# zhoubin-me/agent0

Hardware: AMD Instinct MI355X
Metric: env-frames/sec (learner FPS: transitions collected and saved to replay per second with the learner running, pre-frameskip) (higher is better)
Workload: dtype f32

## Files before the change

agent0_amd/common/atari_wrappers.py:

```python
from __future__ import annotations

from typing import Optional

import torch

ACTION_DIMS = {"Asterix": 9, "BeamRider": 9, "Breakout": 4, "Enduro": 9, "MsPacman": 9, "Qbert": 6, "Seaquest": 18, "SpaceInvaders": 6, "Pong": 6}


class _Space:
    def __init__(self, shape=None, n=None):
        self.shape, self.n = shape, n

    def __getitem__(self, i):
        return self


class DeviceSynthVecEnv:

    H = W = 84
    TASKS = {"stream": 0, "block": 1, "chase": 2}

    def __init__(self, env_id: str, num_envs: int, seed: int = 42, rank: int = 0, ops=None, task: str = "stream"):
        if task not in self.TASKS:
            raise ValueError(f"env_task={task!r}: expected one of {sorted(self.TASKS)}")
# ... 4 lines not shown
        self.ops, self.E, self.seed, self.rank = ops, num_envs, seed, rank
        self.env_id = env_id
        self.action_dim = ACTION_DIMS.get(env_id, 18)
        self.observation_space = _Space(shape=(num_envs, 4, self.H, self.W))
        self.action_space = _Space(n=self.action_dim)
        n = num_envs * 4 * self.H * self.W
        self._obs = [ops.zeros(n, dtype=torch.uint8), ops.zeros(n, dtype=torch.uint8)]
        self._cur = 0
        self.ep_ret = ops.zeros(num_envs)
        self.reward, self.terminal, self.truncated = ops.zeros(num_envs), ops.zeros(num_envs), ops.zeros(num_envs)
        self.life_loss, self.final_mask, self.final_ret = ops.zeros(num_envs), ops.zeros(num_envs), ops.zeros(num_envs)
        self.g = 0

    @property
    def obs(self) -> torch.Tensor:
        return self._obs[self._cur]

    def set_history(self, k: int):
        k = max(int(k), 2)
        if k != len(self._obs):
            n = self._obs[0].numel()
            cur = self._obs[self._cur]
            self._obs = [cur] + [self.ops.zeros(n, dtype=torch.uint8) for _ in range(k - 1)]
            self._cur = 0

    def history(self, j: int) -> torch.Tensor:
        return self._obs[(self._cur - j) % len(self._obs)]

    def reset(self, **kwargs):
        self.g = 0
        self._cur = 0
        self.ops.env_reset(self.seed, self.rank, self.E, self._obs[0], self.ep_ret, task=self.task)
        return self._obs[0], {}

    def step(self, action: torch.Tensor, final_mask: Optional[torch.Tensor] = None, final_ret: Optional[torch.Tensor] = None, ctrl: Optional[torch.Tensor] = None):
        self.g += 1
        nxt = (self._cur + 1) % len(self._obs)
        fm = self.final_mask if final_mask is None else final_mask
        fr = self.final_ret if final_ret is None else final_ret
        self.ops.env_step(self.seed, self.rank, self.E, self.g, self._obs[self._cur], self._obs[nxt], self.ep_ret, self.reward,
                          self.terminal, self.truncated, self.life_loss, fm, fr, ctrl, action=action, A=self.action_dim, task=self.task)
        self._cur = nxt
        info = {"life_loss": self.life_loss, "final_mask": fm, "final_ret": fr}
        return self._obs[nxt], self.reward, self.terminal, self.truncated, info

    def step_commit(self, action, final_mask, final_ret, n, steps, gamma, ring_act, ring_rew, ring_done, obs0, replay, start_slot, ctrl=None):
        self.g += 1
        nxt = (self._cur + 1) % len(self._obs)
        self.ops.env_step_commit(self.seed, self.rank, self.E, self.g, self._obs[self._cur], self._obs[nxt], self.ep_ret, final_mask, final_ret, n, steps, gamma,
                                 action, ring_act, ring_rew, ring_done, obs0, replay.frames, replay.size, start_slot, replay.act, replay.rew, replay.done, ctrl, A=self.action_dim, task=self.task)
        self._cur = nxt
        return self._obs[nxt]

    def act_step_commit(self, tail_args, final_mask, final_ret, n, steps, gamma, ring_act, ring_rew, ring_done, obs0, replay, start_slot, kind: str = "qhead", enc=None):
        self.g += 1
        nxt = (self._cur + 1) % len(self._obs)
        common = (self.seed, self.rank, self.g, self._obs[self._cur], self._obs[nxt], self.ep_ret, final_mask, final_ret, n, steps, gamma, ring_act, ring_rew, ring_done, obs0,
                  replay.frames, replay.size, start_slot, replay.act, replay.rew, replay.done)
        if enc is not None:
            {"qhead": self.ops.actor_qhead_env_step_enc, "dist": self.ops.actor_dist_tail_env_step_enc, "quantile": self.ops.actor_quantile_tail_env_step_enc}[kind](
                *tail_args, *common, task=self.task, wt=enc[0], enc_w=enc[1], act3_next=enc[2])
        else:
            {"qhead": self.ops.actor_qhead_env_step, "dist": self.ops.actor_dist_tail_env_step, "quantile": self.ops.actor_quantile_tail_env_step}[kind](*tail_args, *common, task=self.task)
        self._cur = nxt
        return self._obs[nxt]

    def state_dict(self) -> dict:
        return {"g": int(self.g), "cur": int(self._cur), "seed": int(self.seed), "rank": int(self.rank), "obs": torch.stack(self._obs).cpu(), "ep_ret": self.ep_ret.cpu()}

    def load_state_dict(self, sd: dict):
        if len(sd["obs"]) != len(self._obs) or sd["obs"][0].numel() != self._obs[0].numel():
            raise ValueError(f"env state: {len(sd['obs'])} observation buffers of {sd['obs'][0].numel()} bytes, this env keeps {len(self._obs)} of {self._obs[0].numel()}")
        self.g, self._cur, self.seed, self.rank = int(sd["g"]), int(sd["cur"]), int(sd["seed"]), int(sd["rank"])
        for dst, src in zip(self._obs, sd["obs"]):
            dst.copy_(torch.as_tensor(src).reshape(-1))
        self.ep_ret.copy_(torch.as_tensor(sd["ep_ret"]))

    def close(self):
        pass


from .host_envs import AtariSlice, FireOnReset, LifeLossInfo, PRESS_AFTER_RESET


def real_atari_available() -> bool:
    try:
        import gymnasium, ale_py
    except ImportError:
        return False
    return True


def make_atari(env_id: str, num_envs: int, episode_life: bool = True, seed: int = 42, rank: int = 0, ops=None, synthetic=None, num_workers=None, task: str = "stream",
               groups: int = 1):
    groups = int(groups)
    if not 1 <= groups <= int(num_envs):
        raise ValueError(f"make_atari: groups={groups} must lie in [1, num_envs={num_envs}] (actor.env_groups)")
    if synthetic is None:
        synthetic = not real_atari_available()
    if synthetic:
        return DeviceSynthVecEnv(env_id, num_envs, seed=seed, rank=rank, ops=ops, task=task)
    from .env_pool import HostEnvGroups, HostEnvPool

    if num_workers is None:
        num_workers = 0 if num_envs < 4 else min(16, max(1, num_envs // 16))
    if groups >= 2:
        return HostEnvGroups(AtariSlice(env_id, episode_life, seed + 1000003 * rank), num_envs, groups=groups, obs_shape=(4, 84, 84),
                             action_dim=ACTION_DIMS.get(env_id, 18), num_workers=num_workers, ops=ops)
    return HostEnvPool(AtariSlice(env_id, episode_life, seed + 1000003 * rank), num_envs, obs_shape=(4, 84, 84), action_dim=ACTION_DIMS.get(env_id, 18),
                       num_workers=num_workers, ops=ops)
```

agent0_amd/csrc/net.hip:

```cpp
#include "igemm_x9.h"
#include "short_k_fwd.h"
#include "a0_internal.h"
#include "net_impl.h"
#include "update_tail.h"

#include <vector>

__global__ __launch_bounds__(256) void a0_reduce_slabs_kernel(const float* __restrict__ slabs, long long slab_stride, int nslab,
                                                               float* __restrict__ out, long long count) {
    __shared__ float red[8][33];
    const int c = threadIdx.x & 31, g = threadIdx.x >> 5;
    const long long i = (long long)blockIdx.x * 32 + c;
    float s = 0.f;
    if (i < count)
        for (int z = g; z < nslab; z += 8) s += slabs[(long long)z * slab_stride + i];
    red[g][c] = s;
    __syncthreads();
    if (g == 0 && i < count) {
        float t = 0.f;
#pragma unroll
        for (int j = 0; j < 8; ++j) t += red[j][c];
        out[i] = t;
    }
}
// ... 494 lines not shown
extern "C" int a0_dense_fwd_partial_multi_slabs(int n, int R, int N, int K) { return a0_fwd_multi_splits(n, R, N, K); }

extern "C" int a0_dense_fwd_partial_multi(int n, const float* const* X, int ldx, const float* const* W, int R, int N, int K, float* const* slabs, const long long* slab_stride,
                                          void* stream) {
    A0_TRY
    if (!X || !W || !slabs || (ldx & 3) || !a0_dense_fwd_partial_multi_ok(n, R, N, K)) return a0_fail(A0_EINVAL, "a0_dense_fwd_partial_multi: shapes a0_dense_fwd_partial_multi_ok accepts");
    a0_x9_group<OpMatKC, OpMatKC, EpiSlab> grp;
    for (int i = 0; i < 3; ++i) {
        const int j = i < n ? i : 0;
        if (!X[j] || !W[j] || !slabs[j]) return a0_fail(A0_EINVAL, "a0_dense_fwd_partial_multi: null operand");
        grp.pa[i] = a0_mat_src{X[j], ldx};
        grp.pb[i] = a0_mat_src{W[j], K};
        const long long stride = slab_stride ? slab_stride[j] : (long long)R * N;
        if (stride < (long long)R * N || (stride & 3)) return a0_fail(A0_EINVAL, "a0_dense_fwd_partial_multi: slab stride");
        grp.pe[i] = EpiSlab::Params{slabs[j], stride, N};
    }
    const int splits = a0_fwd_multi_splits(n, R, N, K);
    hipEvent_t e0 = nullptr, e1 = nullptr;
    const bool probe = a0_probe_events(A0_TAG_DENSE_FWD, &e0, &e1);
    A0_HIP_THROW((a0_igemm_x9_group_launch<OpMatKC, OpMatKC, EpiSlab, 4, 2, 1, 1>((hipStream_t)stream, n, grp, R, N, K, splits, e0, e1)));
    if (probe) a0_probe_commit(2.0 * n * (double)R * (double)N * (double)K);
    return A0_OK;
    A0_CATCH
}

#include "actor_tail.h"
__global__ __launch_bounds__(256) void a0_actor_qhead_kernel(const float* __restrict__ slabs, long long slab_stride, int nslab, const float* __restrict__ b1,
                                                             const float* __restrict__ W2, const float* __restrict__ b2, int A, int dueling, int E,
                                                             unsigned long long seed, uint32_t stream_a, uint32_t stream_u, unsigned long long off_a,
                                                             unsigned long long off_u, float eps, const long long* __restrict__ ctrl,
                                                             const float* __restrict__ eps_ptr, int* __restrict__ action, float* __restrict__ qmax) {
    __shared__ float raw[4][64];
    extern __shared__ float w2s[];
    const int lane = threadIdx.x & 63, wave = threadIdx.x >> 6;
    const int e = blockIdx.x * 4 + wave;
    const int NQ = A + (dueling ? 1 : 0);
    for (int i = threadIdx.x; i < NQ * 128; i += 256) ((a0_f4*)w2s)[i] = ((const a0_f4*)W2)[i];
    __syncthreads();
    if (e >= E) return;
    if (ctrl) { off_a += (unsigned long long)ctrl[A0_CTRL_RNG_ACTION]; off_u += (unsigned long long)ctrl[A0_CTRL_RNG_UNIFORM]; }
    eps = a0_env_eps(eps, eps_ptr, (uint32_t)__builtin_amdgcn_readfirstlane(e));
    int act = 0; float best = 0.f;
    a0_qhead_wave(slabs, slab_stride, nslab, b1, w2s, b2, A, dueling, e, lane, raw[wave], seed, stream_a, stream_u, off_a, off_u, eps, act, best);
    if (lane == 0) { action[e] = act; qmax[e] = best; }
}

__global__ __launch_bounds__(512) void a0_actor_qhead_env_kernel(a0_qenv_args P) {
    __shared__ float raw[64];
    __shared__ int s_chase_cell;
    extern __shared__ float w2s[];
    a0_actor_qhead_env_body(P, raw, w2s, &s_chase_cell);
}

extern "C" long long a0_actor_qhead_scratch(int E, int K) {
    const int splits = a0_fc1_splits(E, 512, K);
    return (long long)splits * E * 512;
}

extern "C" int a0_actor_qhead_n(const float* feat, int E, int K, int splits, const float* W1, const float* b1, const float* W2, const float* b2, int A, int dueling,
                                float* scratch, unsigned long long seed, unsigned int stream_a, unsigned int stream_u, unsigned long long off_a,
                                unsigned long long off_u, float eps, const long long* ctrl, const float* eps_ptr, int* action, float* qmax, void* stream) {
    A0_TRY
    if (!feat || !W1 || !b1 || !W2 || !b2 || !scratch || !action || !qmax || E < 1 || K < 4 || (K & 3) || A < 1 || A + (dueling ? 1 : 0) > 24)
        return a0_fail(A0_EINVAL, "a0_actor_qhead: bad argument (A + dueling <= 24: the head rows are staged in 48 KB of LDS)");
    if (splits < 1 || splits > 64 || splits > (K + 31) / 32) return a0_fail(A0_EINVAL, "a0_actor_qhead_n: splits must lie in [1, min(64, ceil(K / 32))]");
    a0_hip_backend bk{(hipStream_t)stream};
    a0_mat_src a{feat, K};
    a0_mat_src bw{W1, K};
    EpiSlab::Params ep{scratch, (long long)E * 512, 512};
    bk.tag = A0_TAG_DENSE_FWD;
    a0_fc1_partial_launch(bk, a, bw, ep, E, 512, K, splits);
    hipLaunchKernelGGL(a0_actor_qhead_kernel, dim3((E + 3) / 4), dim3(256), (size_t)(A + (dueling ? 1 : 0)) * 512 * sizeof(float), (hipStream_t)stream, scratch, (long long)E * 512, splits, b1, W2, b2, A, dueling, E,
                       seed, stream_a, stream_u, off_a, off_u, eps, ctrl, eps_ptr, action, qmax);
    A0_HIP_THROW(hipGetLastError());
    return A0_OK;
    A0_CATCH
}

extern "C" int a0_actor_qhead(const float* feat, int E, int K, const float* W1, const float* b1, const float* W2, const float* b2, int A, int dueling,
                              float* scratch, unsigned long long seed, unsigned int stream_a, unsigned int stream_u, unsigned long long off_a,
                              unsigned long long off_u, float eps, const long long* ctrl, const float* eps_ptr, int* action, float* qmax, void* stream) {
    return a0_actor_qhead_n(feat, E, K, a0_fc1_splits(E, 512, K), W1, b1, W2, b2, A, dueling, scratch, seed, stream_a, stream_u, off_a, off_u, eps, ctrl, eps_ptr, action,
                            qmax, stream);
}

extern "C" int a0_actor_qhead_env_step(const float* feat, int E, int K, const float* W1, const float* b1, const float* W2, const float* b2, int A, int dueling,
                                       float* scratch, unsigned long long seed, unsigned int stream_a, unsigned int stream_u, unsigned long long off_a,
                                       unsigned long long off_u, float eps, const long long* ctrl, const float* eps_ptr, int* action, float* qmax,
                                       unsigned long long env_seed, unsigned int rank, unsigned int g, const uint8_t* obs_in, uint8_t* obs_out, float* ep_ret,
                                       float* final_mask, float* final_ret, int n, long long steps, double gamma, int* ring_act, float* ring_rew, float* ring_done,
                                       const uint8_t* obs0, uint8_t* frames, long long cap, long long start_slot, int* r_act, float* r_rew, float* r_done, int task, void* stream) {
    A0_TRY
    if (!feat || !W1 || !b1 || !W2 || !b2 || !scratch || !action || !qmax || E < 1 || K < 4 || (K & 3) || A < 1 || A + (dueling ? 1 : 0) > 24)
        return a0_fail(A0_EINVAL, "a0_actor_qhead_env_step: bad argument (A + dueling <= 24: the head rows are staged in 48 KB of LDS)");
    if (!obs_in || !obs_out || obs_in == obs_out || !ep_ret || !final_mask || !final_ret || !ring_act || !ring_rew || !ring_done || !obs0 || !frames || !r_act ||
        !r_rew || !r_done || n < 1 || steps < 0 || cap < E || start_slot < 0 || task < A0_ENV_TASK_STREAM || task > A0_ENV_TASK_CHASE || (task == A0_ENV_TASK_CHASE && A < 4))
        return a0_fail(A0_EINVAL, "a0_actor_qhead_env_step: bad env argument (the chase task needs at least four actions)");
    if ((((uintptr_t)obs_in) | ((uintptr_t)obs_out) | ((uintptr_t)obs0) | ((uintptr_t)frames)) & 15) return a0_fail(A0_EINVAL, "a0_actor_qhead_env_step: buffers must be 16-byte aligned");
    a0_hip_backend bk{(hipStream_t)stream};
    const int splits = a0_fc1_splits(E, 512, K);
    a0_mat_src a{feat, K};
    a0_mat_src bw{W1, K};
    EpiSlab::Params ep{scratch, (long long)E * 512, 512};
    bk.tag = A0_TAG_DENSE_FWD;
    a0_fc1_partial_launch(bk, a, bw, ep, E, 512, K, splits);
    a0_qenv_args P;
    P.slabs = scratch; P.slab_stride = (long long)E * 512; P.nslab = splits; P.b1 = b1; P.W2 = W2; P.b2 = b2; P.A = A; P.dueling = dueling; P.E = E;
    P.rng_seed = seed; P.stream_a = stream_a; P.stream_u = stream_u; P.off_a = off_a; P.off_u = off_u; P.eps = eps; P.ctrl = ctrl; P.eps_ptr = eps_ptr;
    P.action = action; P.qmax = qmax;
    P.env_seed = env_seed; P.rank = rank; P.g = g; P.obs_in = obs_in; P.obs_out = obs_out; P.ep_ret = ep_ret; P.final_mask = final_mask; P.final_ret = final_ret;
    P.n = n; P.steps = steps; P.gamma = gamma; P.ring_act = ring_act; P.ring_rew = ring_rew; P.ring_done = ring_done; P.obs0 = obs0; P.frames = frames;
    P.cap = cap; P.start = start_slot % cap; P.r_act = r_act; P.r_rew = r_rew; P.r_done = r_done; P.task = task;
    hipLaunchKernelGGL(a0_actor_qhead_env_kernel, dim3(E), dim3(512), (size_t)(A + (dueling ? 1 : 0)) * 512 * sizeof(float), (hipStream_t)stream, P);
    A0_HIP_THROW(hipGetLastError());
    return A0_OK;
    A0_CATCH
}

extern "C" int a0_actor_qhead_env_step_enc(const float* feat, int E, int K, const float* W1, const float* b1, const float* W2, const float* b2, int A, int dueling,
                                           float* scratch, unsigned long long seed, unsigned int stream_a, unsigned int stream_u, unsigned long long off_a,
                                           unsigned long long off_u, float eps, const long long* ctrl, const float* eps_ptr, int* action, float* qmax,
                                           unsigned long long env_seed, unsigned int rank, unsigned int g, const uint8_t* obs_in, uint8_t* obs_out, float* ep_ret,
                                           float* final_mask, float* final_ret, int n, long long steps, double gamma, int* ring_act, float* ring_rew, float* ring_done,
                                           const uint8_t* obs0, uint8_t* frames, long long cap, long long start_slot, int* r_act, float* r_rew, float* r_done, int task,
                                           const float* wt, const a0_encoder_weights* w, float* act3_next, void* stream) {
    A0_TRY
    if (!feat || !W1 || !b1 || !W2 || !b2 || !scratch || !action || !qmax || E < 1 || K != 3136 || A < 1 || A + (dueling ? 1 : 0) > 24)
        return a0_fail(A0_EINVAL, "a0_actor_qhead_env_step_enc: bad argument (4 x 84 x 84 observations, A + dueling <= 24)");
    if (!obs_in || !obs_out || obs_in == obs_out || !ep_ret || !final_mask || !final_ret || !ring_act || !ring_rew || !ring_done || !obs0 || !frames || !r_act ||
        !r_rew || !r_done || n < 1 || steps < 0 || cap < E || start_slot < 0 || task < A0_ENV_TASK_STREAM || task > A0_ENV_TASK_CHASE || (task == A0_ENV_TASK_CHASE && A < 4))
        return a0_fail(A0_EINVAL, "a0_actor_qhead_env_step_enc: bad env argument");
    if ((((uintptr_t)obs_in) | ((uintptr_t)obs_out) | ((uintptr_t)obs0) | ((uintptr_t)frames)) & 15) return a0_fail(A0_EINVAL, "a0_actor_qhead_env_step_enc: buffers must be 16-byte aligned");
    a0_hip_backend bk{(hipStream_t)stream};
    const int splits = a0_fc1_splits(E, 512, K);
    a0_mat_src a{feat, K};
    a0_mat_src bw{W1, K};
    EpiSlab::Params ep{scratch, (long long)E * 512, 512};
    bk.tag = A0_TAG_DENSE_FWD;
    a0_fc1_partial_launch(bk, a, bw, ep, E, 512, K, splits);
    a0_qenv_args P;
    P.slabs = scratch; P.slab_stride = (long long)E * 512; P.nslab = splits; P.b1 = b1; P.W2 = W2; P.b2 = b2; P.A = A; P.dueling = dueling; P.E = E;
    P.rng_seed = seed; P.stream_a = stream_a; P.stream_u = stream_u; P.off_a = off_a; P.off_u = off_u; P.eps = eps; P.ctrl = ctrl; P.eps_ptr = eps_ptr;
    P.action = action; P.qmax = qmax;
    P.env_seed = env_seed; P.rank = rank; P.g = g; P.obs_in = obs_in; P.obs_out = obs_out; P.ep_ret = ep_ret; P.final_mask = final_mask; P.final_ret = final_ret;
    P.n = n; P.steps = steps; P.gamma = gamma; P.ring_act = ring_act; P.ring_rew = ring_rew; P.ring_done = ring_done; P.obs0 = obs0; P.frames = frames;
    P.cap = cap; P.start = start_slot % cap; P.r_act = r_act; P.r_rew = r_rew; P.r_done = r_done; P.task = task;
    return a0_actor_step_enc_launch(P, wt, w, act3_next, (hipStream_t)stream);
    A0_CATCH
}

__global__ __launch_bounds__(256) void a0_mean_rows_kernel(const float* __restrict__ x, int E, float* __restrict__ out) {
    __shared__ float red[256];
    const float* p = x + (long long)blockIdx.x * E;
    float s = 0.f;
    for (int e = threadIdx.x; e < E; e += 256) s += p[e];
    red[threadIdx.x] = s;
    __syncthreads();
    for (int o = 128; o > 0; o >>= 1) { if ((int)threadIdx.x < o) red[threadIdx.x] += red[threadIdx.x + o]; __syncthreads(); }
    if (threadIdx.x == 0) out[blockIdx.x] = red[0] / (float)E;
}

extern "C" int a0_mean_rows(const float* x, int T, int E, float* out, void* stream) {
    if (!x || !out || T < 1 || E < 1) return a0_fail(A0_EINVAL, "a0_mean_rows: bad argument");
    hipLaunchKernelGGL(a0_mean_rows_kernel, dim3(T), dim3(256), 0, (hipStream_t)stream, x, E, out);
    return a0_fail_hip((int)hipGetLastError(), "a0_mean_rows");
}

extern "C" int a0_dense_dgrad(const float* dY, const float* W, const float* act_mask, float* dX, int R, int N, int K, void* stream) {
    A0_TRY
    if (!dY || !W || !dX || R < 1 || (N & 3) || (K & 3)) return a0_fail(A0_EINVAL, "a0_dense_dgrad: bad shape");
    a0_hip_backend bk{(hipStream_t)stream};
    a0_dense_dgrad_impl(bk, dY, W, act_mask, dX, R, N, K);
    return A0_OK;
    A0_CATCH
}

extern "C" int a0_dense_dgrad_hadamard_ok(int R, int N, int K, int n) {
    return (g_gemm_x9 != 0 && (n == 32 || n == 64) && R >= 4096 && !(R & 255) && !(R % n) && !(N & 15) && N >= 64 && !(K & 3) && K >= 128) ? 1 : 0;
}
extern "C" int a0_dense_dgrad_hadamard(const float* dY, const float* W, const float* emb, const float* feat, float* demb, float* d3, int R, int N, int K, int n, void* stream) {
    A0_TRY
    if (!dY || !W || !emb || !feat || !demb || !d3 || !a0_dense_dgrad_hadamard_ok(R, N, K, n)) return a0_fail(A0_EINVAL, "a0_dense_dgrad_hadamard: shapes a0_dense_dgrad_hadamard_ok accepts");
    const a0_mat_src a{dY, N};
    const a0_mat_src bw{W, K};
    const EpiHadamard::Params e{emb, feat, demb, d3, K, n};
    hipEvent_t e0 = nullptr, e1 = nullptr;
    const bool probe = a0_probe_events(A0_TAG_DENSE_DGRAD, &e0, &e1);
    A0_HIP_THROW((a0_igemm_x9_launch<OpMatKC, OpMatXC, EpiHadamard, 4, 2, 2, 2, 1>((hipStream_t)stream, a, bw, e, R, K, N, 1, e0, e1)));
    if (probe) a0_probe_commit(2.0 * (double)R * (double)N * (double)K);
    return A0_OK;
    A0_CATCH
}

extern "C" int a0_dense_dgrad_wgrad_ok(int R, int N, int K) {
    const long long b128 = (long long)((R + 127) / 128) * ((K + 63) / 64), b64 = (long long)((N + 63) / 64) * ((K + 63) / 64);
    return (g_gemm_x9 != 0 && g_probe.tag == 0 && R == N && R >= 1 && R <= 1024 && !(N & 3) && !(K & 3) && b128 < 256 && b64 >= 256 && N >= 512 &&
            (long long)((R + 127) / 128) * ((K + 127) / 128) < A0_X9_BIG_TILES) ? 1 : 0;
}
static int a0_dense_dgrad_wgrad_small_ok(int R, int N, int K) {
    const long long t1 = (long long)((R + 63) / 64) * ((K + 63) / 64), t2 = (long long)((N + 63) / 64) * ((K + 63) / 64);
    return (g_gemm_x9 != 0 && g_probe.tag == 0 && R >= 64 && R <= 1024 && N >= 64 && !(N & 3) && !(K & 3) && t1 + t2 <= 256 && t2 >= 16) ? 1 : 0;
// ... 126 lines not shown
```

agent0_amd/csrc/runtime.hip:

```cpp
#include "learner_state.h"

#include <chrono>
#include <thread>

namespace {

typedef a0_host_rng Rng;
constexpr int STREAM_EGREEDY_U = 1, STREAM_EGREEDY_A = 2, STREAM_SUMTREE = 5, STREAM_PERM = 6;

struct Owned {
    std::vector<void*> ptrs;
    template <class T> T* alloc(long long n, bool zero = true) {
        void* p = nullptr;
        A0_HIP_THROW(hipMalloc(&p, (size_t)(n > 0 ? n : 1) * sizeof(T)));
        ptrs.push_back(p);
        if (zero) A0_HIP_THROW(hipMemset(p, 0, (size_t)(n > 0 ? n : 1) * sizeof(T)));
        return (T*)p;
    }
    ~Owned() { for (void* p : ptrs) (void)hipFree(p); }
};

__global__ void a0_pow_scalar_kernel(const float* __restrict__ p, double alpha, float* __restrict__ out) {
    const double x = (double)p[0];
    out[0] = (float)(alpha == 0.5 ? sqrt(x) : pow(x, alpha));
// ... 194 lines not shown
        start[g] = (unsigned long long)(R->ep.pos * B); n_perm[g] = (unsigned long long)R->ep.top; seed[g] = R->ep.seed;
        R->ep.pos += 1;
    }
    A0_CHECK(a0_replay_sample_slots_multi(n, start, n_perm, seed, R->top, R->head(), R->size, R->act, R->rew, R->done, B, R->m_idx, R->m_slot, R->m_act, R->m_rew, R->m_done,
                                          R->m_prio, stream));
    for (int g = 0; g < n; ++g) {
        const long long o = (long long)g * B;
        out[g] = a0_batch{R->m_idx + o, R->m_slot + o, R->m_act + o, R->m_rew + o, R->m_done + o, R->m_prio + o, R->ones};
    }
    return A0_OK;
    A0_CATCH
}

extern "C" int a0_rbuf_update_priority(a0_rbuf* R, const float* loss, const int* learner_state, void* stream) {
    A0_TRY
    if (!R || !loss) return a0_fail(A0_EINVAL, "a0_rbuf_update_priority: null argument");
    if (!R->prio) return A0_OK;
    if (R->flat) return a0_priority_update(R->prio_vec, R->b_idx, loss, R->B, (float)R->d.eps, (float)R->d.alpha, R->pstate, learner_state, stream);
    if (a0_sumtree_set_from_loss_ok(R->cap2)) {
        R->top_stale = true;
        return a0_sumtree_set_from_loss(R->tree, R->cap2, R->b_idx, loss, R->B, (float)R->d.eps, (float)R->d.alpha, R->pstate, learner_state, 1, stream);
    }
    A0_CHECK(a0_priority_from_loss(loss, R->B, (float)R->d.eps, (float)R->d.alpha, R->b_prio, R->pstate, learner_state, stream));
    return a0_sumtree_set(R->tree, R->cap2, R->b_idx, R->b_prio, R->B, learner_state, stream);
    A0_CATCH
}

struct a0_actor {
    a0_actor_desc d;
    int E = 0, T = 0, n = 1, K = 2, cur = 0, feat = 3136, obs_bytes = 4 * 84 * 84;
    unsigned g = 0;
    long long steps = 0;
    Rng rng;
    Owned mem;
    std::vector<uint8_t*> obs;
    float *ep_ret = nullptr, *qmax_all = nullptr, *stat_mask = nullptr, *stat_ret = nullptr, *qs = nullptr, *ring_rew = nullptr, *ring_done = nullptr, *act3 = nullptr, *scratch = nullptr;
    int *action = nullptr, *ring_act = nullptr;
    std::vector<float> h_mask, h_ret;
    float *p_mask = nullptr, *p_ret = nullptr, *p_qs = nullptr;
    hipEvent_t stats_ev = nullptr;
    ~a0_actor() {
        if (p_mask) (void)hipHostFree(p_mask);
        if (p_ret) (void)hipHostFree(p_ret);
        if (p_qs) (void)hipHostFree(p_qs);
        if (stats_ev) (void)hipEventDestroy(stats_ev);
    }
    float *h = nullptr, *head_slabs = nullptr, *fwd_scratch = nullptr;
    int dist_Npad = 0;
    float *q_taus = nullptr, *q_cosx = nullptr, *q_x = nullptr;
    float *f_logits = nullptr, *f_tau_all = nullptr;
    bool bound = false;
    float *own_flat = nullptr, *own_wt = nullptr, *own_eff = nullptr, *own_noise = nullptr;
    unsigned int* w_planes = nullptr;
    bool pool_on = false;
    a0_env_pool_desc pool{};
    uint8_t* ring_obs = nullptr;
    long long pool_whole = 0;
    float ladder_alpha = 0.f;
    long long ladder_i0 = 0, ladder_n = 1;
    float* eps_vec = nullptr;
};

struct a0_actor_net {
    const float* flat; const float* wt; float* eff; float* noise;
    const a0_learner* L;
    const float* Wf() const { return L->d.noisy ? eff + L->eff_fc1.w() : flat + L->fc1.w(); }
    const float* bf() const { return L->d.noisy ? eff + L->eff_fc1.b() : flat + L->fc1.b(); }
    const float* Wh() const { return L->d.noisy ? eff + L->eff_head.w() : flat + L->head.w(); }
    const float* bh() const { return L->d.noisy ? eff + L->eff_head.b() : flat + L->head.b(); }
};
static a0_actor_net a0_actor_view(const a0_actor* a, a0_learner* L) {
    if (a->own_flat) return a0_actor_net{a->own_flat, a->own_wt, a->own_eff, a->own_noise, L};
    return a0_actor_net{L->online, L->wt_on, L->eff_on, L->noise, L};
}

extern "C" int a0_actor_bind(a0_actor* a, const a0_learner* L, int own_network) {
    A0_TRY
    if (!a || !L) return a0_fail(A0_EINVAL, "a0_actor_bind: null argument");
    if (L->d.A != a->d.A || (L->d.dueling != 0) != (a->d.dueling != 0)) return a0_fail(A0_EINVAL, "a0_actor_bind: actor and learner were created for different heads");
    const int E = a->E;
    const bool dist = L->d.algo == A0_ALGO_C51 || L->d.algo == A0_ALGO_QR, fqf = L->d.algo == A0_ALGO_FQF, quant = L->d.algo == A0_ALGO_IQN || fqf;
    if (a->bound && a->dist_Npad != L->Npad) return a0_fail(A0_EINVAL, "a0_actor_bind: this actor was sized for another head");
    if (!a->bound) {
        const int nt = fqf ? L->F : (quant ? L->d.iqn_K : 1);
        if (quant) {
            const long long R = (long long)E * nt;
            if (a0_dense_fwd_scratch((int)R, L->feat, 64) != 0) return a0_fail(A0_EINVAL, "a0_actor_bind: E * K rows too few for the embedding kernel this path takes");
            a->h = a->mem.alloc<float>(R * 512);
            a->head_slabs = a->mem.alloc<float>((long long)a0_dense_fwd_partial_slabs((int)R, L->Npad, 512) * R * L->Npad);
            long long sc = a0_dense_fwd_scratch((int)R, 512, L->feat);
            if (fqf && a0_dense_fwd_scratch(E, 32, L->feat) > sc) sc = a0_dense_fwd_scratch(E, 32, L->feat);
            a->fwd_scratch = a->mem.alloc<float>(sc > 4 ? sc : 4);
            a->q_taus = a->mem.alloc<float>(ceil_to(R, 4)); a->q_cosx = a->mem.alloc<float>(R * 64); a->q_x = a->mem.alloc<float>(R * L->feat);
            if (fqf) { a->f_logits = a->mem.alloc<float>((long long)E * 32); a->f_tau_all = a->mem.alloc<float>((long long)E * (nt + 1)); }
            if (a0_dense_fwd_wplanes_ok((int)R, 512, L->feat)) a->w_planes = a->mem.alloc<unsigned int>(a0_weight_planes_words(512, L->feat), false);
        } else if (dist) {
            a->h = a->mem.alloc<float>((long long)E * 512);
            a->head_slabs = a->mem.alloc<float>((long long)a0_dense_fwd_partial_slabs(E, L->Npad, 512) * E * L->Npad);
            const long long sc = a0_dense_fwd_scratch(E, 512, L->feat);
            a->fwd_scratch = a->mem.alloc<float>(sc > 4 ? sc : 4);
        }
        a->dist_Npad = L->Npad;
        a->bound = true;
    }
    if (own_network && !a->own_flat) {
        a->own_flat = a->mem.alloc<float>(L->n_pad); a->own_wt = a->mem.alloc<float>(L->wt_floats);
        if (L->d.noisy) { a->own_eff = a->mem.alloc<float>(L->n_eff); a->own_noise = a->mem.alloc<float>(L->noise_len); }
    }
    A0_HIP_THROW(hipDeviceSynchronize());
    return A0_OK;
    A0_CATCH
}

extern "C" int a0_actor_snapshot(a0_actor* a, const a0_learner* L, void* stream) {
    A0_TRY
    if (!a || !L || !a->own_flat) return a0_fail(A0_EINVAL, "a0_actor_snapshot: an actor bound with its own network (a0_actor_bind(actor, learner, 1))");
    hipStream_t st = (hipStream_t)stream;
    A0_HIP_THROW(hipMemcpyAsync(a->own_flat, L->online, (size_t)L->n_pad * 4, hipMemcpyDeviceToDevice, st));
    A0_HIP_THROW(hipMemcpyAsync(a->own_wt, L->wt_on, (size_t)L->wt_floats * 4, hipMemcpyDeviceToDevice, st));
    if (L->d.noisy) {
        A0_HIP_THROW(hipMemcpyAsync(a->own_eff, L->eff_on, (size_t)L->n_eff * 4, hipMemcpyDeviceToDevice, st));
        A0_HIP_THROW(hipMemcpyAsync(a->own_noise, L->noise, (size_t)L->noise_len * 4, hipMemcpyDeviceToDevice, st));
    }
    return A0_OK;
    A0_CATCH
}

extern "C" int a0_actor_create(const a0_actor_desc* d, a0_actor** out) {
    A0_TRY
    if (!d || !out) return a0_fail(A0_EINVAL, "a0_actor_create: null argument");
    if (d->E < 1 || d->T < 1 || d->A < 1 || d->n_step < 1 || d->reset_noise_freq < 0 || !(d->discount > 0.0) || d->env_task < A0_ENV_TASK_STREAM || d->env_task > A0_ENV_TASK_CHASE || (d->env_task == A0_ENV_TASK_CHASE && d->A < 4))
        return a0_fail(A0_EINVAL, "a0_actor_create: bad description");
    a0_actor* a = new a0_actor();
    try {
        a->d = *d; a->E = d->E; a->T = d->T; a->n = d->n_step;
        a->rng.init(d->seed, d->rank);
        a->K = 2;
        if (a->n > 1) {
            a->K = a->n + 1;
            for (int r = a->n + 1; r < 2 * a->n + 3; ++r) if (a->T % r == 0) { a->K = r; break; }
        }
        const long long E = a->E, T = a->T;
        for (int i = 0; i < a->K; ++i) a->obs.push_back(a->mem.alloc<uint8_t>(E * a->obs_bytes));
        a->ep_ret = a->mem.alloc<float>(E); a->qmax_all = a->mem.alloc<float>(T * E); a->stat_mask = a->mem.alloc<float>(T * E); a->stat_ret = a->mem.alloc<float>(T * E);
        a->qs = a->mem.alloc<float>(T); a->action = a->mem.alloc<int>(E);
        a->ring_act = a->mem.alloc<int>((long long)a->n * E); a->ring_rew = a->mem.alloc<float>((long long)a->n * E); a->ring_done = a->mem.alloc<float>((long long)a->n * E);
        a->act3 = a->mem.alloc<float>(E * a->feat); a->scratch = a->mem.alloc<float>(a0_actor_qhead_scratch(a->E, a->feat));
        a->h_mask.resize((size_t)(T * E)); a->h_ret.resize((size_t)(T * E));
        if (a0_env_synth_reset_task(d->seed, d->rank, a->E, a->obs[0], a->ep_ret, d->env_task, nullptr) != A0_OK) { delete a; return A0_EINVAL; }
        A0_HIP_THROW(hipDeviceSynchronize());
    } catch (...) { delete a; throw; }
    *out = a;
    return A0_OK;
    A0_CATCH
}

extern "C" int a0_actor_destroy(a0_actor* a) { delete a; return A0_OK; }

extern "C" int a0_actor_attach_pool(a0_actor* a, const a0_env_pool_desc* d) {
    A0_TRY
    if (!a || !d) return a0_fail(A0_EINVAL, "a0_actor_attach_pool: null argument");
    if (d->E != a->E || d->nstack < 2 || d->frame_bytes < 16 || d->frame_bytes % 16 || (long long)d->nstack * d->frame_bytes != a->obs_bytes || d->W < 1 || d->seq < 0 ||
        !(d->timeout_s > 0.0) || !d->act_dev || !d->ctl_dev || !d->done_host || !d->new_dev || d->seq_mask <= 0)
        return a0_fail(A0_EINVAL, "a0_actor_attach_pool: bad description (E and nstack * frame_bytes of the actor, at least one worker)");
    for (int h = 0; h < 2; ++h)
        if (!d->new_host[h] || !d->scal_host[h] || !d->obs_host[h] || !d->obs_dev[h] || !d->scal_dev[h]) return a0_fail(A0_EINVAL, "a0_actor_attach_pool: null buffer");
    if (a->own_flat) return a0_fail(A0_ESTATE, "a0_actor_attach_pool: an actor with its own network (the launch schedule) does not drive a pool");
    if (a->steps != 0) return a0_fail(A0_ESTATE, "a0_actor_attach_pool: attach before the first rollout");
    if (a->n > 1 && !a->ring_obs) a->ring_obs = a->mem.alloc<uint8_t>((long long)a->n * a->E * a->obs_bytes);
    a->pool = *d;
    a->pool_on = true;
    a->pool_whole = 0;
    return A0_OK;
    A0_CATCH
}

extern "C" int a0_actor_set_eps_ladder(a0_actor* a, float alpha, long long i0, long long n_total) {
    A0_TRY
    if (!a) return a0_fail(A0_EINVAL, "a0_actor_set_eps_ladder: null handle");
    if (!(alpha > 0.f)) { a->ladder_alpha = 0.f; return A0_OK; }
    if (i0 < 0 || n_total < 1 || i0 + a->E > n_total) return a0_fail(A0_EINVAL, "a0_actor_set_eps_ladder: the actor's envs are [i0, i0 + E) of n_total");
    if (!a->eps_vec) { a->eps_vec = a->mem.alloc<float>(a->E); A0_HIP_THROW(hipDeviceSynchronize()); }
    a->ladder_alpha = alpha; a->ladder_i0 = i0; a->ladder_n = n_total;
    return A0_OK;
    A0_CATCH
}

extern "C" int a0_actor_detach_pool(a0_actor* a) {
    if (!a) return a0_fail(A0_EINVAL, "a0_actor_detach_pool: null handle");
    a->pool_on = false;
    return A0_OK;
}

extern "C" int a0_actor_pool_seq(a0_actor* a, long long* seq_out, long long* whole_out, long long set_seq) {
    if (!a || !a->pool_on) return a0_fail(A0_ESTATE, "a0_actor_pool_seq: no pool attached");
    if (seq_out) *seq_out = a->pool.seq;
    if (whole_out) *whole_out = a->pool_whole;
    if (set_seq >= 0) a->pool.seq = set_seq;
    return A0_OK;
}

static int a0_pool_wait(const a0_env_pool_desc& P, long long seq) {
    const auto t0 = std::chrono::steady_clock::now();
    for (;;) {
        bool all = true, dead = false;
        for (int w = 0; w < P.W; ++w) {
            const long long v = __atomic_load_n(P.done_host + w, __ATOMIC_ACQUIRE);
            all = all && v == seq;
            dead = dead || v < 0;
        }
        if (all) return A0_OK;
        if (dead) return a0_fail(A0_ESTATE, "a0_actor_rollout: an env worker process died");
        const double waited = std::chrono::duration<double>(std::chrono::steady_clock::now() - t0).count();
        if (waited > P.timeout_s) return a0_fail(A0_ESTATE, "a0_actor_rollout: the env workers did not finish a step within the pool's timeout");
        if (waited > 2e-3) std::this_thread::sleep_for(std::chrono::microseconds(20));
    }
}

static int a0_actor_compose(const a0_actor_net& V, void* stream) {
    const a0_learner* L = V.L;
    const float *mu[3], *sg[3], *nin[3], *nw[3], *nb[3];
    float* eff[3];
    int N[3], K[3], r0[3], r1[3];
    for (int k = 0; k < L->n_mods; ++k) {
        const a0_noise_mod& m = L->mods[k];
        const Blk &bm = m.block ? L->head : L->fc1, &bs = m.block ? L->head_sigma : L->fc1_sigma, &be = m.block ? L->eff_head : L->eff_fc1;
        mu[k] = V.flat + bm.off; sg[k] = V.flat + bs.off; eff[k] = V.eff + be.off; N[k] = bm.N; K[k] = bm.K; r0[k] = m.r0; r1[k] = m.r1;
        nin[k] = V.noise + m.off_in; nw[k] = V.noise + m.off_w; nb[k] = V.noise + m.off_b;
// ... 38 lines not shown
                                            E, a->rng.seed, STREAM_EGREEDY_A, STREAM_EGREEDY_U, oa, ou, epsilon, nullptr, eps_vec, a->action, qm, stream));
        } else if (dist) {
            A0_CHECK(a0_dense_fwd(a->act3, L->feat, V.Wf(), V.bf(), a->h, E, 512, L->feat, 1, a->fwd_scratch, stream));
            const int ns = a0_dense_fwd_partial_slabs(E, L->Npad, 512);
            A0_CHECK(a0_dense_fwd_partial(a->h, 512, V.Wh(), E, L->Npad, 512, a->head_slabs, stream));
            const unsigned long long oa = a->rng.reserve(STREAM_EGREEDY_A, E), ou = a->rng.reserve(STREAM_EGREEDY_U, E);
            A0_CHECK(a0_actor_dist_tail(a->head_slabs, (long long)E * L->Npad, ns, V.bh(), L->Npad, A, L->T, a->d.dueling ? 1 : 0, L->d.algo == A0_ALGO_C51 ? 2 : 1,
                                        L->d.algo == A0_ALGO_C51 ? L->atoms : nullptr, E, a->rng.seed, STREAM_EGREEDY_A, STREAM_EGREEDY_U, oa, ou, epsilon, nullptr, eps_vec,
                                        a->action, qm, stream));
        } else {
            const unsigned long long oa = a->rng.reserve(STREAM_EGREEDY_A, E), ou = a->rng.reserve(STREAM_EGREEDY_U, E);
            A0_CHECK(a0_actor_qhead(a->act3, E, a->feat, V.Wf(), V.bf(), V.Wh(), V.bh(), A, a->d.dueling ? 1 : 0, a->scratch, a->rng.seed, STREAM_EGREEDY_A, STREAM_EGREEDY_U,
                                    oa, ou, epsilon, nullptr, eps_vec, a->action, qm, stream));
        }
        A0_CHECK(a0_env_pool_send(a->action, (int*)P.act_dev, E, (long long*)P.ctl_dev, P.step_word | (seq & P.seq_mask), stream));
        A0_CHECK(a0_pool_wait(P, seq));
        int whole = 0;
        A0_CHECK(a0_env_pool_upload((const uint8_t*)P.new_host[half], (uint8_t*)P.new_dev, (const float*)P.scal_host[half], (float*)P.scal_dev[half], 7, 6,
                                    (const uint8_t*)P.obs_host[half], nullptr, nxt, E, P.nstack, P.frame_bytes, &whole, stream));
        a->pool_whole += whole;
        A0_CHECK(a0_host_step_ingest(cur, (const uint8_t*)P.new_dev, (const float*)P.scal_dev[half], nxt, E, P.nstack, P.frame_bytes, P.use_life_loss, a->action, a->n, a->n,
                                     a->steps, a->d.discount, a->ring_act, a->ring_rew, a->ring_done, a->ring_obs, R->frames, R->size, (start + (long long)t * E) % R->size,
                                     R->act, R->rew, R->done, a->stat_mask + (long long)t * E, a->stat_ret + (long long)t * E, nullptr, stream));
        P.seq = seq;
        a->steps += 1;
    }
    return a0_mean_rows(a->qmax_all, a->T, E, a->qs, stream);
}

extern "C" int a0_actor_rollout(a0_actor* a, a0_learner* L, a0_rbuf* R, float epsilon, void* stream) {
    A0_TRY
    a0_trace_scope range("rollout");
    if (!a || !L || !R) return a0_fail(A0_EINVAL, "a0_actor_rollout: null argument");
    if (L->d.A != a->d.A || (L->d.dueling != 0) != (a->d.dueling != 0) || R->obs_bytes != a->obs_bytes || R->size < a->E)
        return a0_fail(A0_EINVAL, "a0_actor_rollout: actor, learner and replay were created for different shapes");
    const int E = a->E, A = a->d.A;
    const bool dist = L->d.algo == A0_ALGO_C51 || L->d.algo == A0_ALGO_QR, fqf = L->d.algo == A0_ALGO_FQF, quant = L->d.algo == A0_ALGO_IQN || fqf;
    const int freq = a->d.reset_noise_freq > 0 ? a->d.reset_noise_freq : 4;
    const int nt = fqf ? L->F : (quant ? L->d.iqn_K : 1);
    if (!a->bound || a->dist_Npad != L->Npad) A0_CHECK(a0_actor_bind(a, L, 0));
    const a0_actor_net V = a0_actor_view(a, L);
    const long long start = R->written % R->size;
    a0_encoder_weights w = L->enc(V.flat);
    if (L->d.noisy && a->steps % freq != 0) A0_CHECK(a0_actor_compose(V, stream));
    const bool planes = quant && a->w_planes && a0_dense_fwd_wplanes_ok(E * nt, 512, L->feat);
    if (planes && !(L->d.noisy && a->steps % freq == 0)) A0_CHECK(a0_split_planes(V.Wf(), a->w_planes, 512, L->feat, stream));
    const float* eps_vec = nullptr;
    if (a->ladder_alpha > 0.f) {
        A0_CHECK(a0_eps_ladder(epsilon, nullptr, a->ladder_alpha, E, a->ladder_i0, a->ladder_n, a->eps_vec, stream));
        eps_vec = a->eps_vec;
        epsilon = A0_EPS_PER_ENV;
    }
    if (a->pool_on) return a0_actor_rollout_pool(a, L, R, epsilon, eps_vec, V, w, start, stream);
    const bool step_enc = !a->own_flat;
    bool feat_ready = false;
    for (int t = 0; t < a->T; ++t) {
        if (L->d.noisy && a->steps % freq == 0) {
            A0_CHECK(a0_rng_normal(a->rng.seed, 4 , a->rng.reserve(4, L->noise_len), 0.1f, V.noise, L->noise_len, stream));
            A0_CHECK(a0_actor_compose(V, stream));
            if (planes) A0_CHECK(a0_split_planes(V.Wf(), a->w_planes, 512, L->feat, stream));
        }
        const uint8_t* cur_obs = a->obs[a->cur];
        a0_frames_arg f{cur_obs, nullptr, (long long)a->obs_bytes, 0};
        if (!feat_ready) A0_CHECK(a0_net_encoder_fwd_fused(L->C, L->H, L->W, V.wt, &w, &f, E, nullptr, nullptr, a->act3, stream));
        feat_ready = false;
        const long long back = (a->steps + 1 < a->n ? a->steps + 1 : a->n) - 1;
        const uint8_t* obs0 = a->obs[((a->cur - back) % a->K + a->K) % a->K];
        if (quant) {
            const int rows = E * nt;
            const float* on = V.flat;
            if (fqf) {
                A0_CHECK(a0_dense_fwd(a->act3, L->feat, on + L->frac.w(), on + L->frac.b(), a->f_logits, E, 32, L->feat, 0, a->fwd_scratch, stream));
                A0_CHECK(a0_fqf_taus_cos(a->f_logits, 32, a->f_tau_all, a->q_taus, a->q_cosx, 64, E, nt, stream));
            } else {
                A0_CHECK(a0_tau_cos_features(a->rng.seed, 3 , a->rng.reserve(3, rows), nullptr, 0, a->q_taus, a->q_cosx, rows, 64, stream));
            }
            A0_CHECK(a0_dense_fwd_mul(a->q_cosx, 64, on + L->cos.w(), on + L->cos.b(), a->act3, nt, a->q_x, rows, L->feat, 64, 1, stream));
            if (planes) A0_CHECK(a0_dense_fwd_wplanes(a->q_x, L->feat, a->w_planes, V.bf(), a->h, rows, 512, L->feat, 1, stream));
            else A0_CHECK(a0_dense_fwd(a->q_x, L->feat, V.Wf(), V.bf(), a->h, rows, 512, L->feat, 1, a->fwd_scratch, stream));
            const int ns = a0_dense_fwd_partial_slabs(rows, L->Npad, 512);
            A0_CHECK(a0_dense_fwd_partial(a->h, 512, V.Wh(), rows, L->Npad, 512, a->head_slabs, stream));
            const unsigned long long oa = a->rng.reserve(STREAM_EGREEDY_A, E), ou = a->rng.reserve(STREAM_EGREEDY_U, E);
            const int nx = (a->cur + 1) % a->K;
            a->g += 1;
            if (step_enc && t + 1 < a->T) {
                A0_CHECK(a0_actor_quantile_tail_env_step_enc(a->head_slabs, (long long)rows * L->Npad, ns, V.bh(), L->Npad, A, nt, a->d.dueling ? 1 : 0, fqf ? 3 : 1, fqf ? a->f_tau_all : nullptr, E, a->rng.seed,
                                                             STREAM_EGREEDY_A, STREAM_EGREEDY_U, oa, ou, epsilon, nullptr, eps_vec, a->action, a->qmax_all + (long long)t * E, a->d.seed,
                                                             a->d.rank, a->g, cur_obs, a->obs[nx], a->ep_ret, a->stat_mask + (long long)t * E, a->stat_ret + (long long)t * E, a->n, a->steps,
                                                             a->d.discount, a->ring_act, a->ring_rew, a->ring_done, obs0, R->frames, R->size, (start + (long long)t * E) % R->size, R->act,
                                                             R->rew, R->done, a->d.env_task, V.wt, &w, a->act3, stream));
                feat_ready = true;
            } else
            A0_CHECK(a0_actor_quantile_tail_env_step(a->head_slabs, (long long)rows * L->Npad, ns, V.bh(), L->Npad, A, nt, a->d.dueling ? 1 : 0, fqf ? 3 : 1, fqf ? a->f_tau_all : nullptr, E, a->rng.seed,
                                                     STREAM_EGREEDY_A, STREAM_EGREEDY_U, oa, ou, epsilon, nullptr, eps_vec, a->action, a->qmax_all + (long long)t * E, a->d.seed,
                                                     a->d.rank, a->g, cur_obs, a->obs[nx], a->ep_ret, a->stat_mask + (long long)t * E, a->stat_ret + (long long)t * E, a->n, a->steps,
                                                     a->d.discount, a->ring_act, a->ring_rew, a->ring_done, obs0, R->frames, R->size, (start + (long long)t * E) % R->size, R->act,
                                                     R->rew, R->done, a->d.env_task, stream));
            a->cur = nx;
            a->steps += 1;
            continue;
        }
        if (dist) {
            A0_CHECK(a0_dense_fwd(a->act3, L->feat, V.Wf(), V.bf(), a->h, E, 512, L->feat, 1, a->fwd_scratch, stream));
            const int ns = a0_dense_fwd_partial_slabs(E, L->Npad, 512);
            A0_CHECK(a0_dense_fwd_partial(a->h, 512, V.Wh(), E, L->Npad, 512, a->head_slabs, stream));
            const unsigned long long oa = a->rng.reserve(STREAM_EGREEDY_A, E), ou = a->rng.reserve(STREAM_EGREEDY_U, E);
            const int nx = (a->cur + 1) % a->K;
            a->g += 1;
            if (4LL * ((long long)A * L->T + L->T) * 4 > 160 * 1024) return a0_fail(A0_EINVAL, "a0_actor_rollout: head too wide for the distributional tail kernel");
            if (step_enc && t + 1 < a->T) {
                A0_CHECK(a0_actor_dist_tail_env_step_enc(a->head_slabs, (long long)E * L->Npad, ns, V.bh(), L->Npad, A, L->T, a->d.dueling ? 1 : 0, L->d.algo == A0_ALGO_C51 ? 2 : 1,
                                                         L->d.algo == A0_ALGO_C51 ? L->atoms : nullptr, E, a->rng.seed,
                                                         STREAM_EGREEDY_A, STREAM_EGREEDY_U, oa, ou, epsilon, nullptr, eps_vec, a->action, a->qmax_all + (long long)t * E, a->d.seed, a->d.rank,
                                                         a->g, cur_obs, a->obs[nx], a->ep_ret, a->stat_mask + (long long)t * E, a->stat_ret + (long long)t * E, a->n, a->steps, a->d.discount,
                                                         a->ring_act, a->ring_rew, a->ring_done, obs0, R->frames, R->size, (start + (long long)t * E) % R->size, R->act, R->rew, R->done,
                                                         a->d.env_task, V.wt, &w, a->act3, stream));
                feat_ready = true;
            } else
            A0_CHECK(a0_actor_dist_tail_env_step(a->head_slabs, (long long)E * L->Npad, ns, V.bh(), L->Npad, A, L->T, a->d.dueling ? 1 : 0, L->d.algo == A0_ALGO_C51 ? 2 : 1,
                                                 L->d.algo == A0_ALGO_C51 ? L->atoms : nullptr, E, a->rng.seed,
                                                 STREAM_EGREEDY_A, STREAM_EGREEDY_U, oa, ou, epsilon, nullptr, eps_vec, a->action, a->qmax_all + (long long)t * E, a->d.seed, a->d.rank,
                                                 a->g, cur_obs, a->obs[nx], a->ep_ret, a->stat_mask + (long long)t * E, a->stat_ret + (long long)t * E, a->n, a->steps, a->d.discount,
                                                 a->ring_act, a->ring_rew, a->ring_done, obs0, R->frames, R->size, (start + (long long)t * E) % R->size, R->act, R->rew, R->done,
                                                 a->d.env_task, stream));
            a->cur = nx;
            a->steps += 1;
            continue;
        }
        if (A + (a->d.dueling ? 1 : 0) > 24) return a0_fail(A0_EINVAL, "a0_actor_rollout: scalar heads with A + dueling <= 24 actions");
        const unsigned long long off_a = a->rng.reserve(STREAM_EGREEDY_A, E), off_u = a->rng.reserve(STREAM_EGREEDY_U, E);
        const int nxt = (a->cur + 1) % a->K;
        a->g += 1;
        if (step_enc && t + 1 < a->T) {
            A0_CHECK(a0_actor_qhead_env_step_enc(a->act3, E, a->feat, V.Wf(), V.bf(), V.Wh(), V.bh(), A, a->d.dueling ? 1 : 0,
                                                 a->scratch, a->rng.seed, STREAM_EGREEDY_A, STREAM_EGREEDY_U, off_a, off_u, epsilon, nullptr, eps_vec, a->action, a->qmax_all + (long long)t * E,
                                                 a->d.seed, a->d.rank, a->g, cur_obs, a->obs[nxt], a->ep_ret, a->stat_mask + (long long)t * E, a->stat_ret + (long long)t * E, a->n, a->steps,
                                                 a->d.discount, a->ring_act, a->ring_rew, a->ring_done, obs0, R->frames, R->size, (start + (long long)t * E) % R->size, R->act, R->rew, R->done,
                                                 a->d.env_task, V.wt, &w, a->act3, stream));
            feat_ready = true;
        } else
        A0_CHECK(a0_actor_qhead_env_step(a->act3, E, a->feat, V.Wf(), V.bf(), V.Wh(), V.bh(), A, a->d.dueling ? 1 : 0,
                                         a->scratch, a->rng.seed, STREAM_EGREEDY_A, STREAM_EGREEDY_U, off_a, off_u, epsilon, nullptr, eps_vec, a->action, a->qmax_all + (long long)t * E,
                                         a->d.seed, a->d.rank, a->g, cur_obs, a->obs[nxt], a->ep_ret, a->stat_mask + (long long)t * E, a->stat_ret + (long long)t * E, a->n, a->steps,
                                         a->d.discount, a->ring_act, a->ring_rew, a->ring_done, obs0, R->frames, R->size, (start + (long long)t * E) % R->size, R->act, R->rew, R->done,
                                         a->d.env_task, stream));
        a->cur = nxt;
        a->steps += 1;
    }
    return a0_mean_rows(a->qmax_all, a->T, E, a->qs, stream);
    A0_CATCH
}

extern "C" int a0_actor_collect(a0_actor* a, float* qs_host, float* returns_host, int max_returns, int* n_returns, void* stream) {
    A0_TRY
    if (!a) return a0_fail(A0_EINVAL, "a0_actor_collect: null handle");
    hipStream_t st = (hipStream_t)stream;
    const size_t n = (size_t)a->T * a->E;
    if (qs_host) A0_HIP_THROW(hipMemcpyAsync(qs_host, a->qs, (size_t)a->T * 4, hipMemcpyDeviceToHost, st));
    A0_HIP_THROW(hipMemcpyAsync(a->h_mask.data(), a->stat_mask, n * 4, hipMemcpyDeviceToHost, st));
    A0_HIP_THROW(hipMemcpyAsync(a->h_ret.data(), a->stat_ret, n * 4, hipMemcpyDeviceToHost, st));
    A0_HIP_THROW(hipStreamSynchronize(st));
    int k = 0;
    for (size_t i = 0; i < n; ++i)
        if (a->h_mask[i] != 0.f) { if (returns_host && k < max_returns) returns_host[k] = a->h_ret[i]; ++k; }
    if (n_returns) *n_returns = k;
    return A0_OK;
    A0_CATCH
}

extern "C" int a0_actor_collect_begin(a0_actor* a, void* stream) {
    A0_TRY
    if (!a) return a0_fail(A0_EINVAL, "a0_actor_collect_begin: null handle");
    hipStream_t st = (hipStream_t)stream;
    const size_t n = (size_t)a->T * a->E;
    if (!a->p_mask) {
        A0_HIP_THROW(hipHostMalloc((void**)&a->p_mask, n * 4, hipHostMallocDefault));
        A0_HIP_THROW(hipHostMalloc((void**)&a->p_ret, n * 4, hipHostMallocDefault));
        A0_HIP_THROW(hipHostMalloc((void**)&a->p_qs, (size_t)a->T * 4, hipHostMallocDefault));
        A0_HIP_THROW(hipEventCreateWithFlags(&a->stats_ev, hipEventDisableTiming));
    }
    A0_HIP_THROW(hipMemcpyAsync(a->p_qs, a->qs, (size_t)a->T * 4, hipMemcpyDeviceToHost, st));
    A0_HIP_THROW(hipMemcpyAsync(a->p_mask, a->stat_mask, n * 4, hipMemcpyDeviceToHost, st));
    A0_HIP_THROW(hipMemcpyAsync(a->p_ret, a->stat_ret, n * 4, hipMemcpyDeviceToHost, st));
    A0_HIP_THROW(hipEventRecord(a->stats_ev, st));
    return A0_OK;
    A0_CATCH
}

extern "C" int a0_actor_collect_end(a0_actor* a, float* qs_host, float* returns_host, int max_returns, int* n_returns) {
    A0_TRY
    if (!a || !a->stats_ev) return a0_fail(A0_EINVAL, "a0_actor_collect_end: no a0_actor_collect_begin before it");
    A0_HIP_THROW(hipEventSynchronize(a->stats_ev));
    const size_t n = (size_t)a->T * a->E;
    if (qs_host) for (int t = 0; t < a->T; ++t) qs_host[t] = a->p_qs[t];
    int k = 0;
    for (size_t i = 0; i < n; ++i)
        if (a->p_mask[i] != 0.f) { if (returns_host && k < max_returns) returns_host[k] = a->p_ret[i]; ++k; }
    if (n_returns) *n_returns = k;
// ... 105 lines not shown
```

agent0_amd/deepq/agent.py:

```python
from __future__ import annotations

import os

from typing import Optional

import numpy as np
import torch

from agent0_amd.common.atari_wrappers import make_atari
from agent0_amd.common.utils import DeviceRng
from .config import AlgoEnum, ExpConfig
from .dist import eps_ladder_span, graph_capture_kwargs
from .engine import DeviceLearner, Workspace
from .model import DeepQNet, layout_from_cfg
from .replay import ReplayDataset, StageRing, TransitionBlock


def _ops_from(cfg, ops=None):
    if cfg.device.value != "cuda":
        raise RuntimeError("agent0_amd runs on MI355X only: set device=cuda (no CPU fallback; see oracle/ for the CPU restatement used in tests)")
    if ops is None:
        from agent0_amd.ops import HipOps
        ops = HipOps()
    return ops


class Actor:
    def __init__(self, cfg: ExpConfig, model: Optional[DeepQNet] = None, replay: Optional[ReplayDataset] = None, ops=None, rank: int = 0, envs=None):
        self.cfg = cfg
        self.ops = ops = model.ops if model is not None else _ops_from(cfg, ops)
        self.rng = DeviceRng(ops, cfg.seed, rank)
        self.envs = envs if envs is not None else make_atari(cfg.env_id, cfg.actor.num_envs, seed=cfg.seed, rank=rank, ops=ops, task=cfg.env_task,
                                                             groups=int(cfg.actor.env_groups))
        self.obs, _ = self.envs.reset()
        self.model = model if model is not None else DeepQNet(cfg, ops=ops)
        self.replay = replay
        self.L = self.model.L
        E = self.E = int(cfg.actor.num_envs)
        self.n = int(cfg.learner.n_step_q)
        self.steps = 0
        self.obs_bytes = self.L.C * self.L.H * self.L.W
        n_tau = self.L.F if self.L.algo == "fqf" else (cfg.learner.iqn.K if self.L.algo == "iqn" else 1)
        self.n_tau = n_tau
        self.ws = Workspace(ops, self.L, E, n_tau)
        self.taus = ops.empty(E * n_tau) if self.L.algo == "iqn" else None
        self.greedy, self.rand_a, self.action = ops.zeros(E, dtype=torch.int32), ops.zeros(E, dtype=torch.int32), ops.zeros(E, dtype=torch.int32)
        self.u, self.qmax = ops.zeros(E), ops.zeros(E)
        T = max(int(cfg.actor.sample_steps), int(cfg.actor.test_steps) if False else int(cfg.actor.sample_steps))
        self.qs = ops.zeros(T)
        self.fused_tail = self.L.algo in ("dqn", "mdqn") and self.L.feat % 4 == 0 and self.L.A + (1 if self.L.dueling else 0) <= 24
        self.dist_tail = (not self.fused_tail) and self.L.algo in ("c51", "qr") and 4 * (self.L.A * self.L.T + self.L.T) * 4 <= 160 * 1024
        self._head_slabs = ops.empty(ops.dense_fwd_partial_slabs(E, self.L.Npad, 512) * E * self.L.Npad) if self.dist_tail else None
        self.quant_tail = (self.L.algo in ("iqn", "fqf") and hasattr(self.envs, "act_step_commit") and self.obs_bytes == 4 * 84 * 84
                           and ops.dense_fwd_scratch(E * n_tau, self.L.feat, self.L.num_cosines) == 0)
        self.quant_slabs = self.L.algo in ("iqn", "fqf") and ops.dense_fwd_scratch(E * n_tau, self.L.feat, self.L.num_cosines) == 0
        if self.quant_slabs:
            self._head_slabs = ops.empty(ops.dense_fwd_partial_slabs(E * n_tau, self.L.Npad, 512) * E * n_tau * self.L.Npad)
        self.qmax_all = ops.zeros(T * E) if (self.fused_tail or self.dist_tail or self.quant_slabs) else None
        self._qh_scratch = ops.empty(ops.actor_qhead_scratch(E, self.L.feat)) if self.fused_tail else None
        self.stat_mask, self.stat_ret = ops.zeros(T * E), ops.zeros(T * E)
        self.ring_act, self.ring_rew, self.ring_done = ops.zeros(self.n * E, dtype=torch.int32), ops.zeros(self.n * E), ops.zeros(self.n * E)
        T_ = int(cfg.actor.sample_steps)
        self.ring_len = next((r for r in range(self.n, 2 * self.n + 1) if T_ % r == 0), self.n)
        self.env_history = self.n > 1 and hasattr(self.envs, "set_history")
        if self.env_history:
            self.envs.set_history(next((r for r in range(self.n + 1, 2 * self.n + 3) if T_ % r == 0), self.n + 1))
        self.ring_obs = ops.zeros(self.ring_len * E * self.obs_bytes, dtype=torch.uint8) if (self.n > 1 and not self.env_history) else None
        self.use_graph = True
        self._graph, self._graph_warm = None, 0
        self.ctrl = ops.zeros(8, dtype=torch.int64)
        self.eps_dev = ops.zeros(1)
        self._ctrl_host = torch.zeros(8, dtype=torch.int64).pin_memory()
        self._eps_host = torch.zeros(1).pin_memory()
        self.rank = int(rank)
        self.ladder_alpha = max(float(cfg.actor.eps_ladder), 0.0)
        self.eps_vec = None
        self.out_act, self.out_rew, self.out_done = ops.zeros(E, dtype=torch.int32), ops.zeros(E), ops.zeros(E)
        self.atoms = self.model.head.atoms.reshape(-1).contiguous() if self.L.algo == "c51" else None
        self._stage = None
        self.fused_commit = hasattr(self.envs, "step_commit") and (self.obs_bytes == 4 * 84 * 84)
        self.tail_env = (self.fused_tail or self.dist_tail) and self.fused_commit and hasattr(self.envs, "act_step_commit") and os.environ.get("A0_TAIL_ENV", "1") != "0"
        self.groups = None
        if hasattr(self.envs, "pools"):
            if not (self.fused_tail or self.dist_tail or self.quant_slabs):
                raise ValueError("a grouped host env needs a head with a one-kernel actor tail (scalar: A + dueling <= 24; c51 / qr: the head's outputs in LDS); use one group")
            self._splits = self._split_plan()
            rows = E * n_tau if self.quant_slabs else E
            self.groups = []
            for pool, off in zip(self.envs.pools, self.envs.offsets):
                k = pool.E
                g = dict(pool=pool, off=off, E=k, ws=Workspace(ops, self.L, k, n_tau), action=self.action[off:off + k],
                         ring_act=ops.zeros(self.n * k, dtype=torch.int32), ring_rew=ops.zeros(self.n * k), ring_done=ops.zeros(self.n * k),
                         out_act=ops.zeros(k, dtype=torch.int32), out_rew=ops.zeros(k), out_done=ops.zeros(k),
                         scratch=ops.empty(self._splits["qhead"] * k * 512) if self.fused_tail else None,
                         slabs=ops.empty(self._splits["head"] * k * (rows // E) * self.L.Npad) if not self.fused_tail else None,
                         ring_obs=ops.zeros(self.ring_len * k * self.obs_bytes, dtype=torch.uint8) if self.n > 1 else None)
                self.groups.append(g)

    def _split_plan(self) -> dict:
        L, ops, dev, E = self.L, self.ops, self.model._dev, self.E
        if self.fused_tail:
            return {"qhead": ops.dense_fwd_partial_slabs(E, 512, L.feat)}
        R = E * self.n_tau if self.quant_slabs else E
        plan = {"fc1": dev.dense_splits("fc1", R), "head": ops.dense_fwd_partial_slabs(R, L.Npad, 512)}
        if L.algo == "fqf":
            plan["frac"] = dev.dense_splits("frac", E)
        return plan

    def _qhead_args(self, epsilon, ctrl, eps_ptr, t):
        L, E, dev, rng = self.L, self.E, self.model._dev, self.rng
        (W1, b1), (W2, b2) = dev.wb("fc1"), dev.wb("head")
        return (self.ws.act3, E, L.feat, W1, b1, W2, b2, L.A, L.dueling, self._qh_scratch, rng.seed, rng.STREAM_EGREEDY_A, rng.STREAM_EGREEDY_U,
                rng.reserve(rng.STREAM_EGREEDY_A, E), rng.reserve(rng.STREAM_EGREEDY_U, E), float(epsilon), self.action, self.qmax_all[t * E:(t + 1) * E], ctrl, eps_ptr)

    def _dist_tail_args(self, epsilon, ctrl, eps_ptr, t):
        L, ops, E, dev, rng = self.L, self.ops, self.E, self.model._dev, self.rng
        dev._dense(self.ws.act3, L.feat, "fc1", self.ws.h, E, True)
        Wh, bh = dev.wb("head")
        ns = ops.dense_fwd_partial(self.ws.h, 512, Wh, E, L.Npad, 512, self._head_slabs)
        return (self._head_slabs, ns, bh, L.Npad, L.A, L.T, L.dueling, 2 if L.algo == "c51" else 1, self.atoms, E, rng.seed, rng.STREAM_EGREEDY_A, rng.STREAM_EGREEDY_U,
                rng.reserve(rng.STREAM_EGREEDY_A, E), rng.reserve(rng.STREAM_EGREEDY_U, E), float(epsilon), self.action, self.qmax_all[t * E:(t + 1) * E], ctrl, eps_ptr)

    def _quant_tail_args(self, epsilon, ctrl, eps_ptr, t, w_planes=None):
        L, ops, E, dev, rng = self.L, self.ops, self.E, self.model._dev, self.rng
        fused_cos = hasattr(ops, "tau_cos_features")
        if L.algo == "fqf":
            dev.fqf_taus(self.ws, E, with_cos=fused_cos)
            taus, aux, mode = self.ws.tau_hat, self.ws.tau_all, 3
        else:
            if fused_cos:
                rng.uniform_cos(rng.STREAM_TAUS, self.taus, self.ws.cosx, E * self.n_tau, L.num_cosines)
            else:
                rng.uniform(rng.STREAM_TAUS, self.taus, E * self.n_tau)
            taus, aux, mode = self.taus, None, 1
        ns = dev.head_slabs(self.ws, E, taus, self.n_tau, self._head_slabs, cos_ready=fused_cos,
                            w_planes=getattr(self, "_planes_on", False) if w_planes is None else w_planes)
        _, bh = dev.wb("head")
        return (self._head_slabs, ns, bh, L.Npad, L.A, self.n_tau, L.dueling, mode, aux, E, rng.seed, rng.STREAM_EGREEDY_A, rng.STREAM_EGREEDY_U,
                rng.reserve(rng.STREAM_EGREEDY_A, E), rng.reserve(rng.STREAM_EGREEDY_U, E), float(epsilon), self.action, self.qmax_all[t * E:(t + 1) * E], ctrl, eps_ptr)

    def _act_device(self, epsilon: float, qs_slot: Optional[torch.Tensor], ctrl=None, eps_ptr=None, t: int = 0, tail: bool = True):
        L, ops, E, dev = self.L, self.ops, self.E, self.model._dev
        dev.encode(self.ws, self.obs, None, self.obs_bytes, 0, E, keep=False)
        if not tail:
            return
        if self.fused_tail:
            ops.actor_qhead(*self._qhead_args(epsilon, ctrl, eps_ptr, t))
            return
        if self.dist_tail:
            ops.actor_dist_tail(*self._dist_tail_args(epsilon, ctrl, eps_ptr, t))
            return
        if self.quant_slabs:
            ops.actor_quantile_tail(*self._quant_tail_args(epsilon, ctrl, eps_ptr, t, w_planes=False))
            return
        if L.algo == "fqf":
            dev.fqf_taus(self.ws, E)
            dev.head(self.ws, E, self.ws.tau_hat, L.F)
        elif L.algo == "iqn":
            self.rng.uniform(self.rng.STREAM_TAUS, self.taus, E * self.n_tau)
            dev.head(self.ws, E, self.taus, self.n_tau)
        else:
            dev.head(self.ws, E)
        dev.select(self.ws, E, self.n_tau, self.greedy, qmax=self.qmax, atoms=self.atoms)
        rng = self.rng
        ops.actor_egreedy_rng(self.greedy, rng.seed, rng.STREAM_EGREEDY_A, rng.STREAM_EGREEDY_U, rng.reserve(rng.STREAM_EGREEDY_A, E),
                              rng.reserve(rng.STREAM_EGREEDY_U, E), L.A, float(epsilon), E, self.action, self.qmax, qs_slot, ctrl, eps_ptr)

    def _eps_ladder(self, epsilon, eps_ptr=None):
        from agent0_amd.ops import EPS_PER_ENV
        i0, n_total = eps_ladder_span(self.rank, self.E)
        if self.eps_vec is None:
            self.eps_vec = self.ops.zeros(self.E)
        self.ops.eps_ladder(epsilon, eps_ptr, self.ladder_alpha, self.E, i0, n_total, self.eps_vec)
        return EPS_PER_ENV, self.eps_vec

    def act(self, epsilon):
        one = self.ops.zeros(1)
        self._act_device(epsilon, one)
        if self.fused_tail or self.dist_tail or self.quant_slabs:
            self.ops.mean_rows(self.qmax_all, 1, self.E, one)
        return self.action.cpu().numpy().astype(np.int64), float(one[0])

    def reset(self):
        self.obs, _ = self.envs.reset()

    def _rollout(self, epsilon, T, start, bound, test, stage, frames_out, ctrl=None, eps_ptr=None):
        cfg, ops, E = self.cfg, self.ops, self.E
        R = self.ring_len
        if self.ladder_alpha > 0 and not test:
            epsilon, eps_ptr = self._eps_ladder(epsilon, eps_ptr)
        if cfg.learner.noisy_net and self.steps % cfg.learner.reset_noise_freq != 0:
            self.model._dev.compose_noise()
        dev = self.model._dev
        step_enc = ((self.tail_env and (self.fused_tail or self.dist_tail) or (self.quant_tail and self.fused_commit and hasattr(ops, "actor_quantile_tail_env_step_enc")))
                    and bound and not test and dev.fused and (self.L.C, self.L.H, self.L.W) == (4, 84, 84) and hasattr(ops, "actor_qhead_env_step_enc")
                    and not isinstance(self.replay, StageRing))
        self._planes_on = bool(self.quant_tail and bound and not test and self.fused_commit and hasattr(ops, "dense_fwd_wplanes")
                               and ops.dense_fwd_wplanes_ok(E * self.n_tau, 512, self.L.feat))
        if self._planes_on and not (cfg.learner.noisy_net and self.steps % cfg.learner.reset_noise_freq == 0):
            dev.refresh_fc1_planes()
        feat_ready = False
        for t in range(T):
            if cfg.learner.noisy_net and self.steps % cfg.learner.reset_noise_freq == 0:
                self.model.reset_noise(rng=self.rng)
                if self._planes_on:
                    dev.refresh_fc1_planes()
            merged = bound and not test and (self.tail_env or (self.quant_tail and self.fused_commit))
            if not feat_ready:
                self._act_device(epsilon, self.qs[t:t + 1], ctrl, eps_ptr, t, tail=not merged)
            cur_obs = self.obs
            if self.n > 1 and self.env_history:
                obs0 = self.envs.history(min(self.steps + 1, self.n) - 1)
            elif self.n > 1:
                slot = self.steps % R
                self.ring_obs[slot * E * self.obs_bytes:(slot + 1) * E * self.obs_bytes].copy_(cur_obs)
                count = min(self.steps + 1, self.n)
                oldest = (self.steps - (count - 1)) % R
                obs0 = self.ring_obs[oldest * E * self.obs_bytes:(oldest + 1) * E * self.obs_bytes]
            else:
                obs0 = cur_obs
            if merged:
                rp = self.replay
                kind = "qhead" if self.fused_tail else ("dist" if self.dist_tail else "quantile")
                targs = {"qhead": self._qhead_args, "dist": self._dist_tail_args, "quantile": self._quant_tail_args}[kind](epsilon, ctrl, eps_ptr, t)
                enc = (dev.wt, dev.encoder_weights(), self.ws.act3) if (step_enc and t + 1 < T) else None
                self.obs = self.envs.act_step_commit(targs, self.stat_mask[t * E:(t + 1) * E], self.stat_ret[t * E:(t + 1) * E], self.n, self.steps,
                                                     float(cfg.learner.discount), self.ring_act, self.ring_rew, self.ring_done, obs0, rp, (start + t * E) % rp.size,
                                                     kind=kind, enc=enc)
                feat_ready = enc is not None
                self.steps += 1
                continue
            if bound and not test and self.fused_commit:
                rp = self.replay
                obs_next = self.envs.step_commit(self.action, self.stat_mask[t * E:(t + 1) * E], self.stat_ret[t * E:(t + 1) * E], self.n, self.steps,
                                                 float(cfg.learner.discount), self.ring_act, self.ring_rew, self.ring_done, obs0, rp, (start + t * E) % rp.size, ctrl)
                self.steps += 1
                self.obs = obs_next
                continue
            obs_next, reward, terminal, truncated, info = self.envs.step(self.action, final_mask=self.stat_mask[t * E:(t + 1) * E],
                                                                         final_ret=self.stat_ret[t * E:(t + 1) * E], ctrl=ctrl)
            ops.actor_nstep(E, self.n, self.steps, float(cfg.learner.discount), self.action, reward, terminal, truncated, info.get("life_loss"),
                            self.ring_act, self.ring_rew, self.ring_done, self.out_act, self.out_rew, self.out_done, ctrl)
            self.steps += 1
            if test:
                frames_out.append(obs_next.view(E, self.L.C, self.L.H, self.L.W)[:4, -1:].cpu().numpy())
            elif bound:
                rp = self.replay
                ops.replay_insert(rp.frames, rp.size, self.obs_bytes, (start + t * E) % rp.size, E, obs0, obs_next, self.out_act, self.out_rew, self.out_done,
                                  rp.act, rp.rew, rp.done, ctrl)
            else:
                sl = slice(t * E, (t + 1) * E)
                stage["obs"][sl].copy_(obs0.view(E, -1)); stage["obs_next"][sl].copy_(obs_next.view(E, -1))
                stage["act"][sl].copy_(self.out_act); stage["rew"][sl].copy_(self.out_rew); stage["done"][sl].copy_(self.out_done)
            self.obs = obs_next
        if self.fused_tail or self.dist_tail or self.quant_slabs:
            ops.mean_rows(self.qmax_all, T, E, self.qs)

    def _rollout_host(self, epsilon, T, start):
        cfg, ops, E, rp = self.cfg, self.ops, self.E, self.replay
        R, ob, gamma = self.ring_len, self.obs_bytes, float(cfg.learner.discount)
        if getattr(self, "_host_actions", None) is None:
            self._host_actions = (self.action, ops.zeros(E, dtype=torch.int32))

        def bookkeeping(t, steps, action, cur_obs, obs_next, reward, terminal, truncated, info):
            sl = slice(t * E, (t + 1) * E)
            self.stat_mask[sl].copy_(info["final_mask"], non_blocking=True)
            self.stat_ret[sl].copy_(info["final_ret"], non_blocking=True)
            if self.n > 1:
                slot = steps % R
                self.ring_obs[slot * E * ob:(slot + 1) * E * ob].copy_(cur_obs)
                oldest = (steps - (min(steps + 1, self.n) - 1)) % R
                obs0 = self.ring_obs[oldest * E * ob:(oldest + 1) * E * ob]
            else:
                obs0 = cur_obs
            ops.actor_nstep(E, self.n, steps, gamma, action, reward, terminal, truncated, info.get("life_loss"), self.ring_act, self.ring_rew, self.ring_done,
                            self.out_act, self.out_rew, self.out_done, None)
            ops.replay_insert(rp.frames, rp.size, ob, (start + t * E) % rp.size, E, obs0, obs_next, self.out_act, self.out_rew, self.out_done, rp.act, rp.rew, rp.done, None)

        eps_ptr = None
        if self.ladder_alpha > 0:
            epsilon, eps_ptr = self._eps_ladder(epsilon)
# ... 407 lines not shown
```

agent0_amd/deepq/engine.py:

```python
from __future__ import annotations

import math
import os
from typing import Dict, List, Optional

import torch

from .layout import Block, NetLayout

MODE_IDENT, MODE_MEAN, MODE_C51, MODE_FQF = 0, 1, 2, 3


def clip_limit(value) -> float:
    return float(value) if value is not None and value > 0 else -1.0


def target_tau_value(value) -> float:
    if value is None or not value > 0:
        return 0.0
    tau = float(value)
    if tau >= 1.0:
        raise ValueError(f"learner.target_tau={tau!r}: must be below 1 (tau >= 1 is the hard copy: leave learner.target_tau off)")
    return tau

# ... 139 lines not shown
        if self._scratch is None or self._scratch.numel() < n:
            self._scratch = self.ops.empty(n)
        return self._scratch

    def encode(self, ws: Workspace, frames, slot, sample_stride, chan_off, B, keep: bool = True):
        if self.fused:
            self.ops.encoder_fwd_fused(self.net, self.wt, self.encoder_weights(), frames, slot, sample_stride, chan_off, B,
                                       ws.act1 if keep else None, ws.act2 if keep else None, ws.act3)
        else:
            self.ops.encoder_fwd(self.net, self.encoder_weights(), frames, slot, sample_stride, chan_off, B, ws.act1, ws.act2, ws.act3)

    def dense_splits(self, name, R) -> int:
        blk = self.L.eff[name] if (self.L.noisy and name in ("fc1", "head")) else self.L.blocks[name]
        return self.ops.dense_fwd_splits(R, blk.N, blk.K)

    def _dense(self, X, ldx, name, Y, R, relu, splits: Optional[int] = None):
        W, b = self.wb(name)
        blk = self.L.eff[name] if (self.L.noisy and name in ("fc1", "head")) else self.L.blocks[name]
        N, K = blk.N, blk.K
        if splits is not None:
            self.ops.dense_fwd_n(X, ldx, W, b, Y, R, N, K, relu, splits, self.scratch(splits * R * N if splits > 1 else 0))
            return
        self.ops.dense_fwd(X, ldx, W, b, Y, R, N, K, relu, self.scratch(self.ops.dense_fwd_scratch(R, N, K)))

    def head(self, ws: Workspace, B, taus: Optional[torch.Tensor] = None, n_tau: int = 1, feat: Optional[torch.Tensor] = None):
        L, ops = self.L, self.ops
        feat = ws.act3 if feat is None else feat
        if not L.quantile:
            self._dense(feat, L.feat, "fc1", ws.h, B, True)
            self._dense(ws.h, 512, "head", ws.raw, B, False)
            ops.dueling_fwd(ws.raw, L.Npad, ws.q, B, L.A, L.T, L.dueling)
            return ws.q
        R = B * n_tau
        ops.cos_features(taus, ws.cosx, R, L.num_cosines)
        if not ws.grads and ops.dense_fwd_scratch(R, L.feat, L.num_cosines) == 0:
            Wc, bc = self.wb("cos")
            ops.dense_fwd_mul(ws.cosx, L.num_cosines, Wc, bc, feat, n_tau, ws.x, R, L.feat, L.num_cosines, True)
        elif ws.grads and ops.dense_fwd_mul_keep_ok(R, L.feat, L.num_cosines, L.num_cosines):
            Wc, bc = self.wb("cos")
            ops.dense_fwd_mul_keep(ws.cosx, L.num_cosines, Wc, bc, feat, n_tau, ws.emb, ws.x, R, L.feat, L.num_cosines, True)
        else:
            self._dense(ws.cosx, L.num_cosines, "cos", ws.emb, R, True)
            ops.hadamard_fwd(ws.emb, feat, ws.x, B, n_tau, L.feat)
        self._dense(ws.x, L.feat, "fc1", ws.h, R, True)
        self._dense(ws.h, 512, "head", ws.raw, R, False)
        ops.dueling_fwd(ws.raw, L.Npad, ws.q, R, L.A, 1, L.dueling)
        return ws.q

    def refresh_fc1_planes(self):
        W, _ = self.wb("fc1")
        if getattr(self, "fc1_planes", None) is None:
            self.fc1_planes = torch.empty(self.ops.weight_planes_words(512, self.L.feat), dtype=torch.int32, device=self.flat.device)
        self.ops.split_planes(W, self.fc1_planes, 512, self.L.feat)

    def head_slabs(self, ws: Workspace, B, taus: torch.Tensor, n_tau: int, slabs: torch.Tensor, cos_ready: bool = False, w_planes: bool = False,
                   splits: Optional[dict] = None) -> int:
        L, ops = self.L, self.ops
        R = B * n_tau
        if not cos_ready:
            ops.cos_features(taus, ws.cosx, R, L.num_cosines)
        Wc, bc = self.wb("cos")
        ops.dense_fwd_mul(ws.cosx, L.num_cosines, Wc, bc, ws.act3, n_tau, ws.x, R, L.feat, L.num_cosines, True)
        if w_planes:
            ops.dense_fwd_wplanes(ws.x, L.feat, self.fc1_planes, self.wb("fc1")[1], ws.h, R, 512, L.feat, True)
        else:
            self._dense(ws.x, L.feat, "fc1", ws.h, R, True, splits=None if splits is None else splits["fc1"])
        Wh, _ = self.wb("head")
        if splits is not None:
            return ops.dense_fwd_partial_n(ws.h, 512, Wh, R, L.Npad, 512, splits["head"], slabs)
        return ops.dense_fwd_partial(ws.h, 512, Wh, R, L.Npad, 512, slabs)

    def fc1(self, ws: Workspace, B):
        self._dense(ws.act3, self.L.feat, "fc1", ws.h, B, True)

    def fqf_taus(self, ws: Workspace, B, with_cos: bool = False, splits: Optional[int] = None):
        L = self.L
        self._dense(ws.act3, L.feat, "frac", ws.frac_logits, B, False, splits=splits)
        if with_cos:
            self.ops.fqf_taus_cos(ws.frac_logits, L.Fpad, ws.tau_all, ws.tau_hat, ws.cosx, L.num_cosines, B, L.F)
        else:
            self.ops.fqf_taus(ws.frac_logits, L.Fpad, ws.tau_all, ws.tau_hat, B, L.F)

    def select(self, ws: Workspace, B, n_tau, a_star, qsel=None, qmax=None, atoms=None):
        L, ops = self.L, self.ops
        if L.algo in ("dqn", "mdqn"):
            ops.select_action(ws.q, L.A, 1, 1, B, L.A, 1, MODE_IDENT, None, a_star, qsel, qmax)
        elif L.algo == "qr":
            ops.select_action(ws.q, L.A * L.T, L.T, 1, B, L.A, L.T, MODE_MEAN, None, a_star, qsel, qmax)
        elif L.algo == "c51":
            ops.select_action(ws.q, L.A * L.T, L.T, 1, B, L.A, L.T, MODE_C51, atoms, a_star, qsel, qmax)
        elif L.algo == "iqn":
            ops.select_action(ws.q, n_tau * L.A, 1, L.A, B, L.A, n_tau, MODE_MEAN, None, a_star, qsel, qmax)
        else:
            ops.select_action(ws.q, n_tau * L.A, 1, L.A, B, L.A, n_tau, MODE_FQF, ws.tau_all, a_star, qsel, qmax)


class DeviceLearner:

    def __init__(self, ops, L: NetLayout, batch_size: int, *, discount=0.99, n_step=1, double_q=False, lr=5e-4,
                 target_update_freq=500, vmin=-10.0, vmax=10.0, K=32, N=64, N_dash=64, max_grad_norm=-1.0, adam_eps=None,
                 mdqn_tau=0.03, mdqn_lo=-1.0, clip_grad_norm=-1.0, target_tau=0.0):
        self.ops, self.L, self.B = ops, L, batch_size
        self.net = ops.net(L.C, L.H, L.W)
        self.online = DeviceNet(ops, L, self.net)
        self.target = DeviceNet(ops, L, self.net)
        self.noise_joint = None
# ... 465 lines not shown
```

agent0_amd/deepq/native_loop.py:

```python
from __future__ import annotations

import ctypes as C
import os
import time
from typing import Optional

import numpy as np
import torch

from agent0_amd import _abi
from .config import ReplayEnum


class _RbufDesc(C.Structure):
    _fields_ = [("size", C.c_longlong), ("obs_bytes", C.c_int), ("B", C.c_int), ("prioritize", C.c_int), ("alpha", C.c_double), ("eps", C.c_double), ("beta0", C.c_double),
                ("total_steps", C.c_longlong), ("seed", C.c_ulonglong)]


class _ActorDesc(C.Structure):
    _fields_ = [("E", C.c_int), ("T", C.c_int), ("A", C.c_int), ("dueling", C.c_int), ("n_step", C.c_int), ("discount", C.c_double), ("seed", C.c_ulonglong), ("rank", C.c_uint),
                ("env_task", C.c_int), ("reset_noise_freq", C.c_int)]


class _PoolDesc(C.Structure):
# ... 99 lines not shown


class NativeLoop:
    def __init__(self, tr):
        self.tr = tr
        self.learner = self.rbuf = self.actor = None
        self.lib, self.ok = _abi.load(), _abi.check
        try:
            self._create(tr)
        except Exception:
            self.close()
            raise

    def _create(self, tr):
        cfg, ops = tr.cfg, tr.ops
        lc, rc = cfg.learner, cfg.replay
        lib, ok = self.lib, self.ok
        eng, rp, actor = tr.learner.engine, tr.replay, tr.actors[1]
        L = eng.L
        self.E, self.T, self.B = int(cfg.actor.num_envs), int(cfg.actor.sample_steps), int(lc.batch_size)
        self.prio = rp.prioritize
        desc = _abi.LearnerDesc(int(cfg.action_dim), int(bool(lc.dueling_head)), int(bool(lc.double_q)), self.B, int(lc.n_step_q), float(lc.discount), float(lc.learning_rate),
                                float(eng.adam_eps), int(lc.target_update_freq), {"dqn": 0, "c51": 1, "iqn": 2, "fqf": 3, "qr": 4, "mdqn": 5}[lc.algo.name], int(lc.qr.num_atoms if lc.algo.name == "qr" else lc.c51.num_atoms), float(lc.c51.vmin), float(lc.c51.vmax),
                                int(bool(lc.noisy_net)), (int(cfg.seed) + 15485863) & 0xFFFFFFFFFFFFFFFF, int(lc.iqn.K), int(lc.iqn.N), int(lc.iqn.N_dash), int(lc.iqn.F), float(lc.mdqn.tau), float(lc.mdqn.lo),
                                float(lc.max_grad_norm))
        p = lambda t: None if t is None else t.data_ptr()
        bufs = _LearnerBuffers(p(eng.online.flat), p(eng.target.flat), p(eng.grads), p(eng.adam_m), p(eng.adam_v), p(eng.state), p(eng.scalars), p(eng.loss_ring),
                               int(eng.loss_ring.numel()), p(eng.online.wt), p(eng.target.wt), p(eng.online.eff), p(eng.target.eff), p(eng.noise_joint), p(getattr(eng, "rms_sq", None)))
        self.learner = C.c_void_p()
        ok(lib.a0_learner_create_on(C.addressof(desc), C.addressof(bufs), C.addressof(self.learner)), "a0_learner_create_on")
        assert int(lib.a0_learner_param_floats(self.learner)) == L.n_params_padded
        if lc.algo.name == "c51":
            atoms = (C.c_float * L.T)(*[float(x) for x in eng.atoms.cpu().tolist()])
            ok(lib.a0_learner_set_support(self.learner, atoms), "a0_learner_set_support")
        if eng.clip_grad_norm > 0:
            ok(lib.a0_learner_set_grad_clip(self.learner, C.c_double(eng.clip_grad_norm), p(eng.gnorm_ring), int(eng.gnorm_ring.numel())), "a0_learner_set_grad_clip")
        hook = eng.grad_hook
        if hook is not None:
            ok(lib.a0_learner_set_exchange(self.learner, C.c_longlong(int(hook.comm) if hook.active else 0)), "a0_learner_set_exchange")
        if lc.noisy_net:
            rng = tr.learner.rng
            ok(lib.a0_learner_set_rng(self.learner, rng.STREAM_NOISE, C.c_ulonglong(rng.offsets.get(rng.STREAM_NOISE, 0))), "a0_learner_set_rng")
        self.flat = self.prio and not rp.use_sumtree
        rd = _RbufDesc(int(rp.size), int(rp.obs_bytes), self.B, 2 if self.flat else int(self.prio), float(rc.alpha), float(rc.eps), float(rc.beta0), int(cfg.trainer.total_steps), int(cfg.seed) + 104729)
        self.rbuf = C.c_void_p()
        ok(lib.a0_rbuf_create_on(C.addressof(rd), p(rp.frames), p(rp.act), p(rp.rew), p(rp.done), p(rp.priority) if self.flat else p(rp._tree) if self.prio else None, p(rp._pstate), C.addressof(self.rbuf)),
           "a0_rbuf_create_on")
        ad = _ActorDesc(self.E, self.T, int(cfg.action_dim), int(bool(lc.dueling_head)), int(lc.n_step_q), float(lc.discount), int(cfg.seed), int(tr.rank),
                        {"stream": 0, "block": 1, "chase": 2}[cfg.env_task], int(lc.reset_noise_freq))
        self.actor = C.c_void_p()
        ok(lib.a0_actor_create(C.addressof(ad), C.addressof(self.actor)), "a0_actor_create")
        if eng.target_tau > 0:
            ok(lib.a0_learner_set_target_tau(self.learner, C.c_double(eng.target_tau)), "a0_learner_set_target_tau")
        if actor.ladder_alpha > 0:
            from .dist import eps_ladder_span
            ops.actor_set_eps_ladder(self.actor, actor.ladder_alpha, *eps_ladder_span(int(tr.rank), self.E))
        self.lp = bool(tr.use_lp)
        ok(lib.a0_actor_bind(self.actor, self.learner, int(self.lp)), "a0_actor_bind")
        from agent0_amd.common.env_pool import HostEnvPool
        self.pool = actor.envs if isinstance(actor.envs, HostEnvPool) else None
        if self.pool is not None:
            self._pool_desc = pool_desc(self.pool)
            ok(lib.a0_actor_attach_pool(self.actor, C.addressof(self._pool_desc)), "a0_actor_attach_pool")
            self._pool_whole = 0
        self.stage = None
        if self.lp:
            sg = tr.stage
            sd = _RbufDesc(int(sg.size), int(sg.obs_bytes), min(self.B, int(sg.size)), 0, float(rc.alpha), float(rc.eps), float(rc.beta0), int(cfg.trainer.total_steps), int(cfg.seed) + 7)
            self._stage_pstate = ops.zeros(1)
            self.stage = C.c_void_p()
            ok(lib.a0_rbuf_create_on(C.addressof(sd), p(sg.frames), p(sg.act), p(sg.rew), p(sg.done), None, p(self._stage_pstate), C.addressof(self.stage)), "a0_rbuf_create_on (stage)")
            self._lp_pending = None
        lp = C.c_void_p()
        ok(lib.a0_learner_loss_buffer(self.learner, C.addressof(lp)), "a0_learner_loss_buffer")
        self.loss_ptr = lp
        self._qs, self._rs, self._nret = (C.c_float * self.T)(), (C.c_float * (self.T * self.E))(), C.c_int()
        self._pending_rollout = False
        self.fqf = lc.algo.name == "fqf"
        self._floss = ops.empty(self.B) if self.fqf else None
        self.frames_ptr = p(rp.frames)
        self.row_bytes = int(rp.row_bytes)

    def _rollout(self, st):
        tr, lib = self.tr, self.lib
        pool = self.pool
        if pool is not None:
            self.ok(lib.a0_actor_pool_seq(self.actor, None, None, C.c_longlong(pool.seq)), "a0_actor_pool_seq")
        self.ok(lib.a0_actor_rollout(self.actor, self.learner, self.rbuf, C.c_float(tr.epsilon_fn(tr.frame_count)), st), "a0_actor_rollout")
        if pool is not None:
            self._sync_pool()

    def _sync_pool(self):
        pool, actor = self.pool, self.tr.actors[1]
        seq, whole = C.c_longlong(), C.c_longlong()
        self.ok(self.lib.a0_actor_pool_seq(self.actor, C.byref(seq), C.byref(whole), C.c_longlong(-1)), "a0_actor_pool_seq")
        pool.g += seq.value - pool.seq
        pool.seq = seq.value
        pool.full_uploads += whole.value - self._pool_whole
        self._pool_whole = whole.value
        actor.obs = pool._obs[pool.seq & 1]

    def _commit(self, st):
        tr, rp = self.tr, self.tr.replay
        n = self.T * self.E
        self.ok(self.lib.a0_rbuf_commit(self.rbuf, n, st), "a0_rbuf_commit")
        tr.frame_count += n
# ... 206 lines not shown
```

agent0_amd/ops.py:

```python
from __future__ import annotations

import ctypes as C
from typing import Optional

import torch

from . import _abi
from ._abi import A0Error, EncoderPass, EncoderWeights, FramesArg, LearnerDesc, NetDesc, check


def _stream() -> int:
    return torch._C._cuda_getCurrentRawStream(torch._C._cuda_getDevice())


def _req(t: Optional[torch.Tensor], dtype, min_numel: int, name: str, optional: bool = False):
    if t is None:
        if optional:
            return None
        raise A0Error(f"{name}: tensor required")
    if not t.is_cuda:
        raise A0Error(f"{name}: expected a HIP device tensor (got {t.device}); agent0_amd has no CPU path")
    if t.dtype != dtype:
        raise A0Error(f"{name}: expected {dtype}, got {t.dtype}")
    if not t.is_contiguous():
# ... 259 lines not shown

    def update_tail(self, params, grads, m, v, n, state, scalars, b1, b2, eps, target, n_total, plan, w, C_, wt, wt_target, loss=None, loss_n=0, loss_ring=None):
        ew = self._enc_w(w)
        nw = self.conv_wt_floats(C_)
        check(self.lib.a0_update_tail(_req(params, torch.float32, n_total, "params"), _req(grads, torch.float32, n_total, "grads"), _req(m, torch.float32, n, "m"),
                                      _req(v, torch.float32, n, "v"), n, _req(state, torch.int32, 8, "state"), _req(scalars, torch.float32, 2, "scalars"),
                                      b1, b2, eps, _req(target, torch.float32, n_total, "target"), n_total, C.addressof(plan), C.addressof(ew), C_,
                                      _req(wt, torch.float32, nw, "wt"), _req(wt_target, torch.float32, nw, "wt_target"),
                                      _req(loss, torch.float32, max(loss_n, 1), "loss", optional=True), int(loss_n), _req(loss_ring, torch.float32, 1, "loss_ring", optional=True),
                                      0 if loss_ring is None else int(loss_ring.numel()), _stream()), "a0_update_tail")

    def dense_fwd_scratch(self, R, N, K) -> int:
        return int(self.lib.a0_dense_fwd_scratch(R, N, K))

    def dense_wgrad_scratch(self, R, N, K) -> int:
        return int(self.lib.a0_dense_wgrad_scratch(R, N, K))

    def dense_fwd(self, X, ldx, W, b, Y, R, N, K, relu, scratch):
        need = self.dense_fwd_scratch(R, N, K)
        check(self.lib.a0_dense_fwd(_req(X, torch.float32, (R - 1) * ldx + K, "X"), ldx, _req(W, torch.float32, N * K, "W"), _req(b, torch.float32, N, "b"),
                                    _req(Y, torch.float32, R * N, "Y"), R, N, K, int(relu),
                                    _req(scratch, torch.float32, need, "scratch", optional=(need == 0)), _stream()), "a0_dense_fwd")

    def dense_fwd_splits(self, R, N, K) -> int:
        return int(self.lib.a0_dense_fwd_splits(R, N, K))

    def dense_fwd_n(self, X, ldx, W, b, Y, R, N, K, relu, splits, scratch):
        need = splits * R * N if splits > 1 else 0
        check(self.lib.a0_dense_fwd_n(_req(X, torch.float32, (R - 1) * ldx + K, "X"), ldx, _req(W, torch.float32, N * K, "W"), _req(b, torch.float32, N, "b"),
                                      _req(Y, torch.float32, R * N, "Y"), R, N, K, int(relu), int(splits),
                                      _req(scratch, torch.float32, need, "scratch", optional=(need == 0)), _stream()), "a0_dense_fwd_n")

    def dense_dgrad_hadamard_ok(self, R, N, K, n) -> bool:
        return bool(self.lib.a0_dense_dgrad_hadamard_ok(R, N, K, n))

    def dense_dgrad_hadamard(self, dY, W, emb, feat, demb, d3, R, N, K, n):
        check(self.lib.a0_dense_dgrad_hadamard(_req(dY, torch.float32, R * N, "dY"), _req(W, torch.float32, N * K, "W"), _req(emb, torch.float32, R * K, "emb"),
                                               _req(feat, torch.float32, (R // n) * K, "feat"), _req(demb, torch.float32, R * K, "demb"), _req(d3, torch.float32, (R // n) * K, "d3"),
                                               R, N, K, n, _stream()), "a0_dense_dgrad_hadamard")

    def weight_planes_words(self, N, K) -> int:
        return int(self.lib.a0_weight_planes_words(N, K))

    def split_planes(self, W, planes, N, K):
        check(self.lib.a0_split_planes(_req(W, torch.float32, N * K, "W"), _req(planes, torch.int32, self.weight_planes_words(N, K), "planes"), N, K, _stream()), "a0_split_planes")

    def dense_fwd_wplanes_ok(self, R, N, K) -> bool:
        return bool(self.lib.a0_dense_fwd_wplanes_ok(R, N, K))

    def dense_fwd_wplanes(self, X, ldx, planes, b, Y, R, N, K, relu):
        check(self.lib.a0_dense_fwd_wplanes(_req(X, torch.float32, (R - 1) * ldx + K, "X"), ldx, _req(planes, torch.int32, self.weight_planes_words(N, K), "planes"),
                                            _req(b, torch.float32, N, "b"), _req(Y, torch.float32, R * N, "Y"), R, N, K, int(relu), _stream()), "a0_dense_fwd_wplanes")

    def dense_fwd_mul(self, X, ldx, W, b, M, group, Y, R, N, K, relu):
        check(self.lib.a0_dense_fwd_mul(_req(X, torch.float32, (R - 1) * ldx + K, "X"), ldx, _req(W, torch.float32, N * K, "W"), _req(b, torch.float32, N, "b"),
                                        _req(M, torch.float32, ((R - 1) // group + 1) * N, "M"), group, _req(Y, torch.float32, R * N, "Y"), R, N, K, int(relu), _stream()),
              "a0_dense_fwd_mul")

    def dense_fwd_mul_keep_ok(self, R, N, K, ldx) -> bool:
        return bool(self.lib.a0_dense_fwd_mul_keep_ok(R, N, K, ldx))

    def dense_fwd_mul_keep(self, X, ldx, W, b, M, group, E, Y, R, N, K, relu):
        check(self.lib.a0_dense_fwd_mul_keep(_req(X, torch.float32, (R - 1) * ldx + K, "X"), ldx, _req(W, torch.float32, N * K, "W"), _req(b, torch.float32, N, "b"),
                                             _req(M, torch.float32, ((R - 1) // group + 1) * N, "M"), group, _req(E, torch.float32, R * N, "E"),
                                             _req(Y, torch.float32, R * N, "Y"), R, N, K, int(relu), _stream()), "a0_dense_fwd_mul_keep")

    def dense_dgrad(self, dY, W, mask, dX, R, N, K):
        check(self.lib.a0_dense_dgrad(_req(dY, torch.float32, R * N, "dY"), _req(W, torch.float32, N * K, "W"),
                                      _req(mask, torch.float32, R * K, "mask", optional=True), _req(dX, torch.float32, R * K, "dX"), R, N, K, _stream()), "a0_dense_dgrad")

    def dense_wgrad(self, dY, X, ldx, grad, R, N, K, slabs):
        need = self.dense_wgrad_scratch(R, N, K)
        check(self.lib.a0_dense_wgrad(_req(dY, torch.float32, R * N, "dY"), _req(X, torch.float32, (R - 1) * ldx + K, "X"), ldx,
                                      _req(grad, torch.float32, N * K + N, "grad"), R, N, K,
                                      _req(slabs, torch.float32, need, "slabs", optional=(need == 0)), _stream()), "a0_dense_wgrad")

    def dueling_fwd(self, raw, ld, q, R, A, T, dueling):
        check(self.lib.a0_dueling_fwd(_req(raw, torch.float32, R * ld, "raw"), ld, _req(q, torch.float32, R * A * T, "q"), R, A, T, int(dueling), _stream()), "a0_dueling_fwd")

    def dueling_bwd(self, dq, draw, ld, R, A, T, dueling):
        check(self.lib.a0_dueling_bwd(_req(dq, torch.float32, R * A * T, "dq"), _req(draw, torch.float32, R * ld, "draw"), ld, R, A, T, int(dueling), _stream()), "a0_dueling_bwd")

    def select_action(self, x, sb, sa, st, B, A, T, mode, aux, a_star, qsel, qmax):
        span = (B - 1) * sb + (A - 1) * sa + (T - 1) * st + 1
        check(self.lib.a0_select_action(_req(x, torch.float32, span, "x"), sb, sa, st, B, A, T, mode,
                                        _req(aux, torch.float32, T if mode == 2 else (B * (T + 1) if mode == 3 else 0), "aux", optional=mode < 2),
                                        _req(a_star, torch.int32, B, "a_star", optional=True), _req(qsel, torch.float32, B * A, "qsel", optional=True),
                                        _req(qmax, torch.float32, B, "qmax", optional=True), _stream()), "a0_select_action")

    def loss_dqn(self, q, q_next, A, act, a_star, rew, done, wgt, gamma_n, B, loss, dq, state):
        check(self.lib.a0_loss_dqn(_req(q, torch.float32, B * A, "q"), _req(q_next, torch.float32, B * A, "q_next"), A, _req(act, torch.int32, B, "act"),
                                   _req(a_star, torch.int32, B, "a_star"), _req(rew, torch.float32, B, "rew"), _req(done, torch.float32, B, "done"),
                                   _req(wgt, torch.float32, B, "wgt"), gamma_n, B, _req(loss, torch.float32, B, "loss"), _req(dq, torch.float32, B * A, "dq"),
                                   _req(state, torch.int32, 8, "state"), _stream()), "a0_loss_dqn")

    def loss_mdqn(self, q, q_next, q_cur_tgt, A, act, rew, done, wgt, gamma_n, tau, lo, B, loss, dq, state):
        check(self.lib.a0_loss_mdqn(_req(q, torch.float32, B * A, "q"), _req(q_next, torch.float32, B * A, "q_next"), _req(q_cur_tgt, torch.float32, B * A, "q_cur_tgt"), A,
                                    _req(act, torch.int32, B, "act"), _req(rew, torch.float32, B, "rew"), _req(done, torch.float32, B, "done"),
                                    _req(wgt, torch.float32, B, "wgt"), gamma_n, tau, lo, B, _req(loss, torch.float32, B, "loss"), _req(dq, torch.float32, B * A, "dq"),
                                    _req(state, torch.int32, 8, "state"), _stream()), "a0_loss_mdqn")

    def loss_c51(self, logits, tgt_logits, A, T, act, a_star, rew, done, wgt, atoms, gamma_n, vmin, vmax, B, loss, dlogits, m_out, state):
        check(self.lib.a0_loss_c51(_req(logits, torch.float32, B * A * T, "logits"), _req(tgt_logits, torch.float32, B * A * T, "tgt_logits"), A, T,
                                   _req(act, torch.int32, B, "act"), _req(a_star, torch.int32, B, "a_star"), _req(rew, torch.float32, B, "rew"),
                                   _req(done, torch.float32, B, "done"), _req(wgt, torch.float32, B, "wgt"), _req(atoms, torch.float32, T, "atoms"),
                                   gamma_n, vmin, vmax, B, _req(loss, torch.float32, B, "loss"), _req(dlogits, torch.float32, B * A * T, "dlogits"),
# ... 315 lines not shown
    def actor_quantile_tail_env_step(self, slabs, nslab, bias, ld, A, T, dueling, mode, taus, E, seed, stream_a, stream_u, off_a, off_u, eps, action, qmax, ctrl, eps_ptr,
                                     env_seed, rank, g, obs_in, obs_out, ep_ret, final_mask, final_ret, n, steps, gamma, ring_act, ring_rew, ring_done, obs0, frames, cap,
                                     start_slot, r_act, r_rew, r_done, task=0):
        nb = E * 4 * 84 * 84
        check(self.lib.a0_actor_quantile_tail_env_step(
            _req(slabs, torch.float32, nslab * E * T * ld, "slabs"), E * T * ld, nslab, _req(bias, torch.float32, A + (1 if dueling else 0), "bias"), ld, A, T, int(dueling),
            mode, _req(taus, torch.float32, E * (T + 1), "taus", optional=(mode != 3)), E, seed, stream_a, stream_u, off_a, off_u, float(eps),
            _req(ctrl, torch.int64, 8, "ctrl", optional=True), _eps_req(eps, eps_ptr, E),
            _req(action, torch.int32, E, "action"), _req(qmax, torch.float32, E, "qmax"),
            env_seed, rank, g, _req(obs_in, torch.uint8, nb, "obs_in"), _req(obs_out, torch.uint8, nb, "obs_out"), _req(ep_ret, torch.float32, E, "ep_ret"),
            _req(final_mask, torch.float32, E, "final_mask"), _req(final_ret, torch.float32, E, "final_ret"), n, steps, float(gamma),
            _req(ring_act, torch.int32, n * E, "ring_act"), _req(ring_rew, torch.float32, n * E, "ring_rew"), _req(ring_done, torch.float32, n * E, "ring_done"),
            _req(obs0, torch.uint8, nb, "obs0"), _req(frames, torch.uint8, cap * 8 * 84 * 84, "frames"), cap, start_slot, _req(r_act, torch.int32, cap, "r_act"),
            _req(r_rew, torch.float32, cap, "r_rew"), _req(r_done, torch.float32, cap, "r_done"), int(task), _stream()), "a0_actor_quantile_tail_env_step")

    def actor_quantile_tail_env_step_enc(self, slabs, nslab, bias, ld, A, T, dueling, mode, taus, E, seed, stream_a, stream_u, off_a, off_u, eps, action, qmax, ctrl, eps_ptr,
                                         env_seed, rank, g, obs_in, obs_out, ep_ret, final_mask, final_ret, n, steps, gamma, ring_act, ring_rew, ring_done, obs0, frames, cap,
                                         start_slot, r_act, r_rew, r_done, task=0, wt=None, enc_w=None, act3_next=None):
        nb = E * 4 * 84 * 84
        ew = self._enc_w(enc_w)
        check(self.lib.a0_actor_quantile_tail_env_step_enc(
            _req(slabs, torch.float32, nslab * E * T * ld, "slabs"), E * T * ld, nslab, _req(bias, torch.float32, A + (1 if dueling else 0), "bias"), ld, A, T, int(dueling),
            mode, _req(taus, torch.float32, E * (T + 1), "taus", optional=(mode != 3)), E, seed, stream_a, stream_u, off_a, off_u, float(eps),
            _req(ctrl, torch.int64, 8, "ctrl", optional=True), _eps_req(eps, eps_ptr, E),
            _req(action, torch.int32, E, "action"), _req(qmax, torch.float32, E, "qmax"),
            env_seed, rank, g, _req(obs_in, torch.uint8, nb, "obs_in"), _req(obs_out, torch.uint8, nb, "obs_out"), _req(ep_ret, torch.float32, E, "ep_ret"),
            _req(final_mask, torch.float32, E, "final_mask"), _req(final_ret, torch.float32, E, "final_ret"), n, steps, float(gamma),
            _req(ring_act, torch.int32, n * E, "ring_act"), _req(ring_rew, torch.float32, n * E, "ring_rew"), _req(ring_done, torch.float32, n * E, "ring_done"),
            _req(obs0, torch.uint8, nb, "obs0"), _req(frames, torch.uint8, cap * 8 * 84 * 84, "frames"), cap, start_slot, _req(r_act, torch.int32, cap, "r_act"),
            _req(r_rew, torch.float32, cap, "r_rew"), _req(r_done, torch.float32, cap, "r_done"), int(task),
            _req(wt, torch.float32, self.conv_wt_floats(4), "wt"), C.addressof(ew), _req(act3_next, torch.float32, E * 3136, "act3_next"), _stream()), "a0_actor_quantile_tail_env_step_enc")

    def actor_qhead_scratch(self, E, K) -> int:
        return int(self.lib.a0_actor_qhead_scratch(E, K))

    def actor_qhead(self, feat, E, K, W1, b1, W2, b2, A, dueling, scratch, seed, stream_a, stream_u, off_a, off_u, eps, action, qmax, ctrl=None, eps_ptr=None):
        nq = A + (1 if dueling else 0)
        check(self.lib.a0_actor_qhead(_req(feat, torch.float32, E * K, "feat"), E, K, _req(W1, torch.float32, 512 * K, "W1"), _req(b1, torch.float32, 512, "b1"),
                                      _req(W2, torch.float32, nq * 512, "W2"), _req(b2, torch.float32, nq, "b2"), A, int(dueling),
                                      _req(scratch, torch.float32, self.actor_qhead_scratch(E, K), "scratch"), seed, stream_a, stream_u, off_a, off_u, float(eps),
                                      _req(ctrl, torch.int64, 8, "ctrl", optional=True), _eps_req(eps, eps_ptr, E),
                                      _req(action, torch.int32, E, "action"), _req(qmax, torch.float32, E, "qmax"), _stream()), "a0_actor_qhead")

    def actor_qhead_n(self, feat, E, K, splits, W1, b1, W2, b2, A, dueling, scratch, seed, stream_a, stream_u, off_a, off_u, eps, action, qmax, ctrl=None, eps_ptr=None):
        nq = A + (1 if dueling else 0)
        check(self.lib.a0_actor_qhead_n(_req(feat, torch.float32, E * K, "feat"), E, K, int(splits), _req(W1, torch.float32, 512 * K, "W1"), _req(b1, torch.float32, 512, "b1"),
                                        _req(W2, torch.float32, nq * 512, "W2"), _req(b2, torch.float32, nq, "b2"), A, int(dueling),
                                        _req(scratch, torch.float32, splits * E * 512, "scratch"), seed, stream_a, stream_u, off_a, off_u, float(eps),
                                        _req(ctrl, torch.int64, 8, "ctrl", optional=True), _eps_req(eps, eps_ptr, E),
                                        _req(action, torch.int32, E, "action"), _req(qmax, torch.float32, E, "qmax"), _stream()), "a0_actor_qhead_n")

    def actor_qhead_env_step(self, feat, E, K, W1, b1, W2, b2, A, dueling, scratch, seed, stream_a, stream_u, off_a, off_u, eps, action, qmax, ctrl, eps_ptr,
                             env_seed, rank, g, obs_in, obs_out, ep_ret, final_mask, final_ret, n, steps, gamma, ring_act, ring_rew, ring_done, obs0, frames, cap,
                             start_slot, r_act, r_rew, r_done, task=0):
        nq = A + (1 if dueling else 0)
        nb = E * 4 * 84 * 84
        check(self.lib.a0_actor_qhead_env_step(
            _req(feat, torch.float32, E * K, "feat"), E, K, _req(W1, torch.float32, 512 * K, "W1"), _req(b1, torch.float32, 512, "b1"),
            _req(W2, torch.float32, nq * 512, "W2"), _req(b2, torch.float32, nq, "b2"), A, int(dueling),
            _req(scratch, torch.float32, self.actor_qhead_scratch(E, K), "scratch"), seed, stream_a, stream_u, off_a, off_u, float(eps),
            _req(ctrl, torch.int64, 8, "ctrl", optional=True), _eps_req(eps, eps_ptr, E),
            _req(action, torch.int32, E, "action"), _req(qmax, torch.float32, E, "qmax"),
            env_seed, rank, g, _req(obs_in, torch.uint8, nb, "obs_in"), _req(obs_out, torch.uint8, nb, "obs_out"), _req(ep_ret, torch.float32, E, "ep_ret"),
            _req(final_mask, torch.float32, E, "final_mask"), _req(final_ret, torch.float32, E, "final_ret"), n, steps, float(gamma),
            _req(ring_act, torch.int32, n * E, "ring_act"), _req(ring_rew, torch.float32, n * E, "ring_rew"), _req(ring_done, torch.float32, n * E, "ring_done"),
            _req(obs0, torch.uint8, nb, "obs0"), _req(frames, torch.uint8, cap * 8 * 84 * 84, "frames"), cap, start_slot, _req(r_act, torch.int32, cap, "r_act"),
            _req(r_rew, torch.float32, cap, "r_rew"), _req(r_done, torch.float32, cap, "r_done"), int(task), _stream()), "a0_actor_qhead_env_step")

    def actor_qhead_env_step_enc(self, feat, E, K, W1, b1, W2, b2, A, dueling, scratch, seed, stream_a, stream_u, off_a, off_u, eps, action, qmax, ctrl, eps_ptr,
                                 env_seed, rank, g, obs_in, obs_out, ep_ret, final_mask, final_ret, n, steps, gamma, ring_act, ring_rew, ring_done, obs0, frames, cap,
                                 start_slot, r_act, r_rew, r_done, task=0, wt=None, enc_w=None, act3_next=None):
        nq = A + (1 if dueling else 0)
        nb = E * 4 * 84 * 84
        ew = self._enc_w(enc_w)
        check(self.lib.a0_actor_qhead_env_step_enc(
            _req(feat, torch.float32, E * K, "feat"), E, K, _req(W1, torch.float32, 512 * K, "W1"), _req(b1, torch.float32, 512, "b1"),
            _req(W2, torch.float32, nq * 512, "W2"), _req(b2, torch.float32, nq, "b2"), A, int(dueling),
            _req(scratch, torch.float32, self.actor_qhead_scratch(E, K), "scratch"), seed, stream_a, stream_u, off_a, off_u, float(eps),
            _req(ctrl, torch.int64, 8, "ctrl", optional=True), _eps_req(eps, eps_ptr, E),
            _req(action, torch.int32, E, "action"), _req(qmax, torch.float32, E, "qmax"),
            env_seed, rank, g, _req(obs_in, torch.uint8, nb, "obs_in"), _req(obs_out, torch.uint8, nb, "obs_out"), _req(ep_ret, torch.float32, E, "ep_ret"),
            _req(final_mask, torch.float32, E, "final_mask"), _req(final_ret, torch.float32, E, "final_ret"), n, steps, float(gamma),
            _req(ring_act, torch.int32, n * E, "ring_act"), _req(ring_rew, torch.float32, n * E, "ring_rew"), _req(ring_done, torch.float32, n * E, "ring_done"),
            _req(obs0, torch.uint8, nb, "obs0"), _req(frames, torch.uint8, cap * 8 * 84 * 84, "frames"), cap, start_slot, _req(r_act, torch.int32, cap, "r_act"),
            _req(r_rew, torch.float32, cap, "r_rew"), _req(r_done, torch.float32, cap, "r_done"), int(task),
            _req(wt, torch.float32, self.conv_wt_floats(4), "wt"), C.addressof(ew), _req(act3_next, torch.float32, E * K, "act3_next"), _stream()), "a0_actor_qhead_env_step_enc")

    def mean_rows(self, x, T, E, out):
        check(self.lib.a0_mean_rows(_req(x, torch.float32, T * E, "x"), T, E, _req(out, torch.float32, T, "out"), _stream()), "a0_mean_rows")

    def fill_f32(self, p, n, v):
        check(self.lib.a0_fill_f32(_req(p, torch.float32, n, "p"), n, v, _stream()), "a0_fill_f32")

    def priority_update(self, priority, ids, loss, B, eps, alpha, pstate, state):
        check(self.lib.a0_priority_update(_req(priority, torch.float32, 1, "priority"), _req(ids, torch.int64, B, "ids"), _req(loss, torch.float32, B, "loss"), B,
                                          eps, alpha, _req(pstate, torch.float32, 1, "pstate"), _req(state, torch.int32, 8, "state", optional=True), _stream()), "a0_priority_update")

    def priority_tail(self, priority, size, n, pstate, alpha):
        check(self.lib.a0_priority_tail(_req(priority, torch.float32, size, "priority"), size, n, _req(pstate, torch.float32, 1, "pstate"), alpha, _stream()), "a0_priority_tail")

    def sum_f32(self, x, n, scratch256, out):
        check(self.lib.a0_sum_f32(_req(x, torch.float32, n, "x"), n, _req(scratch256, torch.float32, 256, "scratch256"), _req(out, torch.float32, 1, "out"), _stream()), "a0_sum_f32")

    def is_weights(self, prio, B, psum, top, beta, w):
        check(self.lib.a0_is_weights(_req(prio, torch.float32, B, "prio"), B, _req(psum, torch.float32, 1, "psum"), top, beta, _req(w, torch.float32, B, "w"), _stream()), "a0_is_weights")

    def perm_batch(self, start, count, n, seed, out):
        check(self.lib.a0_perm_batch(start, count, n, seed & 0xFFFFFFFF, _req(out, torch.int64, count, "out"), _stream()), "a0_perm_batch")

    def sumtree_set(self, tree, cap2, idx, val, n, state=None):
        check(self.lib.a0_sumtree_set(_req(tree, torch.float32, 2 * cap2, "tree"), cap2, _req(idx, torch.int64, n, "idx"), _req(val, torch.float32, n, "val"), n,
                                      _req(state, torch.int32, 8, "state", optional=True), _stream()), "a0_sumtree_set")

    def sumtree_sample_batch(self, seed, stream, offset, tree, cap2, B, top, cap, beta, r_act, r_rew, r_done, idx_out, slot_out, act, rew, done, prio, w, rebuild_top=False):
        check(self.lib.a0_sumtree_sample_batch(seed, stream, offset, _req(tree, torch.float32, 2 * cap2, "tree"), cap2, B, top, cap, float(beta),
                                               _req(r_act, torch.int32, cap, "r_act"), _req(r_rew, torch.float32, cap, "r_rew"), _req(r_done, torch.float32, cap, "r_done"),
                                               _req(idx_out, torch.int64, B, "idx_out"), _req(slot_out, torch.int32, B, "slot_out"), _req(act, torch.int32, B, "act"),
                                               _req(rew, torch.float32, B, "rew"), _req(done, torch.float32, B, "done"), _req(prio, torch.float32, B, "prio"),
                                               _req(w, torch.float32, B, "w"), 1 if rebuild_top else 0, _stream()), "a0_sumtree_sample_batch")

    def sumtree_set_range(self, tree, cap2, start, n, size, val):
        check(self.lib.a0_sumtree_set_range(_req(tree, torch.float32, 2 * cap2, "tree"), cap2, start, n, size, _req(val, torch.float32, 1, "val"), _stream()),
              "a0_sumtree_set_range")

    def sumtree_rebuild(self, tree, cap2):
        check(self.lib.a0_sumtree_rebuild(_req(tree, torch.float32, 2 * cap2, "tree"), cap2, _stream()), "a0_sumtree_rebuild")

    def sumtree_sample(self, tree, cap2, xi, B, out_idx, out_p):
        check(self.lib.a0_sumtree_sample(_req(tree, torch.float32, 2 * cap2, "tree"), cap2, _req(xi, torch.float32, B, "xi"), B,
                                         _req(out_idx, torch.int64, B, "out_idx"), _req(out_p, torch.float32, B, "out_p"), _stream()), "a0_sumtree_sample")

    def sumtree_set_from_loss_ok(self, cap2) -> bool:
        return bool(self.lib.a0_sumtree_set_from_loss_ok(cap2))

    def sumtree_top_rebuild(self, tree, cap2):
        check(self.lib.a0_sumtree_top_rebuild(_req(tree, torch.float32, 2 * cap2, "tree"), cap2, _stream()), "a0_sumtree_top_rebuild")

    def snapshot_pack_bound(self, rows, frames_per_row, frame_bytes) -> int:
        n = int(self.lib.a0_snapshot_pack_bound(rows, frames_per_row, frame_bytes))
# ... 213 lines not shown
```

include/agent0_hip.h:

```cpp
#ifndef AGENT0_HIP_H
#define AGENT0_HIP_H

#include <stdint.h>

#ifdef __cplusplus
extern "C" {
#endif

#define A0_ABI_VERSION 1

#define A0_CTRL_ENV_STEP 0
#define A0_CTRL_ACTOR_STEPS 1
#define A0_CTRL_RNG_ACTION 2
#define A0_CTRL_RNG_UNIFORM 3
#define A0_CTRL_REPLAY_SLOT 4
#define A0_CTRL_RNG_TAUS 5
#define A0_CTRL_RNG_NOISE 6
#define A0_CTRL_WORDS 8

const char* a0_last_error(void);
int a0_abi_version(void);
const char* a0_build_info(void);
int a0_device_info(int* cu_count, long long* hbm_bytes, char* arch_name64);

// ... 49 lines not shown
int a0_net_encoder_wgrad(const a0_net* net, const a0_encoder_weights* w, const a0_frames_arg* frames, int B, const float* act1, const float* act2,
                         const float* d3, const float* d2, const float* d1, float* g1, float* g2, float* g3, float* slabs, const a0_pending_reduce* pend,
                         void* stream);

typedef struct a0_update_tail_plan { a0_reduce_seg seg[8]; int n; } a0_update_tail_plan;
int a0_net_encoder_wgrad_tail(const a0_net* net, const a0_encoder_weights* w, const a0_frames_arg* frames, int B, const float* act1, const float* act2,
                              const float* d3, const float* d2, const float* d1, float* g1, float* g2, float* g3, float* slabs, const a0_pending_reduce* pend,
                              a0_update_tail_plan* plan, int* state, float* scalars2, double lr, double beta1, double beta2, int target_update_freq, void* stream);

long long a0_dense_fwd_scratch(int R, int N, int K);
int a0_dense_fwd(const float* X, int ldx, const float* W, const float* b, float* Y, int R, int N, int K, int relu,
                 float* scratch, void* stream);
int a0_dense_fwd_splits(int R, int N, int K);
int a0_dense_fwd_n(const float* X, int ldx, const float* W, const float* b, float* Y, int R, int N, int K, int relu, int splits, float* scratch, void* stream);
int a0_dense_dgrad(const float* dY, const float* W, const float* act_mask, float* dX, int R, int N, int K, void* stream);
int a0_dense_dgrad_wgrad_ok(int R, int N, int K);
int a0_dense_dgrad_wgrad_ok2(int R, int N, int K);
int a0_dense_dgrad_wgrad(const float* dY, const float* W, const float* X, int ldx, float* dX, float* grad_w_b, int R, int N, int K, void* stream);
int a0_dense_dgrad_wgrad2_ok(int R, int N, int K, int N2, int K2);
int a0_dense_dgrad_wgrad2(const float* dY, const float* W, const float* X, int ldx, float* dX, float* grad, int R, int N, int K,
                          const float* dY2, const float* X2, int ldx2, float* grad2, int N2, int K2, void* stream);
long long a0_dense_wgrad_scratch(int R, int N, int K);
int a0_dense_wgrad(const float* dY, const float* X, int ldx, float* grad_w_b, int R, int N, int K, float* slabs, void* stream);
int a0_dense_wgrad_multi(int n, const float* const* dY, const float* const* X, const int* ldx, float* const* grad_w_b, const int* R, const int* N, const int* K,
                         float* slabs, const long long* slab_off, a0_pending_reduce* pend, void* stream);

int a0_dense_fwd_mul(const float* X, int ldx, const float* W, const float* b, const float* M, int group, float* Y, int R, int N, int K, int relu, void* stream);

int a0_dense_fwd_mul_keep_ok(int R, int N, int K, int ldx);
int a0_dense_fwd_mul_keep(const float* X, int ldx, const float* W, const float* b, const float* M, int group, float* E, float* Y, int R, int N, int K, int relu, void* stream);

int a0_dense_fwd_partial_slabs(int R, int N, int K);
int a0_dense_fwd_partial(const float* X, int ldx, const float* W, int R, int N, int K, float* slabs, void* stream);
int a0_dense_fwd_partial_n(const float* X, int ldx, const float* W, int R, int N, int K, int splits, float* slabs, void* stream);
int a0_dense_fwd_partial_multi_ok(int n, int R, int N, int K);
int a0_dense_fwd_partial_multi_slabs(int n, int R, int N, int K);
int a0_dense_fwd_partial_multi(int n, const float* const* X, int ldx, const float* const* W, int R, int N, int K, float* const* slabs, const long long* slab_stride,
                               void* stream);
int a0_reduce_bias_act_multi(int n, const float* const* slabs, const long long* slab_stride, const int* nslab, const float* const* bias, float* const* out,
                             const int* rows, int N, int relu, void* stream);

int a0_probe_begin(int tag, int max_launches);
int a0_probe_end(double* host_out3);

int a0_trace_enabled(void);
int a0_trace_rank(int rank);
int a0_trace_push(const char* name);
int a0_trace_pop(void);

long long a0_weight_planes_words(int N, int K);
int a0_split_planes(const float* W, unsigned int* planes, int N, int K, void* stream);
int a0_dense_fwd_wplanes_ok(int R, int N, int K);
int a0_dense_fwd_wplanes(const float* X, int ldx, const unsigned int* Wplanes, const float* b, float* Y, int R, int N, int K, int relu, void* stream);

int a0_gemm_mode(int mode);

int a0_x9_products(int n);

int a0_dueling_fwd(const float* raw, int ld, float* q, int R, int A, int T, int dueling, void* stream);
int a0_dueling_bwd(const float* dq, float* draw, int ld, int R, int A, int T, int dueling, void* stream);

int a0_select_action(const float* x, long long sb, long long sa, long long st, int B, int A, int T, int mode,
                     const float* aux, int* a_star, float* qsel, float* qmax, void* stream);
int a0_actor_dist_tail(const float* slabs, long long slab_stride, int nslab, const float* bias, int ld, int A, int T, int dueling, int mode,
                       const float* atoms, int E, unsigned long long seed, unsigned int stream_a, unsigned int stream_u, unsigned long long off_a,
                       unsigned long long off_u, float eps, const long long* ctrl, const float* eps_ptr, int* action, float* qmax, void* stream);
int a0_actor_quantile_tail(const float* slabs, long long slab_stride, int nslab, const float* bias, int ld, int A, int T, int dueling, int mode,
                           const float* taus, int E, unsigned long long seed, unsigned int stream_a, unsigned int stream_u, unsigned long long off_a,
                           unsigned long long off_u, float eps, const long long* ctrl, const float* eps_ptr, int* action, float* qmax, void* stream);
int a0_actor_dist_tail_env_step(const float* slabs, long long slab_stride, int nslab, const float* bias, int ld, int A, int T, int dueling, int mode,
                                const float* atoms, int E, unsigned long long seed, unsigned int stream_a, unsigned int stream_u, unsigned long long off_a,
                                unsigned long long off_u, float eps, const long long* ctrl, const float* eps_ptr, int* action, float* qmax,
                                unsigned long long env_seed, unsigned int rank, unsigned int g, const uint8_t* obs_in, uint8_t* obs_out, float* ep_ret,
                                float* final_mask, float* final_ret, int n, long long steps, double gamma, int* ring_act, float* ring_rew, float* ring_done,
                                const uint8_t* obs0, uint8_t* frames, long long cap, long long start_slot, int* r_act, float* r_rew, float* r_done, int task, void* stream);

int a0_actor_quantile_tail_env_step(const float* slabs, long long slab_stride, int nslab, const float* bias, int ld, int A, int T, int dueling, int mode,
                                    const float* taus, int E, unsigned long long seed, unsigned int stream_a, unsigned int stream_u, unsigned long long off_a,
                                    unsigned long long off_u, float eps, const long long* ctrl, const float* eps_ptr, int* action, float* qmax,
                                    unsigned long long env_seed, unsigned int rank, unsigned int g, const uint8_t* obs_in, uint8_t* obs_out, float* ep_ret,
                                    float* final_mask, float* final_ret, int n, long long steps, double gamma, int* ring_act, float* ring_rew, float* ring_done,
                                    const uint8_t* obs0, uint8_t* frames, long long cap, long long start_slot, int* r_act, float* r_rew, float* r_done, int task, void* stream);

int a0_loss_dqn(const float* q, const float* q_next, int A, const int* act, const int* a_star, const float* rew,
                const float* done, const float* wgt, float gamma_n, int B, float* loss, float* dq, int* nan_flag, void* stream);
int a0_dqn_head_loss(const float* h_on, const float* h_tg, const float* h_sel, const float* W_on, const float* b_on, const float* W_tg,
                     const float* b_tg, int A, int dueling, int ld, const int* act, const float* rew, const float* done, const float* wgt,
                     float gamma_n, int B, float* loss, float* q_on_out, float* q_tg_out, float* draw, int* nan_flag, void* stream);
int a0_dqn_head_loss_slabs(const float* slabs_on, const float* slabs_tg, const float* slabs_sel, long long slab_stride, int nslab, const float* b1_on,
                           const float* b1_tg, float* h_on_out, const float* W_on, const float* b_on, const float* W_tg, const float* b_tg, int A,
                           int dueling, int ld, const int* act, const float* rew, const float* done, const float* wgt, float gamma_n, int B, float* loss,
                           float* q_on_out, float* q_tg_out, float* draw, int* nan_flag, float* dh_out, void* stream);

int a0_loss_mdqn(const float* q, const float* q_next, const float* q_cur_tgt, int A, const int* act, const float* rew, const float* done,
                 const float* wgt, float gamma_n, float tau, float lo, int B, float* loss, float* dq, int* nan_flag, void* stream);
int a0_mdqn_head_loss_slabs(const float* slabs_on, const float* slabs_tg, const float* slabs_cur, long long slab_stride, int nslab, const float* b1_on,
                            const float* b1_tg, float* h_on_out, const float* W_on, const float* b_on, const float* W_tg, const float* b_tg, int A,
                            int dueling, int ld, const int* act, const float* rew, const float* done, const float* wgt, float gamma_n, float tau, float lo,
                            int B, float* loss, float* q_on_out, float* q_tg_out, float* q_cur_out, float* draw, int* nan_flag, float* dh_out, void* stream);
int a0_c51_head_loss_slabs(const float* slabs_on, long long stride_on, int nslab_on, int rows_on, const float* slabs_tg, long long stride_tg, int nslab_tg,
                           int sel_off, const float* bias_on, const float* bias_tg, int ld, int A, int T, int dueling, const int* act, const float* rew,
                           const float* done, const float* wgt, const float* atoms, float gamma_n, float vmin, float vmax, int B, float* loss, float* draw,
                           float* q_on_out, float* q_tg_out, float* m_out, int* a_star_out, int* nan_flag, void* stream);
int a0_qr_head_loss_slabs(const float* slabs_on, long long stride_on, int nslab_on, int rows_on, const float* slabs_tg, long long stride_tg, int nslab_tg,
                          int sel_off, const float* bias_on, const float* bias_tg, int ld, int A, int T, int dueling, const int* act, const float* rew,
                          const float* done, const float* wgt, const float* taus, float gamma_n, int B, float* loss, float* draw, float* q_on_out,
// ... 76 lines not shown
int a0_learner_create_on(const a0_learner_desc* desc, const a0_learner_buffers* buffers, a0_learner** out);
int a0_learner_set_rng(a0_learner* learner, int stream_id, unsigned long long offset);
int a0_learner_rng_state(a0_learner* learner, unsigned long long* words, int set);
int a0_learner_destroy(a0_learner* learner);
long long a0_learner_param_floats(const a0_learner* learner);
int a0_learner_set_exchange(a0_learner* learner, long long comm);
int a0_learner_set_grad_clip(a0_learner* learner, double max_norm, float* norm_ring_dev, int ring_cap);
int a0_learner_set_target_tau(a0_learner* learner, double tau);
int a0_learner_set_params(a0_learner* learner, const float* online_packed, const float* target_packed, void* stream);
int a0_learner_get(const a0_learner* learner, float* online_out, float* target_out, float* adam_m_out, float* adam_v_out, int* state_out8, void* stream);
int a0_learner_loss_buffer(const a0_learner* learner, float** loss_dev);
enum { A0_PEEK_GRADS = 0, A0_PEEK_ACT1 = 1, A0_PEEK_ACT2 = 2, A0_PEEK_ACT3 = 3, A0_PEEK_FC1 = 4, A0_PEEK_LOSS = 5, A0_PEEK_GRAD_NORM_RING = 6  };
int a0_learner_peek(const a0_learner* learner, int what, float** dev_ptr, long long* count);
int a0_learner_get_frac_loss(const a0_learner* learner, float* out_dev, void* stream);
int a0_learner_set_support(a0_learner* learner, const float* atoms_host);
int a0_learner_update(a0_learner* learner, const uint8_t* frames, const int* slot, long long row_bytes, const int* act, const float* rew, const float* done,
                      const float* wgt, float* loss_out, void* stream);

typedef struct a0_rbuf a0_rbuf;
typedef struct a0_rbuf_desc {
    long long size; int obs_bytes, B, prioritize;
    double alpha, eps, beta0; long long total_steps;
    unsigned long long seed;
} a0_rbuf_desc;
typedef struct a0_batch { const long long* idx; const int* slot; const int* act; const float* rew; const float* done; const float* prio; const float* weights; } a0_batch;
int a0_rbuf_create(const a0_rbuf_desc* desc, a0_rbuf** out);
int a0_rbuf_create_on(const a0_rbuf_desc* desc, uint8_t* frames, int* act, float* rew, float* done, float* tree, float* max_p, a0_rbuf** out);
int a0_rbuf_destroy(a0_rbuf* replay);
long long a0_rbuf_len(const a0_rbuf* replay);
long long a0_rbuf_write_cursor(const a0_rbuf* replay);
int a0_rbuf_info(const a0_rbuf* replay, long long* top, long long* written, double* beta);
int a0_rbuf_buffers(a0_rbuf* replay, uint8_t** frames, int** act, float** rew, float** done, float** tree, float** max_p);
int a0_rbuf_read(const a0_rbuf* replay, long long rows, uint8_t* frames_out, int* act_out, float* rew_out, float* done_out, float* tree_out, float* max_p_out, void* stream);
int a0_rbuf_commit(a0_rbuf* replay, long long n, void* stream);
int a0_rbuf_extend_from(a0_rbuf* replay, const a0_rbuf* stage, long long start_row, long long n, void* stream);
int a0_rbuf_sample(a0_rbuf* replay, a0_batch* out, void* stream);
int a0_rbuf_sample_block(a0_rbuf* replay, int n, a0_batch* out, void* stream);
int a0_rbuf_update_priority(a0_rbuf* replay, const float* loss, const int* learner_state, void* stream);

typedef struct a0_actor a0_actor;
typedef struct a0_actor_desc {
    int E, T, A, dueling, n_step;
    double discount;
    unsigned long long seed; unsigned int rank;
    int env_task;
    int reset_noise_freq;
} a0_actor_desc;
int a0_actor_create(const a0_actor_desc* desc, a0_actor** out);
int a0_actor_destroy(a0_actor* actor);
int a0_actor_bind(a0_actor* actor, const a0_learner* learner, int own_network);
int a0_actor_snapshot(a0_actor* actor, const a0_learner* learner, void* stream);
int a0_actor_rollout(a0_actor* actor, a0_learner* learner, a0_rbuf* replay, float epsilon, void* stream);
int a0_actor_set_eps_ladder(a0_actor* actor, float alpha, long long i0, long long n_total);
int a0_actor_collect(a0_actor* actor, float* qs_host, float* returns_host, int max_returns, int* n_returns, void* stream);
typedef struct a0_env_pool_desc {
    int E, nstack, W, use_life_loss;
    long long frame_bytes;
    void* new_host[2]; void* scal_host[2]; void* obs_host[2];
    void* act_dev; void* ctl_dev;
    long long* done_host;
    void* obs_dev[2]; void* scal_dev[2]; void* new_dev;
    long long step_word, seq_mask;
    long long seq;
    double timeout_s;
} a0_env_pool_desc;
int a0_actor_attach_pool(a0_actor* actor, const a0_env_pool_desc* desc);
int a0_actor_detach_pool(a0_actor* actor);
int a0_actor_pool_seq(a0_actor* actor, long long* seq_out, long long* whole_out, long long set_seq);
int a0_actor_collect_begin(a0_actor* actor, void* stream);
int a0_actor_collect_end(a0_actor* actor, float* qs_host, float* returns_host, int max_returns, int* n_returns);

long long a0_rbuf_state_size(const a0_rbuf* replay);
int a0_rbuf_state_save(a0_rbuf* replay, void* blob_host, long long capacity, void* stream);
int a0_rbuf_state_load(a0_rbuf* replay, const void* blob_host, long long bytes, void* stream);
long long a0_actor_state_size(const a0_actor* actor);
int a0_actor_state_save(a0_actor* actor, void* blob_host, long long capacity, void* stream);
int a0_actor_state_load(a0_actor* actor, const void* blob_host, long long bytes, void* stream);
long long a0_snapshot_pack_bound(long long rows, int frames_per_row, int frame_bytes);
long long a0_snapshot_literal_offset(long long rows, int frames_per_row);
int a0_snapshot_pack(const uint8_t* rows, long long n_rows, int frames_per_row, int frame_bytes, long long stride, uint8_t* packed, unsigned int* work, void* stream);
int a0_snapshot_unpack(const uint8_t* packed, long long n_rows, int frames_per_row, int frame_bytes, uint8_t* rows_out, int* bad_flag, void* stream);

int a0_nan_flag_export(const int* state, float* out, void* stream);
int a0_rmsprop_step(float* params, const float* grads, float* square_avg, long long n, double lr, double alpha, double eps,
                    double max_grad_norm, float* clip_scratch, void* stream);
int a0_target_sync(float* target, const float* online, long long n, const int* state, int force, void* stream);
int a0_noisy_compose(const float* mu, const float* sigma, float* eff, int N, int K, int r0, int r1, const float* noise_in,
                     const float* noise_out_w, const float* noise_out_b, void* stream);
int a0_noisy_grad_sigma(const float* gmu, float* gsigma, int N, int K, int r0, int r1, const float* noise_in,
                        const float* noise_out_w, const float* noise_out_b, void* stream);
int a0_noisy_multi(int grad, int nmod, const float* const* mu, const float* const* sigma, float* const* eff, const int* N, const int* K, const int* r0,
                   const int* r1, const float* const* noise_in, const float* const* noise_out_w, const float* const* noise_out_b, void* stream);

int a0_replay_insert(uint8_t* frames, long long cap, int obs_bytes, long long start_slot, int n, const uint8_t* obs,
                     const uint8_t* obs_next, const int* act, const float* rew, const float* done, int* r_act,
                     float* r_rew, float* r_done, const long long* ctrl, void* stream);
int a0_replay_lookup(const long long* idx, int B, long long top, long long head, long long cap, int* slot, const int* r_act,
                     const float* r_rew, const float* r_done, const float* priority, int* act, float* rew, float* done,
                     float* prio, long long* idx_out, void* stream);
int a0_replay_gather(const uint8_t* frames, int row_bytes, const int* slot, int B, uint8_t* out, void* stream);
int a0_replay_sample_gather(int mode, unsigned long long start, unsigned long long n_perm, unsigned int seed, const float* tree, long long cap2,
                            const float* xi, long long top, long long head, long long cap, const uint8_t* frames, int row_bytes, const int* r_act,
                            const float* r_rew, const float* r_done, const float* priority, int B, uint8_t* out, long long* idx_out, int* slot_out,
                            int* act, float* rew, float* done, float* prio, void* stream);
int a0_replay_sample_slots(unsigned long long start, unsigned long long n_perm, unsigned int seed, long long top, long long head, long long cap,
                           const int* r_act, const float* r_rew, const float* r_done, const float* priority, int B, long long* idx_out, int* slot_out,
                           int* act, float* rew, float* done, float* prio, void* stream);
int a0_replay_sample_slots_multi(int n, const unsigned long long* start, const unsigned long long* n_perm, const unsigned int* seed, long long top, long long head, long long cap,
                                 const int* r_act, const float* r_rew, const float* r_done, int B, long long* idx_out, int* slot_out, int* act, float* rew, float* done,
                                 float* prio, void* stream);
int a0_fill_f32(float* p, long long n, float v, void* stream);
int a0_priority_update(float* priority, const long long* ids, const float* loss, int B, float eps, float alpha,
                       float* pstate, const int* state, void* stream);
int a0_priority_tail(float* priority, long long size, long long n, const float* pstate, float alpha, void* stream);
int a0_sum_f32(const float* x, long long n, float* scratch256, float* out, void* stream);
int a0_is_weights(const float* prio, int B, const float* psum, long long top, float beta, float* w, void* stream);
int a0_perm_batch(unsigned long long start, int count, unsigned long long n, unsigned int seed, long long* out, void* stream);
int a0_sumtree_set(float* tree, long long cap2, const long long* idx, const float* val, int n, const int* state, void* stream);
int a0_sumtree_set_range(float* tree, long long cap2, long long start, long long n, long long size, const float* val, void* stream);
int a0_sumtree_rebuild(float* tree, long long cap2, void* stream);
int a0_sumtree_sample(const float* tree, long long cap2, const float* xi, int B, long long* out_idx, float* out_p, void* stream);
int a0_sumtree_sample_batch(unsigned long long seed, unsigned int stream, unsigned long long offset, float* tree, long long cap2, int B, long long top,
                            long long cap, float beta, const int* r_act, const float* r_rew, const float* r_done, long long* idx_out, int* slot_out,
                            int* act, float* rew, float* done, float* prio, float* w, int rebuild_top, void* stream_h);
int a0_priority_from_loss(const float* loss, int n, float eps, float alpha, float* val, float* pstate, const int* state, void* stream);
int a0_sumtree_set_from_loss_ok(long long cap2);
int a0_sumtree_set_from_loss(float* tree, long long cap2, const long long* idx, const float* loss, int n, float eps, float alpha, float* pstate, const int* state,
                             int defer_top, void* stream);
int a0_sumtree_top_rebuild(float* tree, long long cap2, void* stream);

#define A0_EPS_PER_ENV (-1.0f)
int a0_eps_ladder(float eps, const float* eps_ptr, float alpha, int E, long long i0, long long n_total, float* eps_vec, void* stream);
int a0_actor_egreedy(const int* greedy, const int* rand_action, const float* u, float eps, int E, int* action,
                     const float* qmax, float* qs_out, void* stream);
long long a0_actor_qhead_scratch(int E, int K);
int a0_actor_qhead(const float* feat, int E, int K, const float* W1, const float* b1, const float* W2, const float* b2, int A, int dueling,
                   float* scratch, unsigned long long seed, unsigned int stream_a, unsigned int stream_u, unsigned long long off_a,
                   unsigned long long off_u, float eps, const long long* ctrl, const float* eps_ptr, int* action, float* qmax, void* stream);
int a0_actor_qhead_n(const float* feat, int E, int K, int splits, const float* W1, const float* b1, const float* W2, const float* b2, int A, int dueling,
                     float* scratch, unsigned long long seed, unsigned int stream_a, unsigned int stream_u, unsigned long long off_a,
                     unsigned long long off_u, float eps, const long long* ctrl, const float* eps_ptr, int* action, float* qmax, void* stream);
int a0_actor_qhead_env_step(const float* feat, int E, int K, const float* W1, const float* b1, const float* W2, const float* b2, int A, int dueling,
                            float* scratch, unsigned long long seed, unsigned int stream_a, unsigned int stream_u, unsigned long long off_a,
                            unsigned long long off_u, float eps, const long long* ctrl, const float* eps_ptr, int* action, float* qmax,
                            unsigned long long env_seed, unsigned int rank, unsigned int g, const uint8_t* obs_in, uint8_t* obs_out, float* ep_ret,
                            float* final_mask, float* final_ret, int n, long long steps, double gamma, int* ring_act, float* ring_rew, float* ring_done,
                            const uint8_t* obs0, uint8_t* frames, long long cap, long long start_slot, int* r_act, float* r_rew, float* r_done, int task, void* stream);
int a0_mean_rows(const float* x, int T, int E, float* out, void* stream);

int a0_actor_qhead_env_step_enc(const float* feat, int E, int K, const float* W1, const float* b1, const float* W2, const float* b2, int A, int dueling,
                                float* scratch, unsigned long long seed, unsigned int stream_a, unsigned int stream_u, unsigned long long off_a,
                                unsigned long long off_u, float eps, const long long* ctrl, const float* eps_ptr, int* action, float* qmax,
                                unsigned long long env_seed, unsigned int rank, unsigned int g, const uint8_t* obs_in, uint8_t* obs_out, float* ep_ret,
                                float* final_mask, float* final_ret, int n, long long steps, double gamma, int* ring_act, float* ring_rew, float* ring_done,
                                const uint8_t* obs0, uint8_t* frames, long long cap, long long start_slot, int* r_act, float* r_rew, float* r_done, int task,
                                const float* wt, const a0_encoder_weights* w, float* act3_next, void* stream);
int a0_actor_dist_tail_env_step_enc(const float* slabs, long long slab_stride, int nslab, const float* bias, int ld, int A, int T, int dueling, int mode,
                                    const float* atoms, int E, unsigned long long seed, unsigned int stream_a, unsigned int stream_u, unsigned long long off_a,
                                    unsigned long long off_u, float eps, const long long* ctrl, const float* eps_ptr, int* action, float* qmax,
                                    unsigned long long env_seed, unsigned int rank, unsigned int g, const uint8_t* obs_in, uint8_t* obs_out, float* ep_ret,
                                    float* final_mask, float* final_ret, int n, long long steps, double gamma, int* ring_act, float* ring_rew, float* ring_done,
                                    const uint8_t* obs0, uint8_t* frames, long long cap, long long start_slot, int* r_act, float* r_rew, float* r_done, int task,
                                    const float* wt, const a0_encoder_weights* w, float* act3_next, void* stream);
int a0_actor_quantile_tail_env_step_enc(const float* slabs, long long slab_stride, int nslab, const float* bias, int ld, int A, int T, int dueling, int mode,
                                        const float* taus, int E, unsigned long long seed, unsigned int stream_a, unsigned int stream_u, unsigned long long off_a,
                                        unsigned long long off_u, float eps, const long long* ctrl, const float* eps_ptr, int* action, float* qmax,
                                        unsigned long long env_seed, unsigned int rank, unsigned int g, const uint8_t* obs_in, uint8_t* obs_out, float* ep_ret,
                                        float* final_mask, float* final_ret, int n, long long steps, double gamma, int* ring_act, float* ring_rew, float* ring_done,
                                        const uint8_t* obs0, uint8_t* frames, long long cap, long long start_slot, int* r_act, float* r_rew, float* r_done, int task,
                                        const float* wt, const a0_encoder_weights* w, float* act3_next, void* stream);
int a0_actor_egreedy_rng(const int* greedy, unsigned long long seed, unsigned int stream_a, unsigned int stream_u, unsigned long long off_a,
                         unsigned long long off_u, int A, float eps, int E, int* action, const float* qmax, float* qs_out,
                         const long long* ctrl, const float* eps_ptr, void* stream);
int a0_actor_nstep(int E, int n, long long steps, double gamma, const int* action, const float* reward, const float* terminal,
                   const float* truncated, const float* life_loss, int* ring_act, float* ring_rew, float* ring_done,
                   int* out_act, float* out_rew, float* out_done, const long long* ctrl, void* stream);

int a0_env_frame_stack(const uint8_t* prev, const uint8_t* newest, const float* advance, uint8_t* out, int E, int nstack, long long frame_bytes,
                       void* stream);

int a0_host_device_pointer(void* host, void** dev);
int a0_env_pool_upload(const uint8_t* new_host, uint8_t* new_dev, const float* scal_host, float* scal_dev, int n_scal, int advance_row,
                       const uint8_t* obs_host, const uint8_t* prev, uint8_t* out, int E, int nstack, long long frame_bytes, int* n_whole,
                       void* stream);
int a0_env_pool_send(const int* action, int* act_host_dev, int E, long long* ctl_host_dev, long long word, void* stream);
int a0_host_step_ingest(const uint8_t* prev, const uint8_t* newest, const float* scal, uint8_t* out, int E, int nstack, long long frame_bytes,
                        int use_life_loss, const int* action, int n, int ring_len, long long steps, double gamma, int* ring_act, float* ring_rew,
                        float* ring_done, uint8_t* ring_obs, uint8_t* frames, long long cap, long long start_slot, int* r_act, float* r_rew,
                        float* r_done, float* stat_mask, float* stat_ret, const long long* ctrl, void* stream);

int a0_rng_u32(unsigned long long seed, unsigned int stream_id, unsigned long long offset, unsigned int* out, long long n, void* stream);
int a0_rng_uniform(unsigned long long seed, unsigned int stream_id, unsigned long long offset, float* out, long long n, void* stream);
int a0_rng_randint(unsigned long long seed, unsigned int stream_id, unsigned long long offset, int hi, int* out, long long n, void* stream);
int a0_rng_normal(unsigned long long seed, unsigned int stream_id, unsigned long long offset, float stdv, float* out, long long n, void* stream);
int a0_rng_uniform_ctrl(unsigned long long seed, unsigned int stream_id, unsigned long long offset, float* out, long long n, const long long* ctrl,
                        int ctrl_idx, void* stream);
int a0_rng_normal_ctrl(unsigned long long seed, unsigned int stream_id, unsigned long long offset, float stdv, float* out, long long n,
                       const long long* ctrl, int ctrl_idx, void* stream);
#define A0_ENV_TASK_STREAM 0
#define A0_ENV_TASK_BLOCK 1
#define A0_ENV_TASK_CHASE 2
int a0_env_synth_reset(unsigned long long seed, unsigned int rank, int E, uint8_t* obs, float* ep_ret, void* stream);
int a0_env_synth_reset_task(unsigned long long seed, unsigned int rank, int E, uint8_t* obs, float* ep_ret, int task, void* stream);
int a0_env_synth_step(unsigned long long seed, unsigned int rank, int E, unsigned int g, const uint8_t* obs_in, uint8_t* obs_out,
                      float* ep_ret, float* reward, float* terminal, float* truncated, float* life_loss, float* final_mask,
                      float* final_ret, const int* action, int A, int task, const long long* ctrl, void* stream);
int a0_env_synth_step_commit(unsigned long long seed, unsigned int rank, int E, unsigned int g, const uint8_t* obs_in, uint8_t* obs_out, float* ep_ret,
                             float* final_mask, float* final_ret, int n, long long steps, double gamma, const int* action, int* ring_act,
                             float* ring_rew, float* ring_done, const uint8_t* obs0, uint8_t* frames, long long cap, long long start_slot, int* r_act,
// ... 13 lines not shown
```

Baseline: 2.335 million.

## Add pre-split bf16 weight planes for actor fc1 with ring-prefetched MFMA kernel

Adds a dedicated actor fc1 kernel that reads W1 as pre-split hi/mid/lo bf16 planes, laid out per MFMA fragment, instead of splitting the fp32 weights into planes inside the GEMM each step. Weight tiles are prefetched through a four-deep register ring while activations are staged through double-buffered LDS. The qhead env-step entry points gain an optional w1_planes argument and fall back to the old path when it is absent. The planes must be regenerated whenever W1 changes, and whether they are used by default depends on whether the actor wiring passes them, which is not fully visible here.

After: 2.383 million, median of 6. +2.1%, better.

```diff
diff --git a/agent0_amd/common/atari_wrappers.py b/agent0_amd/common/atari_wrappers.py
--- a/agent0_amd/common/atari_wrappers.py
+++ b/agent0_amd/common/atari_wrappers.py
@@ -80,16 +80,17 @@
         self._cur = nxt
         return self._obs[nxt]
 
-    def act_step_commit(self, tail_args, final_mask, final_ret, n, steps, gamma, ring_act, ring_rew, ring_done, obs0, replay, start_slot, kind: str = "qhead", enc=None):
+    def act_step_commit(self, tail_args, final_mask, final_ret, n, steps, gamma, ring_act, ring_rew, ring_done, obs0, replay, start_slot, kind: str = "qhead", enc=None, w1_planes=None):
         self.g += 1
         nxt = (self._cur + 1) % len(self._obs)
         common = (self.seed, self.rank, self.g, self._obs[self._cur], self._obs[nxt], self.ep_ret, final_mask, final_ret, n, steps, gamma, ring_act, ring_rew, ring_done, obs0,
                   replay.frames, replay.size, start_slot, replay.act, replay.rew, replay.done)
+        extra = {"w1_planes": w1_planes} if (kind == "qhead" and w1_planes is not None) else {}
         if enc is not None:
             {"qhead": self.ops.actor_qhead_env_step_enc, "dist": self.ops.actor_dist_tail_env_step_enc, "quantile": self.ops.actor_quantile_tail_env_step_enc}[kind](
-                *tail_args, *common, task=self.task, wt=enc[0], enc_w=enc[1], act3_next=enc[2])
+                *tail_args, *common, task=self.task, wt=enc[0], enc_w=enc[1], act3_next=enc[2], **extra)
         else:
-            {"qhead": self.ops.actor_qhead_env_step, "dist": self.ops.actor_dist_tail_env_step, "quantile": self.ops.actor_quantile_tail_env_step}[kind](*tail_args, *common, task=self.task)
+            {"qhead": self.ops.actor_qhead_env_step, "dist": self.ops.actor_dist_tail_env_step, "quantile": self.ops.actor_quantile_tail_env_step}[kind](*tail_args, *common, task=self.task, **extra)
         self._cur = nxt
         return self._obs[nxt]
 
diff --git a/agent0_amd/csrc/actor_fc1.hip b/agent0_amd/csrc/actor_fc1.hip
--- /dev/null
+++ b/agent0_amd/csrc/actor_fc1.hip
@@ -0,0 +1,169 @@
+#include "igemm_x9.h"
+#include "a0_internal.h"
+#include "net_impl.h"
+
+constexpr int A0_FC1_RING = 4;
+
+__global__ __launch_bounds__(256) void a0_actor_fc1_kernel(const float* __restrict__ X, int ldx, const uint4* __restrict__ Wp, float* __restrict__ slabs, int R, int N, int K,
+                                                           int kchunk, int gx, int gy) {
+    typedef a0_x9_stager<OpMatKC, 64, 256, 2> SA;
+    constexpr int APL = SA::IM::PLANE, ABYTES = 3 * APL, D = A0_FC1_RING;
+    static_assert(SA::R == 2 && (D % 2) == 0, "two feature pieces per thread and tile");
+    __shared__ __attribute__((aligned(16))) char As[2 * ABYTES];
+
+    const int tid = threadIdx.x, lane = tid & 63, wave = __builtin_amdgcn_readfirstlane(tid >> 6);
+    const int wm = wave >> 1, wn = wave & 1;
+    int bx, by, bz;
+    {
+        const int n = gridDim.x, id = blockIdx.x, per = n >> 3;
+        const int L = (id < (per << 3)) ? (id & 7) * per + (id >> 3) : id;
+        if (gy <= gx) { by = L % gy; const int t = L / gy; bx = t % gx; bz = t / gx; }
+        else          { bx = L % gx; const int t = L / gx; by = t % gy; bz = t / gy; }
+    }
+    const int x0 = bx * 64, y0 = by * 64;
+    const int kb = bz * kchunk;
+    const int ke = (K < kb + kchunk) ? K : (kb + kchunk);
+    const int nt = ke > kb ? (ke - kb) >> 5 : 0;
+    float* const out = slabs + (long long)bz * R * N + (y0 + wn * 32 + (lane & 31));
+    if (nt < 1) {
+#pragma unroll
+        for (int r = 0; r < 16; ++r) {
+            const int x = x0 + wm * 32 + (r & 3) + 8 * (r >> 2) + 4 * (lane >> 5);
+            if (x < R) out[(long long)x * N] = 0.f;
+        }
+        return;
+    }
+
+    const a0_mat_src pa{X, ldx};
+    SA sa;
+    sa.init(pa, x0, R, kb, ke, tid);
+
+    const int T = K >> 5, t0 = kb >> 5;
+    const uint4* const wbase = Wp + (long long)((y0 >> 5) + wn) * (K >> 4) * (3 * 64) + lane;
+    a0_u32x4g ring[D][6];
+    auto fill = [&](int slot, int tile) {
+        const int tt = tile < T ? tile : T - 1;
+        const a0_u32x4g* p = (const a0_u32x4g*)(wbase + (long long)tt * (6 * 64));
+#pragma unroll
+        for (int i = 0; i < 6; ++i) ring[slot][i] = p[i * 64];
+    };
+
+    a0_acc16 acc;
+#pragma unroll
+    for (int r = 0; r < 16; ++r) acc[r] = 0.f;
+
+    typename SA::Slot s0, s1;
+    s0.okmask = s1.okmask = 0u;
+#pragma unroll
+    for (int p = 0; p < 2; ++p) sa.template fetch_piece<true>(pa, s0, p, kb, ke, tid);
+#pragma unroll
+    for (int p = 0; p < 2; ++p) sa.template fetch_piece<true>(pa, s1, p, kb + 32, ke, tid);
+#pragma unroll
+    for (int d = 0; d < D; ++d) fill(d, t0 + d);
+
+    a0_x9_piece pc;
+    a0_f4 unused = a0_zero4();
+    auto micro = [&](int u, typename SA::Slot& s, char* a_dst, int k_fetch) {
+        const int p = u / 6, st = u % 6;
+        if (st == 0) pc.v = sa.template value<false, true>(s, p, unused);
+        else if (st <= 4) pc.split(st - 1);
+        else { sa.store(pc, p, a_dst, tid); sa.template fetch_piece<true>(pa, s, p, k_fetch, ke, tid); }
+    };
+    const int abase = SA::frag_base(lane, wm * 32);
+
+    auto mma_tile = [&](int buf, typename SA::Slot& s, const a0_u32x4g (&b)[6], int k_fetch) {
+        const char* ap = As + buf * ABYTES;
+        char* a_dst = As + (buf ^ 1) * ABYTES;
+        a0_u32x4g a[2][3];
+#pragma unroll
+        for (int ks = 0; ks < 2; ++ks)
+#pragma unroll
+            for (int t = 2; t >= 0; --t) a[ks][t] = SA::frag(ap + t * APL, abase, 0, ks);
+        __builtin_amdgcn_sched_barrier(0);
+#pragma unroll
+        for (int n = 0; n < 12; ++n) {
+            constexpr int TA[6] = {2, 1, 0, 1, 0, 0};
+            constexpr int TB[6] = {0, 1, 2, 0, 1, 0};
+            const int ks = n / 6, q = n % 6;
+            acc = __builtin_amdgcn_mfma_f32_32x32x16_bf16(__builtin_bit_cast(a0_bf16x8g, a[ks][TA[q]]), __builtin_bit_cast(a0_bf16x8g, b[ks * 3 + TB[q]]), acc, 0, 0, 0);
+            micro(n, s, a_dst, k_fetch);
+            __builtin_amdgcn_sched_barrier(0);
+        }
+    };
+
+#pragma unroll
+    for (int u = 0; u < 12; ++u) micro(u, s0, As, kb + 64);
+    __syncthreads();
+    int tb = 0;
+#pragma unroll 1
+    for (; tb + D <= nt; tb += D) {
+#pragma unroll
+        for (int u = 0; u < D; ++u) {
+            mma_tile(u & 1, (u & 1) ? s0 : s1, ring[u], kb + 32 * (tb + u + 3));
+            fill(u, t0 + tb + u + D);
+            __builtin_amdgcn_sched_barrier(0);
+            __syncthreads();
+        }
+    }
+#pragma unroll
+    for (int u = 0; u < D - 1; ++u) {
+        if (tb + u < nt) {
+            mma_tile(u & 1, (u & 1) ? s0 : s1, ring[u], kb + 32 * (tb + u + 3));
+            __syncthreads();
+        }
+    }
+
+#pragma unroll
+    for (int r = 0; r < 16; ++r) {
+        const int x = x0 + wm * 32 + (r & 3) + 8 * (r >> 2) + 4 * (lane >> 5);
+        if (x < R) out[(long long)x * N] = acc[r];
+    }
+}
+
+__global__ __launch_bounds__(256) void a0_actor_fc1_planes_kernel(const float* __restrict__ W, uint4* __restrict__ planes, int K, long long count) {
+    const long long i = (long long)blockIdx.x * blockDim.x + threadIdx.x;
+    if (i >= count) return;
+    const int lane = (int)(i & 63), K16 = K >> 4;
+    const long long g = i >> 6;
+    const int nb = (int)(g / K16), ks = (int)(g - (long long)nb * K16);
+    const a0_f4* src = (const a0_f4*)(W + (long long)(nb * 32 + (lane & 31)) * K + ks * 16 + 8 * (lane >> 5));
+    a0_u32x2g hi[2], mid[2], lo[2];
+#pragma unroll
+    for (int h = 0; h < 2; ++h) {
+        a0_x9_piece pc;
+        pc.v = src[h];
+#pragma unroll
+        for (int e = 0; e < 4; ++e) pc.split(e);
+        pc.pack(hi[h], mid[h], lo[h]);
+    }
+    uint4* o = planes + g * (3 * 64) + lane;
+    o[0] = uint4{hi[0].x, hi[0].y, hi[1].x, hi[1].y};
+    o[64] = uint4{mid[0].x, mid[0].y, mid[1].x, mid[1].y};
+    o[128] = uint4{lo[0].x, lo[0].y, lo[1].x, lo[1].y};
+}
+
+extern "C" long long a0_actor_fc1_planes_words(int N, int K) { return (N < 1 || K < 1) ? 0 : (long long)N * (K / 8) * 12; }
+
+extern "C" int a0_actor_fc1_planes(const float* W, unsigned int* planes, int N, int K, void* stream) {
+    if (!W || !planes || N < 32 || (N & 31) || K < 16 || (K & 15) || ((((uintptr_t)W) | ((uintptr_t)planes)) & 15))
+        return a0_fail(A0_EINVAL, "a0_actor_fc1_planes: bad argument (N a multiple of 32, K a multiple of 16, 16-byte aligned buffers)");
+    const long long count = (long long)(N / 32) * (K / 16) * 64;
+    hipLaunchKernelGGL(a0_actor_fc1_planes_kernel, dim3((unsigned)((count + 255) / 256)), dim3(256), 0, (hipStream_t)stream, W, (uint4*)planes, K, count);
+    return a0_fail_hip((int)hipGetLastError(), "a0_actor_fc1_planes");
+}
+
+extern "C" int a0_actor_fc1_ok(int R, int N, int K) {
+    return (R >= 1 && R <= 256 && N == 512 && K >= 32 && !(K & 31) && a0_gemm_mode(-1) != 0 && a0_x9_products_now() == 6) ? 1 : 0;
+}
+
+extern "C" int a0_actor_fc1_n(const float* X, int ldx, const unsigned int* planes, int R, int N, int K, int splits, float* slabs, void* stream) {
+    if (!X || !planes || !slabs || (ldx & 3) || ldx < K || !a0_actor_fc1_ok(R, N, K) || ((((uintptr_t)X) | ((uintptr_t)planes)) & 15))
+        return a0_fail(A0_EINVAL, "a0_actor_fc1_n: shapes a0_actor_fc1_ok accepts (16-byte aligned rows)");
+    if (splits < 1 || splits > 64 || splits > (K + 31) / 32) return a0_fail(A0_EINVAL, "a0_actor_fc1_n: splits must lie in [1, min(64, ceil(K / 32))]");
+    const int ktiles = K / 32;
+    const int kchunk = ((ktiles + splits - 1) / splits) * 32;
+    const int gx = (R + 63) / 64, gy = N / 64;
+    A0_LAUNCH_PROBED(A0_TAG_DENSE_FWD, 2.0 * (double)R * (double)N * (double)K, a0_actor_fc1_kernel, dim3((unsigned)(gx * gy * splits)), dim3(256), 0, (hipStream_t)stream, X, ldx,
+                     (const uint4*)planes, slabs, R, N, K, kchunk, gx, gy);
+    return a0_fail_hip((int)hipGetLastError(), "a0_actor_fc1_n");
+}
diff --git a/agent0_amd/csrc/net.hip b/agent0_amd/csrc/net.hip
--- a/agent0_amd/csrc/net.hip
+++ b/agent0_amd/csrc/net.hip
@@ -570,6 +570,31 @@
     a0_actor_qhead_env_body(P, raw, w2s, &s_chase_cell);
 }
 
+extern "C" int a0_actor_fc1_dense_ok(int R, int N, int K) {
+    return (a0_actor_fc1_ok(R, N, K) && a0_fwd_splits((R + 127) / 128, (N + 63) / 64, K) > 1) ? 1 : 0;
+}
+extern "C" int a0_actor_fc1_dense(const float* X, int ldx, const unsigned int* planes, const float* b, float* Y, int R, int N, int K, int relu, float* scratch, void* stream) {
+    A0_TRY
+    if (!b || !Y || !scratch || !a0_actor_fc1_dense_ok(R, N, K)) return a0_fail(A0_EINVAL, "a0_actor_fc1_dense: shapes a0_actor_fc1_dense_ok accepts");
+    const int splits = a0_fwd_splits((R + 127) / 128, (N + 63) / 64, K);
+    const int rc = a0_actor_fc1_n(X, ldx, planes, R, N, K, splits, scratch, stream);
+    if (rc != A0_OK) return rc;
+    a0_hip_backend bk{(hipStream_t)stream};
+    bk.reduce_bias_act(scratch, (long long)R * N, splits, b, Y, R, N, relu);
+    return A0_OK;
+    A0_CATCH
+}
+
+static int a0_actor_fc1_slabs(a0_hip_backend& bk, const float* feat, int K, const float* W1, const unsigned int* w1_planes, int E, int splits, float* scratch) {
+    if (w1_planes && a0_actor_fc1_ok(E, 512, K)) return a0_actor_fc1_n(feat, K, w1_planes, E, 512, K, splits, scratch, (void*)bk.st);
+    a0_mat_src a{feat, K};
+    a0_mat_src bw{W1, K};
+    EpiSlab::Params ep{scratch, (long long)E * 512, 512};
+    bk.tag = A0_TAG_DENSE_FWD;
+    a0_fc1_partial_launch(bk, a, bw, ep, E, 512, K, splits);
+    return A0_OK;
+}
+
 extern "C" long long a0_actor_qhead_scratch(int E, int K) {
     const int splits = a0_fc1_splits(E, 512, K);
     return (long long)splits * E * 512;
@@ -602,12 +627,12 @@
                             qmax, stream);
 }
 
-extern "C" int a0_actor_qhead_env_step(const float* feat, int E, int K, const float* W1, const float* b1, const float* W2, const float* b2, int A, int dueling,
+extern "C" int a0_actor_qhead_env_step_wp(const float* feat, int E, int K, const float* W1, const float* b1, const float* W2, const float* b2, int A, int dueling,
                                        float* scratch, unsigned long long seed, unsigned int stream_a, unsigned int stream_u, unsigned long long off_a,
                                        unsigned long long off_u, float eps, const long long* ctrl, const float* eps_ptr, int* action, float* qmax,
                                        unsigned long long env_seed, unsigned int rank, unsigned int g, const uint8_t* obs_in, uint8_t* obs_out, float* ep_ret,
                                        float* final_mask, float* final_ret, int n, long long steps, double gamma, int* ring_act, float* ring_rew, float* ring_done,
-                                       const uint8_t* obs0, uint8_t* frames, long long cap, long long start_slot, int* r_act, float* r_rew, float* r_done, int task, void* stream) {
+                                       const uint8_t* obs0, uint8_t* frames, long long cap, long long start_slot, int* r_act, float* r_rew, float* r_done, int task, const unsigned int* w1_planes, void* stream) {
     A0_TRY
     if (!feat || !W1 || !b1 || !W2 || !b2 || !scratch || !action || !qmax || E < 1 || K < 4 || (K & 3) || A < 1 || A + (dueling ? 1 : 0) > 24)
         return a0_fail(A0_EINVAL, "a0_actor_qhead_env_step: bad argument (A + dueling <= 24: the head rows are staged in 48 KB of LDS)");
@@ -617,11 +642,7 @@
     if ((((uintptr_t)obs_in) | ((uintptr_t)obs_out) | ((uintptr_t)obs0) | ((uintptr_t)frames)) & 15) return a0_fail(A0_EINVAL, "a0_actor_qhead_env_step: buffers must be 16-byte aligned");
     a0_hip_backend bk{(hipStream_t)stream};
     const int splits = a0_fc1_splits(E, 512, K);
-    a0_mat_src a{feat, K};
-    a0_mat_src bw{W1, K};
-    EpiSlab::Params ep{scratch, (long long)E * 512, 512};
-    bk.tag = A0_TAG_DENSE_FWD;
-    a0_fc1_partial_launch(bk, a, bw, ep, E, 512, K, splits);
+    { const int rc = a0_actor_fc1_slabs(bk, feat, K, W1, w1_planes, E, splits, scratch); if (rc != A0_OK) return rc; }
     a0_qenv_args P;
     P.slabs = scratch; P.slab_stride = (long long)E * 512; P.nslab = splits; P.b1 = b1; P.W2 = W2; P.b2 = b2; P.A = A; P.dueling = dueling; P.E = E;
     P.rng_seed = seed; P.stream_a = stream_a; P.stream_u = stream_u; P.off_a = off_a; P.off_u = off_u; P.eps = eps; P.ctrl = ctrl; P.eps_ptr = eps_ptr;
@@ -634,14 +655,22 @@
     return A0_OK;
     A0_CATCH
 }
-
-extern "C" int a0_actor_qhead_env_step_enc(const float* feat, int E, int K, const float* W1, const float* b1, const float* W2, const float* b2, int A, int dueling,
+extern "C" int a0_actor_qhead_env_step(const float* feat, int E, int K, const float* W1, const float* b1, const float* W2, const float* b2, int A, int dueling,
+                                       float* scratch, unsigned long long seed, unsigned int stream_a, unsigned int stream_u, unsigned long long off_a,
+                                       unsigned long long off_u, float eps, const long long* ctrl, const float* eps_ptr, int* action, float* qmax,
+                                       unsigned long long env_seed, unsigned int rank, unsigned int g, const uint8_t* obs_in, uint8_t* obs_out, float* ep_ret,
+                                       float* final_mask, float* final_ret, int n, long long steps, double gamma, int* ring_act, float* ring_rew, float* ring_done,
+                                       const uint8_t* obs0, uint8_t* frames, long long cap, long long start_slot, int* r_act, float* r_rew, float* r_done, int task, void* stream) {
+    return a0_actor_qhead_env_step_wp(feat, E, K, W1, b1, W2, b2, A, dueling, scratch, seed, stream_a, stream_u, off_a, off_u, eps, ctrl, eps_ptr, action, qmax, env_seed, rank, g, obs_in, obs_out, ep_ret, final_mask, final_ret, n, steps, gamma, ring_act, ring_rew, ring_done, obs0, frames, cap, start_slot, r_act, r_rew, r_done, task, nullptr, stream);
+}
+
+extern "C" int a0_actor_qhead_env_step_enc_wp(const float* feat, int E, int K, const float* W1, const float* b1, const float* W2, const float* b2, int A, int dueling,
                                            float* scratch, unsigned long long seed, unsigned int stream_a, unsigned int stream_u, unsigned long long off_a,
                                            unsigned long long off_u, float eps, const long long* ctrl, const float* eps_ptr, int* action, float* qmax,
                                            unsigned long long env_seed, unsigned int rank, unsigned int g, const uint8_t* obs_in, uint8_t* obs_out, float* ep_ret,
                                            float* final_mask, float* final_ret, int n, long long steps, double gamma, int* ring_act, float* ring_rew, float* ring_done,
                                            const uint8_t* obs0, uint8_t* frames, long long cap, long long start_slot, int* r_act, float* r_rew, float* r_done, int task,
-                                           const float* wt, const a0_encoder_weights* w, float* act3_next, void* stream) {
+                                           const float* wt, const a0_encoder_weights* w, float* act3_next, const unsigned int* w1_planes, void* stream) {
     A0_TRY
     if (!feat || !W1 || !b1 || !W2 || !b2 || !scratch || !action || !qmax || E < 1 || K != 3136 || A < 1 || A + (dueling ? 1 : 0) > 24)
         return a0_fail(A0_EINVAL, "a0_actor_qhead_env_step_enc: bad argument (4 x 84 x 84 observations, A + dueling <= 24)");
@@ -651,11 +680,7 @@
     if ((((uintptr_t)obs_in) | ((uintptr_t)obs_out) | ((uintptr_t)obs0) | ((uintptr_t)frames)) & 15) return a0_fail(A0_EINVAL, "a0_actor_qhead_env_step_enc: buffers must be 16-byte aligned");
     a0_hip_backend bk{(hipStream_t)stream};
     const int splits = a0_fc1_splits(E, 512, K);
-    a0_mat_src a{feat, K};
-    a0_mat_src bw{W1, K};
-    EpiSlab::Params ep{scratch, (long long)E * 512, 512};
-    bk.tag = A0_TAG_DENSE_FWD;
-    a0_fc1_partial_launch(bk, a, bw, ep, E, 512, K, splits);
+    { const int rc = a0_actor_fc1_slabs(bk, feat, K, W1, w1_planes, E, splits, scratch); if (rc != A0_OK) return rc; }
     a0_qenv_args P;
     P.slabs = scratch; P.slab_stride = (long long)E * 512; P.nslab = splits; P.b1 = b1; P.W2 = W2; P.b2 = b2; P.A = A; P.dueling = dueling; P.E = E;
     P.rng_seed = seed; P.stream_a = stream_a; P.stream_u = stream_u; P.off_a = off_a; P.off_u = off_u; P.eps = eps; P.ctrl = ctrl; P.eps_ptr = eps_ptr;
@@ -665,6 +690,15 @@
     P.cap = cap; P.start = start_slot % cap; P.r_act = r_act; P.r_rew = r_rew; P.r_done = r_done; P.task = task;
     return a0_actor_step_enc_launch(P, wt, w, act3_next, (hipStream_t)stream);
     A0_CATCH
+}
+extern "C" int a0_actor_qhead_env_step_enc(const float* feat, int E, int K, const float* W1, const float* b1, const float* W2, const float* b2, int A, int dueling,
+                                           float* scratch, unsigned long long seed, unsigned int stream_a, unsigned int stream_u, unsigned long long off_a,
+                                           unsigned long long off_u, float eps, const long long* ctrl, const float* eps_ptr, int* action, float* qmax,
+                                           unsigned long long env_seed, unsigned int rank, unsigned int g, const uint8_t* obs_in, uint8_t* obs_out, float* ep_ret,
+                                           float* final_mask, float* final_ret, int n, long long steps, double gamma, int* ring_act, float* ring_rew, float* ring_done,
+                                           const uint8_t* obs0, uint8_t* frames, long long cap, long long start_slot, int* r_act, float* r_rew, float* r_done, int task,
+                                           const float* wt, const a0_encoder_weights* w, float* act3_next, void* stream) {
+    return a0_actor_qhead_env_step_enc_wp(feat, E, K, W1, b1, W2, b2, A, dueling, scratch, seed, stream_a, stream_u, off_a, off_u, eps, ctrl, eps_ptr, action, qmax, env_seed, rank, g, obs_in, obs_out, ep_ret, final_mask, final_ret, n, steps, gamma, ring_act, ring_rew, ring_done, obs0, frames, cap, start_slot, r_act, r_rew, r_done, task, wt, w, act3_next, nullptr, stream);
 }
 
 __global__ __launch_bounds__(256) void a0_mean_rows_kernel(const float* __restrict__ x, int E, float* __restrict__ out) {
diff --git a/agent0_amd/csrc/runtime.hip b/agent0_amd/csrc/runtime.hip
--- a/agent0_amd/csrc/runtime.hip
+++ b/agent0_amd/csrc/runtime.hip
@@ -270,6 +270,9 @@
     bool bound = false;
     float *own_flat = nullptr, *own_wt = nullptr, *own_eff = nullptr, *own_noise = nullptr;
     unsigned int* w_planes = nullptr;
+    unsigned int* fc1_planes = nullptr;
+    bool fc1_planes_on = true;
+    long long fc1_launches = 0;
     bool pool_on = false;
     a0_env_pool_desc pool{};
     uint8_t* ring_obs = nullptr;
@@ -317,6 +320,9 @@
             a->head_slabs = a->mem.alloc<float>((long long)a0_dense_fwd_partial_slabs(E, L->Npad, 512) * E * L->Npad);
             const long long sc = a0_dense_fwd_scratch(E, 512, L->feat);
             a->fwd_scratch = a->mem.alloc<float>(sc > 4 ? sc : 4);
+            if (a0_actor_fc1_dense_ok(E, 512, L->feat)) a->fc1_planes = a->mem.alloc<unsigned int>(a0_actor_fc1_planes_words(512, L->feat), false);
+        } else if (a0_actor_fc1_ok(E, 512, L->feat)) {
+            a->fc1_planes = a->mem.alloc<unsigned int>(a0_actor_fc1_planes_words(512, L->feat), false);
         }
         a->dist_Npad = L->Npad;
         a->bound = true;
@@ -392,6 +398,14 @@
     return A0_OK;
     A0_CATCH
 }
+
+extern "C" int a0_actor_set_fc1_planes(a0_actor* a, int on) {
+    if (!a) return a0_fail(A0_EINVAL, "a0_actor_set_fc1_planes: null handle");
+    a->fc1_planes_on = on != 0;
+    return A0_OK;
+}
+
+extern "C" long long a0_actor_fc1_launches(const a0_actor* a) { return a ? a->fc1_launches : -1; }
 
 extern "C" int a0_actor_set_eps_ladder(a0_actor* a, float alpha, long long i0, long long n_total) {
     A0_TRY
@@ -536,6 +550,10 @@
         epsilon = A0_EPS_PER_ENV;
     }
     if (a->pool_on) return a0_actor_rollout_pool(a, L, R, epsilon, eps_vec, V, w, start, stream);
+    const bool fc1p = !quant && a->fc1_planes_on && a->fc1_planes && a->feat == L->feat && (dist ? a0_actor_fc1_dense_ok(E, 512, a->feat) : a0_actor_fc1_ok(E, 512, a->feat));
+    a->fc1_launches += fc1p ? a->T : 0;
+    if (fc1p && !(L->d.noisy && a->steps % freq == 0)) A0_CHECK(a0_actor_fc1_planes(V.Wf(), a->fc1_planes, 512, a->feat, stream));
+    const unsigned int* const w1p = fc1p ? a->fc1_planes : nullptr;
     const bool step_enc = !a->own_flat;
     bool feat_ready = false;
     for (int t = 0; t < a->T; ++t) {
@@ -543,6 +561,7 @@
             A0_CHECK(a0_rng_normal(a->rng.seed, 4 , a->rng.reserve(4, L->noise_len), 0.1f, V.noise, L->noise_len, stream));
             A0_CHECK(a0_actor_compose(V, stream));
             if (planes) A0_CHECK(a0_split_planes(V.Wf(), a->w_planes, 512, L->feat, stream));
+            if (fc1p) A0_CHECK(a0_actor_fc1_planes(V.Wf(), a->fc1_planes, 512, a->feat, stream));
         }
         const uint8_t* cur_obs = a->obs[a->cur];
         a0_frames_arg f{cur_obs, nullptr, (long long)a->obs_bytes, 0};
@@ -585,7 +604,8 @@
             continue;
         }
         if (dist) {
-            A0_CHECK(a0_dense_fwd(a->act3, L->feat, V.Wf(), V.bf(), a->h, E, 512, L->feat, 1, a->fwd_scratch, stream));
+            if (fc1p) A0_CHECK(a0_actor_fc1_dense(a->act3, L->feat, a->fc1_planes, V.bf(), a->h, E, 512, L->feat, 1, a->fwd_scratch, stream));
+            else A0_CHECK(a0_dense_fwd(a->act3, L->feat, V.Wf(), V.bf(), a->h, E, 512, L->feat, 1, a->fwd_scratch, stream));
             const int ns = a0_dense_fwd_partial_slabs(E, L->Npad, 512);
             A0_CHECK(a0_dense_fwd_partial(a->h, 512, V.Wh(), E, L->Npad, 512, a->head_slabs, stream));
             const unsigned long long oa = a->rng.reserve(STREAM_EGREEDY_A, E), ou = a->rng.reserve(STREAM_EGREEDY_U, E);
@@ -616,18 +636,18 @@
         const int nxt = (a->cur + 1) % a->K;
         a->g += 1;
         if (step_enc && t + 1 < a->T) {
-            A0_CHECK(a0_actor_qhead_env_step_enc(a->act3, E, a->feat, V.Wf(), V.bf(), V.Wh(), V.bh(), A, a->d.dueling ? 1 : 0,
+            A0_CHECK(a0_actor_qhead_env_step_enc_wp(a->act3, E, a->feat, V.Wf(), V.bf(), V.Wh(), V.bh(), A, a->d.dueling ? 1 : 0,
                                                  a->scratch, a->rng.seed, STREAM_EGREEDY_A, STREAM_EGREEDY_U, off_a, off_u, epsilon, nullptr, eps_vec, a->action, a->qmax_all + (long long)t * E,
                                                  a->d.seed, a->d.rank, a->g, cur_obs, a->obs[nxt], a->ep_ret, a->stat_mask + (long long)t * E, a->stat_ret + (long long)t * E, a->n, a->steps,
                                                  a->d.discount, a->ring_act, a->ring_rew, a->ring_done, obs0, R->frames, R->size, (start + (long long)t * E) % R->size, R->act, R->rew, R->done,
-                                                 a->d.env_task, V.wt, &w, a->act3, stream));
+                                                 a->d.env_task, V.wt, &w, a->act3, w1p, stream));
             feat_ready = true;
         } else
-        A0_CHECK(a0_actor_qhead_env_step(a->act3, E, a->feat, V.Wf(), V.bf(), V.Wh(), V.bh(), A, a->d.dueling ? 1 : 0,
+        A0_CHECK(a0_actor_qhead_env_step_wp(a->act3, E, a->feat, V.Wf(), V.bf(), V.Wh(), V.bh(), A, a->d.dueling ? 1 : 0,
                                          a->scratch, a->rng.seed, STREAM_EGREEDY_A, STREAM_EGREEDY_U, off_a, off_u, epsilon, nullptr, eps_vec, a->action, a->qmax_all + (long long)t * E,
                                          a->d.seed, a->d.rank, a->g, cur_obs, a->obs[nxt], a->ep_ret, a->stat_mask + (long long)t * E, a->stat_ret + (long long)t * E, a->n, a->steps,
                                          a->d.discount, a->ring_act, a->ring_rew, a->ring_done, obs0, R->frames, R->size, (start + (long long)t * E) % R->size, R->act, R->rew, R->done,
-                                         a->d.env_task, stream));
+                                         a->d.env_task, w1p, stream));
         a->cur = nxt;
         a->steps += 1;
     }
diff --git a/agent0_amd/deepq/agent.py b/agent0_amd/deepq/agent.py
--- a/agent0_amd/deepq/agent.py
+++ b/agent0_amd/deepq/agent.py
@@ -74,6 +74,8 @@
         self._eps_host = torch.zeros(1).pin_memory()
         self.rank = int(rank)
         self.ladder_alpha = max(float(cfg.actor.eps_ladder), 0.0)
+        self.fc1_planes = True
+        self.fc1_launches = 0
         self.eps_vec = None
         self.out_act, self.out_rew, self.out_done = ops.zeros(E, dtype=torch.int32), ops.zeros(E), ops.zeros(E)
         self.atoms = self.model.head.atoms.reshape(-1).contiguous() if self.L.algo == "c51" else None
@@ -113,9 +115,12 @@
         return (self.ws.act3, E, L.feat, W1, b1, W2, b2, L.A, L.dueling, self._qh_scratch, rng.seed, rng.STREAM_EGREEDY_A, rng.STREAM_EGREEDY_U,
                 rng.reserve(rng.STREAM_EGREEDY_A, E), rng.reserve(rng.STREAM_EGREEDY_U, E), float(epsilon), self.action, self.qmax_all[t * E:(t + 1) * E], ctrl, eps_ptr)
 
-    def _dist_tail_args(self, epsilon, ctrl, eps_ptr, t):
+    def _dist_tail_args(self, epsilon, ctrl, eps_ptr, t, fc1p=None):
         L, ops, E, dev, rng = self.L, self.ops, self.E, self.model._dev, self.rng
-        dev._dense(self.ws.act3, L.feat, "fc1", self.ws.h, E, True)
+        if getattr(self, "_fc1p_on", False) if fc1p is None else fc1p:
+            ops.actor_fc1_dense(self.ws.act3, L.feat, dev.actor_fc1_planes, dev.wb("fc1")[1], self.ws.h, E, 512, L.feat, True, dev.scratch(ops.dense_fwd_scratch(E, 512, L.feat)))
+        else:
+            dev._dense(self.ws.act3, L.feat, "fc1", self.ws.h, E, True)
         Wh, bh = dev.wb("head")
         ns = ops.dense_fwd_partial(self.ws.h, 512, Wh, E, L.Npad, 512, self._head_slabs)
         return (self._head_slabs, ns, bh, L.Npad, L.A, L.T, L.dueling, 2 if L.algo == "c51" else 1, self.atoms, E, rng.seed, rng.STREAM_EGREEDY_A, rng.STREAM_EGREEDY_U,
@@ -148,7 +153,7 @@
             ops.actor_qhead(*self._qhead_args(epsilon, ctrl, eps_ptr, t))
             return
         if self.dist_tail:
-            ops.actor_dist_tail(*self._dist_tail_args(epsilon, ctrl, eps_ptr, t))
+            ops.actor_dist_tail(*self._dist_tail_args(epsilon, ctrl, eps_ptr, t, fc1p=False))
             return
         if self.quant_slabs:
             ops.actor_quantile_tail(*self._quant_tail_args(epsilon, ctrl, eps_ptr, t, w_planes=False))
@@ -199,12 +204,18 @@
                                and ops.dense_fwd_wplanes_ok(E * self.n_tau, 512, self.L.feat))
         if self._planes_on and not (cfg.learner.noisy_net and self.steps % cfg.learner.reset_noise_freq == 0):
             dev.refresh_fc1_planes()
+        self._fc1p_on = bool(self.fc1_planes and self.tail_env and bound and not test and hasattr(ops, "actor_fc1_planes")
+                             and (ops.actor_fc1_ok(E, 512, self.L.feat) if self.fused_tail else self.dist_tail and ops.actor_fc1_dense_ok(E, 512, self.L.feat)))
+        if self._fc1p_on and not (cfg.learner.noisy_net and self.steps % cfg.learner.reset_noise_freq == 0):
+            dev.refresh_actor_fc1_planes()
         feat_ready = False
         for t in range(T):
             if cfg.learner.noisy_net and self.steps % cfg.learner.reset_noise_freq == 0:
                 self.model.reset_noise(rng=self.rng)
                 if self._planes_on:
                     dev.refresh_fc1_planes()
+                if self._fc1p_on:
+                    dev.refresh_actor_fc1_planes()
             merged = bound and not test and (self.tail_env or (self.quant_tail and self.fused_commit))
             if not feat_ready:
                 self._act_device(epsilon, self.qs[t:t + 1], ctrl, eps_ptr, t, tail=not merged)
@@ -226,7 +237,8 @@
                 enc = (dev.wt, dev.encoder_weights(), self.ws.act3) if (step_enc and t + 1 < T) else None
                 self.obs = self.envs.act_step_commit(targs, self.stat_mask[t * E:(t + 1) * E], self.stat_ret[t * E:(t + 1) * E], self.n, self.steps,
                                                      float(cfg.learner.discount), self.ring_act, self.ring_rew, self.ring_done, obs0, rp, (start + t * E) % rp.size,
-                                                     kind=kind, enc=enc)
+                                                     kind=kind, enc=enc, w1_planes=dev.actor_fc1_planes if (self._fc1p_on and kind == "qhead") else None)
+                self.fc1_launches += 1 if self._fc1p_on else 0
                 feat_ready = enc is not None
                 self.steps += 1
                 continue
diff --git a/agent0_amd/deepq/engine.py b/agent0_amd/deepq/engine.py
--- a/agent0_amd/deepq/engine.py
+++ b/agent0_amd/deepq/engine.py
@@ -215,6 +215,12 @@
         if getattr(self, "fc1_planes", None) is None:
             self.fc1_planes = torch.empty(self.ops.weight_planes_words(512, self.L.feat), dtype=torch.int32, device=self.flat.device)
         self.ops.split_planes(W, self.fc1_planes, 512, self.L.feat)
+
+    def refresh_actor_fc1_planes(self):
+        W, _ = self.wb("fc1")
+        if getattr(self, "actor_fc1_planes", None) is None:
+            self.actor_fc1_planes = torch.empty(self.ops.actor_fc1_planes_words(512, self.L.feat), dtype=torch.int32, device=self.flat.device)
+        self.ops.actor_fc1_planes(W, self.actor_fc1_planes, 512, self.L.feat)
 
     def head_slabs(self, ws: Workspace, B, taus: torch.Tensor, n_tau: int, slabs: torch.Tensor, cos_ready: bool = False, w_planes: bool = False,
                    splits: Optional[dict] = None) -> int:
diff --git a/agent0_amd/deepq/native_loop.py b/agent0_amd/deepq/native_loop.py
--- a/agent0_amd/deepq/native_loop.py
+++ b/agent0_amd/deepq/native_loop.py
@@ -175,6 +175,8 @@
         ok(lib.a0_actor_create(C.addressof(ad), C.addressof(self.actor)), "a0_actor_create")
         if eng.target_tau > 0:
             ok(lib.a0_learner_set_target_tau(self.learner, C.c_double(eng.target_tau)), "a0_learner_set_target_tau")
+        if not actor.fc1_planes:
+            ok(lib.a0_actor_set_fc1_planes(self.actor, 0), "a0_actor_set_fc1_planes")
         if actor.ladder_alpha > 0:
             from .dist import eps_ladder_span
             ops.actor_set_eps_ladder(self.actor, actor.ladder_alpha, *eps_ladder_span(int(tr.rank), self.E))
diff --git a/agent0_amd/ops.py b/agent0_amd/ops.py
--- a/agent0_amd/ops.py
+++ b/agent0_amd/ops.py
@@ -335,6 +335,30 @@
         check(self.lib.a0_dense_fwd_wplanes(_req(X, torch.float32, (R - 1) * ldx + K, "X"), ldx, _req(planes, torch.int32, self.weight_planes_words(N, K), "planes"),
                                             _req(b, torch.float32, N, "b"), _req(Y, torch.float32, R * N, "Y"), R, N, K, int(relu), _stream()), "a0_dense_fwd_wplanes")
 
+    def actor_fc1_planes_words(self, N, K) -> int:
+        return int(self.lib.a0_actor_fc1_planes_words(N, K))
+
+    def actor_fc1_planes(self, W, planes, N, K):
+        check(self.lib.a0_actor_fc1_planes(_req(W, torch.float32, N * K, "W"), _req(planes, torch.int32, self.actor_fc1_planes_words(N, K), "planes"), N, K, _stream()),
+              "a0_actor_fc1_planes")
+
+    def actor_fc1_ok(self, R, N, K) -> bool:
+        return bool(self.lib.a0_actor_fc1_ok(R, N, K))
+
+    def actor_fc1(self, X, ldx, planes, R, N, K, slabs, splits=None) -> int:
+        ns = self.dense_fwd_partial_slabs(R, N, K) if splits is None else int(splits)
+        check(self.lib.a0_actor_fc1_n(_req(X, torch.float32, (R - 1) * ldx + K, "X"), ldx, _req(planes, torch.int32, self.actor_fc1_planes_words(N, K), "planes"), R, N, K, ns,
+                                      _req(slabs, torch.float32, ns * R * N, "slabs"), _stream()), "a0_actor_fc1")
+        return ns
+
+    def actor_fc1_dense_ok(self, R, N, K) -> bool:
+        return bool(self.lib.a0_actor_fc1_dense_ok(R, N, K))
+
+    def actor_fc1_dense(self, X, ldx, planes, b, Y, R, N, K, relu, scratch):
+        check(self.lib.a0_actor_fc1_dense(_req(X, torch.float32, (R - 1) * ldx + K, "X"), ldx, _req(planes, torch.int32, self.actor_fc1_planes_words(N, K), "planes"),
+                                          _req(b, torch.float32, N, "b"), _req(Y, torch.float32, R * N, "Y"), R, N, K, int(relu),
+                                          _req(scratch, torch.float32, self.dense_fwd_scratch(R, N, K), "scratch"), _stream()), "a0_actor_fc1_dense")
+
     def dense_fwd_mul(self, X, ldx, W, b, M, group, Y, R, N, K, relu):
         check(self.lib.a0_dense_fwd_mul(_req(X, torch.float32, (R - 1) * ldx + K, "X"), ldx, _req(W, torch.float32, N * K, "W"), _req(b, torch.float32, N, "b"),
                                         _req(M, torch.float32, ((R - 1) // group + 1) * N, "M"), group, _req(Y, torch.float32, R * N, "Y"), R, N, K, int(relu), _stream()),
@@ -756,28 +780,10 @@
 
     def actor_qhead_env_step(self, feat, E, K, W1, b1, W2, b2, A, dueling, scratch, seed, stream_a, stream_u, off_a, off_u, eps, action, qmax, ctrl, eps_ptr,
                              env_seed, rank, g, obs_in, obs_out, ep_ret, final_mask, final_ret, n, steps, gamma, ring_act, ring_rew, ring_done, obs0, frames, cap,
-                             start_slot, r_act, r_rew, r_done, task=0):
+                             start_slot, r_act, r_rew, r_done, task=0, w1_planes=None):
         nq = A + (1 if dueling else 0)
         nb = E * 4 * 84 * 84
-        check(self.lib.a0_actor_qhead_env_step(
-            _req(feat, torch.float32, E * K, "feat"), E, K, _req(W1, torch.float32, 512 * K, "W1"), _req(b1, torch.float32, 512, "b1"),
-            _req(W2, torch.float32, nq * 512, "W2"), _req(b2, torch.float32, nq, "b2"), A, int(dueling),
-            _req(scratch, torch.float32, self.actor_qhead_scratch(E, K), "scratch"), seed, stream_a, stream_u, off_a, off_u, float(eps),
-            _req(ctrl, torch.int64, 8, "ctrl", optional=True), _eps_req(eps, eps_ptr, E),
-            _req(action, torch.int32, E, "action"), _req(qmax, torch.float32, E, "qmax"),
-            env_seed, rank, g, _req(obs_in, torch.uint8, nb, "obs_in"), _req(obs_out, torch.uint8, nb, "obs_out"), _req(ep_ret, torch.float32, E, "ep_ret"),
-            _req(final_mask, torch.float32, E, "final_mask"), _req(final_ret, torch.float32, E, "final_ret"), n, steps, float(gamma),
-            _req(ring_act, torch.int32, n * E, "ring_act"), _req(ring_rew, torch.float32, n * E, "ring_rew"), _req(ring_done, torch.float32, n * E, "ring_done"),
-            _req(obs0, torch.uint8, nb, "obs0"), _req(frames, torch.uint8, cap * 8 * 84 * 84, "frames"), cap, start_slot, _req(r_act, torch.int32, cap, "r_act"),
-            _req(r_rew, torch.float32, cap, "r_rew"), _req(r_done, torch.float32, cap, "r_done"), int(task), _stream()), "a0_actor_qhead_env_step")
-
-    def actor_qhead_env_step_enc(self, feat, E, K, W1, b1, W2, b2, A, dueling, scratch, seed, stream_a, stream_u, off_a, off_u, eps, action, qmax, ctrl, eps_ptr,
-                                 env_seed, rank, g, obs_in, obs_out, ep_ret, final_mask, final_ret, n, steps, gamma, ring_act, ring_rew, ring_done, obs0, frames, cap,
-                                 start_slot, r_act, r_rew, r_done, task=0, wt=None, enc_w=None, act3_next=None):
-        nq = A + (1 if dueling else 0)
-        nb = E * 4 * 84 * 84
-        ew = self._enc_w(enc_w)
-        check(self.lib.a0_actor_qhead_env_step_enc(
+        check(self.lib.a0_actor_qhead_env_step_wp(
             _req(feat, torch.float32, E * K, "feat"), E, K, _req(W1, torch.float32, 512 * K, "W1"), _req(b1, torch.float32, 512, "b1"),
             _req(W2, torch.float32, nq * 512, "W2"), _req(b2, torch.float32, nq, "b2"), A, int(dueling),
             _req(scratch, torch.float32, self.actor_qhead_scratch(E, K), "scratch"), seed, stream_a, stream_u, off_a, off_u, float(eps),
@@ -788,7 +794,27 @@
             _req(ring_act, torch.int32, n * E, "ring_act"), _req(ring_rew, torch.float32, n * E, "ring_rew"), _req(ring_done, torch.float32, n * E, "ring_done"),
             _req(obs0, torch.uint8, nb, "obs0"), _req(frames, torch.uint8, cap * 8 * 84 * 84, "frames"), cap, start_slot, _req(r_act, torch.int32, cap, "r_act"),
             _req(r_rew, torch.float32, cap, "r_rew"), _req(r_done, torch.float32, cap, "r_done"), int(task),
-            _req(wt, torch.float32, self.conv_wt_floats(4), "wt"), C.addressof(ew), _req(act3_next, torch.float32, E * K, "act3_next"), _stream()), "a0_actor_qhead_env_step_enc")
+            _req(w1_planes, torch.int32, self.actor_fc1_planes_words(512, K), "w1_planes", optional=True), _stream()), "a0_actor_qhead_env_step")
+
+    def actor_qhead_env_step_enc(self, feat, E, K, W1, b1, W2, b2, A, dueling, scratch, seed, stream_a, stream_u, off_a, off_u, eps, action, qmax, ctrl, eps_ptr,
+                                 env_seed, rank, g, obs_in, obs_out, ep_ret, final_mask, final_ret, n, steps, gamma, ring_act, ring_rew, ring_done, obs0, frames, cap,
+                                 start_slot, r_act, r_rew, r_done, task=0, wt=None, enc_w=None, act3_next=None, w1_planes=None):
+        nq = A + (1 if dueling else 0)
+        nb = E * 4 * 84 * 84
+        ew = self._enc_w(enc_w)
+        check(self.lib.a0_actor_qhead_env_step_enc_wp(
+            _req(feat, torch.float32, E * K, "feat"), E, K, _req(W1, torch.float32, 512 * K, "W1"), _req(b1, torch.float32, 512, "b1"),
+            _req(W2, torch.float32, nq * 512, "W2"), _req(b2, torch.float32, nq, "b2"), A, int(dueling),
+            _req(scratch, torch.float32, self.actor_qhead_scratch(E, K), "scratch"), seed, stream_a, stream_u, off_a, off_u, float(eps),
+            _req(ctrl, torch.int64, 8, "ctrl", optional=True), _eps_req(eps, eps_ptr, E),
+            _req(action, torch.int32, E, "action"), _req(qmax, torch.float32, E, "qmax"),
+            env_seed, rank, g, _req(obs_in, torch.uint8, nb, "obs_in"), _req(obs_out, torch.uint8, nb, "obs_out"), _req(ep_ret, torch.float32, E, "ep_ret"),
+            _req(final_mask, torch.float32, E, "final_mask"), _req(final_ret, torch.float32, E, "final_ret"), n, steps, float(gamma),
+            _req(ring_act, torch.int32, n * E, "ring_act"), _req(ring_rew, torch.float32, n * E, "ring_rew"), _req(ring_done, torch.float32, n * E, "ring_done"),
+            _req(obs0, torch.uint8, nb, "obs0"), _req(frames, torch.uint8, cap * 8 * 84 * 84, "frames"), cap, start_slot, _req(r_act, torch.int32, cap, "r_act"),
+            _req(r_rew, torch.float32, cap, "r_rew"), _req(r_done, torch.float32, cap, "r_done"), int(task),
+            _req(wt, torch.float32, self.conv_wt_floats(4), "wt"), C.addressof(ew), _req(act3_next, torch.float32, E * K, "act3_next"),
+            _req(w1_planes, torch.int32, self.actor_fc1_planes_words(512, K), "w1_planes", optional=True), _stream()), "a0_actor_qhead_env_step_enc")
 
     def mean_rows(self, x, T, E, out):
         check(self.lib.a0_mean_rows(_req(x, torch.float32, T * E, "x"), T, E, _req(out, torch.float32, T, "out"), _stream()), "a0_mean_rows")
diff --git a/include/agent0_hip.h b/include/agent0_hip.h
--- a/include/agent0_hip.h
+++ b/include/agent0_hip.h
@@ -125,6 +125,13 @@
 int a0_split_planes(const float* W, unsigned int* planes, int N, int K, void* stream);
 int a0_dense_fwd_wplanes_ok(int R, int N, int K);
 int a0_dense_fwd_wplanes(const float* X, int ldx, const unsigned int* Wplanes, const float* b, float* Y, int R, int N, int K, int relu, void* stream);
+
+long long a0_actor_fc1_planes_words(int N, int K);
+int a0_actor_fc1_planes(const float* W, unsigned int* planes, int N, int K, void* stream);
+int a0_actor_fc1_ok(int R, int N, int K);
+int a0_actor_fc1_dense_ok(int R, int N, int K);
+int a0_actor_fc1_dense(const float* X, int ldx, const unsigned int* planes, const float* b, float* Y, int R, int N, int K, int relu, float* scratch, void* stream);
+int a0_actor_fc1_n(const float* X, int ldx, const unsigned int* planes, int R, int N, int K, int splits, float* slabs, void* stream);
 
 int a0_gemm_mode(int mode);
 
@@ -307,6 +314,8 @@
 int a0_actor_snapshot(a0_actor* actor, const a0_learner* learner, void* stream);
 int a0_actor_rollout(a0_actor* actor, a0_learner* learner, a0_rbuf* replay, float epsilon, void* stream);
 int a0_actor_set_eps_ladder(a0_actor* actor, float alpha, long long i0, long long n_total);
+int a0_actor_set_fc1_planes(a0_actor* actor, int on);
+long long a0_actor_fc1_launches(const a0_actor* actor);
 int a0_actor_collect(a0_actor* actor, float* qs_host, float* returns_host, int max_returns, int* n_returns, void* stream);
 typedef struct a0_env_pool_desc {
     int E, nstack, W, use_life_loss;
@@ -401,6 +410,12 @@
                             unsigned long long env_seed, unsigned int rank, unsigned int g, const uint8_t* obs_in, uint8_t* obs_out, float* ep_ret,
                             float* final_mask, float* final_ret, int n, long long steps, double gamma, int* ring_act, float* ring_rew, float* ring_done,
                             const uint8_t* obs0, uint8_t* frames, long long cap, long long start_slot, int* r_act, float* r_rew, float* r_done, int task, void* stream);
+int a0_actor_qhead_env_step_wp(const float* feat, int E, int K, const float* W1, const float* b1, const float* W2, const float* b2, int A, int dueling,
+                            float* scratch, unsigned long long seed, unsigned int stream_a, unsigned int stream_u, unsigned long long off_a,
+                            unsigned long long off_u, float eps, const long long* ctrl, const float* eps_ptr, int* action, float* qmax,
+                            unsigned long long env_seed, unsigned int rank, unsigned int g, const uint8_t* obs_in, uint8_t* obs_out, float* ep_ret,
+                            float* final_mask, float* final_ret, int n, long long steps, double gamma, int* ring_act, float* ring_rew, float* ring_done,
+                            const uint8_t* obs0, uint8_t* frames, long long cap, long long start_slot, int* r_act, float* r_rew, float* r_done, int task, const unsigned int* w1_planes, void* stream);
 int a0_mean_rows(const float* x, int T, int E, float* out, void* stream);
 
 int a0_actor_qhead_env_step_enc(const float* feat, int E, int K, const float* W1, const float* b1, const float* W2, const float* b2, int A, int dueling,
@@ -410,6 +425,13 @@
                                 float* final_mask, float* final_ret, int n, long long steps, double gamma, int* ring_act, float* ring_rew, float* ring_done,
                                 const uint8_t* obs0, uint8_t* frames, long long cap, long long start_slot, int* r_act, float* r_rew, float* r_done, int task,
                                 const float* wt, const a0_encoder_weights* w, float* act3_next, void* stream);
+int a0_actor_qhead_env_step_enc_wp(const float* feat, int E, int K, const float* W1, const float* b1, const float* W2, const float* b2, int A, int dueling,
+                                float* scratch, unsigned long long seed, unsigned int stream_a, unsigned int stream_u, unsigned long long off_a,
+                                unsigned long long off_u, float eps, const long long* ctrl, const float* eps_ptr, int* action, float* qmax,
+                                unsigned long long env_seed, unsigned int rank, unsigned int g, const uint8_t* obs_in, uint8_t* obs_out, float* ep_ret,
+                                float* final_mask, float* final_ret, int n, long long steps, double gamma, int* ring_act, float* ring_rew, float* ring_done,
+                                const uint8_t* obs0, uint8_t* frames, long long cap, long long start_slot, int* r_act, float* r_rew, float* r_done, int task,
+                                const float* wt, const a0_encoder_weights* w, float* act3_next, const unsigned int* w1_planes, void* stream);
 int a0_actor_dist_tail_env_step_enc(const float* slabs, long long slab_stride, int nslab, const float* bias, int ld, int A, int T, int dueling, int mode,
                                     const float* atoms, int E, unsigned long long seed, unsigned int stream_a, unsigned int stream_u, unsigned long long off_a,
                                     unsigned long long off_u, float eps, const long long* ctrl, const float* eps_ptr, int* action, float* qmax,
```
